# CODARcode/MGARD

Hardware: AMD Instinct MI355X
Metric: compress GB/s (input) at rel-Linf 1e-3, 3D 512^3 f32, decompose+quantize on device-resident data (higher is better)
Workload: dtype f32; 1 GPU; 3D 512x512x512 float32 uniform grid, REL L-inf tol 1e-3, s=inf; [norm+]decompose+quantize (int64 out); l_target=9, dict_size=8192, parallelism=1 subdomain per GPU

## Files before the change

### include/mgard_hip.h

```cpp
#ifndef MGARD_HIP_H
#define MGARD_HIP_H

#include <stddef.h>
#include <stdint.h>

#ifdef __cplusplus
extern "C" {
#endif

typedef enum mgh_status {
  MGH_SUCCESS = 0,
  MGH_ERR_INVALID_ARGUMENT = -1,
  MGH_ERR_UNSUPPORTED_DIMENSION = -2,
  MGH_ERR_UNSUPPORTED_DTYPE = -3,
  MGH_ERR_DEVICE = -4,
  MGH_ERR_OUT_OF_MEMORY = -5,
  MGH_ERR_NO_DEVICE = -6
} mgh_status;

typedef enum mgh_dtype { MGH_FLOAT = 0, MGH_DOUBLE = 1 } mgh_dtype;
typedef enum mgh_error_bound { MGH_REL = 0, MGH_ABS = 1 } mgh_error_bound;

#define MGH_MAX_DIM 5

// ... 30 lines not shown
int mgh_dequantize(mgh_hierarchy *h, int64_t *d_quantized, int error_bound_type, double tol,
                   double s, double norm, uint64_t dict_size, int prep_huffman,
                   const uint64_t *d_outlier_idx, const int64_t *d_outlier_val,
                   uint64_t outlier_count, void *d_coeff, void *stream);

int mgh_decompose_quantize(mgh_hierarchy *h, const void *d_data, int error_bound_type,
                           double tol, double s, double norm, double *h_norm_out,
                           uint64_t dict_size, int prep_huffman, int64_t *d_quantized,
                           uint64_t *d_outlier_count, uint64_t *d_outlier_idx,
                           int64_t *d_outlier_val, uint64_t outlier_capacity,
                           void *d_coeff_opt, void *stream);

int mgh_decompose_quantize_sym16(mgh_hierarchy *h, const void *d_data, int error_bound_type,
                                 double tol, double s, double norm, double *h_norm_out,
                                 uint64_t dict_size, uint16_t *d_symbols,
                                 uint64_t *d_outlier_count, uint64_t *d_outlier_idx,
                                 int64_t *d_outlier_val, uint64_t outlier_capacity, void *stream);

int mgh_dequantize_recompose_sym16(mgh_hierarchy *h, const uint16_t *d_symbols, int error_bound_type,
                                   double tol, double s, double norm, uint64_t dict_size,
                                   const uint64_t *d_outlier_idx, const int64_t *d_outlier_val,
                                   uint64_t outlier_count, void *d_data_out, void *stream);
int mgh_sym16_supported(const mgh_hierarchy *h);

#define MGH_LD_IN 0
#define MGH_LD_OUT 1
int mgh_set_ld(mgh_hierarchy *h, int which, const uint64_t *ld);

int mgh_norm_stream_begin(mgh_hierarchy *h, void *stream);
int mgh_norm_stream_add(mgh_hierarchy *h, const void *d_part, uint64_t count, double s, int cold,
                        void *stream);

int mgh_norm_device(mgh_hierarchy *h, const void *d_data, double s, void *d_norm_out,
                    void *stream);

int mgh_decompose_quantize_dn(mgh_hierarchy *h, const void *d_data, int error_bound_type,
                              double tol, double s, const void *d_norm, uint64_t num_subdomains,
                              uint64_t dict_size, int prep_huffman, int64_t *d_quantized,
                              uint64_t *d_outlier_count, uint64_t *d_outlier_idx,
                              int64_t *d_outlier_val, uint64_t outlier_capacity, void *stream);

int mgh_dequantize_recompose(mgh_hierarchy *h, int64_t *d_quantized, int error_bound_type,
                             double tol, double s, double norm, uint64_t dict_size,
                             int prep_huffman, const uint64_t *d_outlier_idx,
                             const int64_t *d_outlier_val, uint64_t outlier_count, void *d_data,
                             void *stream);

int mgh_recompose_to_level(mgh_hierarchy *h, const void *d_coeff, int level, void *d_out, void *stream);
int mgh_dequantize_recompose_to_level(mgh_hierarchy *h, int64_t *d_quantized, int error_bound_type,
                                      double tol, double s, double norm, uint64_t dict_size,
                                      int prep_huffman, const uint64_t *d_outlier_idx,
                                      const int64_t *d_outlier_val, uint64_t outlier_count, int level,
                                      void *d_out, void *stream);
int mgh_dequantize_recompose_sym16_to_level(mgh_hierarchy *h, const uint16_t *d_symbols,
                                            int error_bound_type, double tol, double s, double norm,
                                            uint64_t dict_size, const uint64_t *d_outlier_idx,
                                            const int64_t *d_outlier_val, uint64_t outlier_count,
                                            int level, void *d_out, void *stream);
int mgh_level_box_from_linear(mgh_hierarchy *h, const int64_t *d_linear, int level, int64_t *d_box_out,
                              void *stream);
int mgh_dequantize_recompose_linear_to_level(mgh_hierarchy *h, int64_t *d_linear, int error_bound_type,
                                             double tol, double s, double norm, uint64_t dict_size,
                                             int prep_huffman, const uint64_t *d_outlier_idx,
                                             const int64_t *d_outlier_val, uint64_t outlier_count,
                                             int level, void *d_out, void *stream);
int mgh_refine_level(mgh_hierarchy *h, const void *d_coarse, int64_t *d_segment, int error_bound_type,
                     double tol, double s, double norm, uint64_t dict_size, int prep_huffman,
                     const uint64_t *d_outlier_idx, const int64_t *d_outlier_val, uint64_t outlier_count,
                     int level, void *d_out, void *stream);
int mgh_level_nodes(const mgh_hierarchy *h, int level, int dim, uint64_t *h_idx_out, uint64_t cap);

int mgh_outlier_restore(int64_t *d_q, uint64_t n, const uint64_t *d_outlier_idx,
                        const int64_t *d_outlier_val, uint64_t outlier_count, void *stream);

int mgh_level_linearize(mgh_hierarchy *h, const int64_t *d_in, int64_t *d_out, int inverse,
                        uint64_t *d_outlier_idx, const uint64_t *d_outlier_count, uint64_t outlier_count,
                        uint64_t outlier_capacity, void *stream);

int mgh_profile_enable(mgh_hierarchy *h, int enable);
int mgh_profile_filter(mgh_hierarchy *h, const char *kernel_name_or_null);
int mgh_profile_read(mgh_hierarchy *h, const char **names, double *total_ms, uint64_t *launches,
                     int cap, int reset);

int mgh_stream_calibrate(int dtype, const void *d_in, int64_t *d_out, void *d_side, uint64_t n,
                         int reps, double *ms_out, void *stream);

#ifdef __cplusplus
}
#endif
#endif
```

### mgard_amd/__init__.py

```python
import ctypes as C
import os

import numpy as np

from . import _build

REL, ABS = 0, 1
LD_IN, LD_OUT = 0, 1
FLOAT, DOUBLE = 0, 1
INF = float("inf")

_lib = None

SYMBOLS = [
    "mgh_last_error", "mgh_device_count", "mgh_hierarchy_create", "mgh_hierarchy_destroy",
    "mgh_l_target", "mgh_level_shape", "mgh_total_num_elems", "mgh_device_bytes", "mgh_norm_device_ptr",
    "mgh_hierarchy_table", "mgh_norm", "mgh_decompose", "mgh_recompose", "mgh_quantize",
    "mgh_dequantize", "mgh_decompose_quantize", "mgh_dequantize_recompose",
    "mgh_norm_device", "mgh_decompose_quantize_dn", "mgh_decompose_quantize_sym16",
    "mgh_dequantize_recompose_sym16", "mgh_sym16_supported",
    "mgh_profile_enable", "mgh_profile_filter", "mgh_profile_read", "mgh_stream_calibrate",
    "mgh_level_linearize", "mgh_outlier_restore", "mgh_norm_stream_begin", "mgh_norm_stream_add",
    "mgh_set_ld",
    "mgh_recompose_to_level", "mgh_dequantize_recompose_to_level",
    "mgh_dequantize_recompose_sym16_to_level", "mgh_level_nodes",
    "mgh_level_box_from_linear", "mgh_dequantize_recompose_linear_to_level",
    "mgh_refine_level",
]


class MgardHipError(RuntimeError):
    pass


def lib_path():
    return _build.LIB


def load_library():
    global _lib
    if _lib is not None:
        return _lib
    if not os.path.exists(_build.LIB):
        raise MgardHipError(
            "libmgard_hip.so is not built: run `python -c 'import __graft_entry__ as g; g.build()'`")
    import torch
    L = C.CDLL(_build.LIB)
    vp, u64, i64p, u64p = C.c_void_p, C.c_uint64, C.POINTER(C.c_int64), C.POINTER(C.c_uint64)
    L.mgh_last_error.restype = C.c_char_p
    L.mgh_device_count.restype = C.c_int
    L.mgh_hierarchy_create.argtypes = [C.POINTER(vp), C.c_int, u64p, C.c_int, C.POINTER(vp),
                                       C.c_int, u64, C.c_int]
    L.mgh_hierarchy_destroy.argtypes = [vp]
    L.mgh_hierarchy_destroy.restype = None
    L.mgh_l_target.argtypes = [vp]
    L.mgh_level_shape.argtypes = [vp, C.c_int, u64p]
    L.mgh_total_num_elems.argtypes = [vp]
    L.mgh_total_num_elems.restype = u64
    L.mgh_device_bytes.argtypes = [vp]
    L.mgh_device_bytes.restype = C.c_size_t
    L.mgh_hierarchy_table.argtypes = [vp, C.c_int, C.c_int, C.c_int, vp, u64]
    L.mgh_hierarchy_table.restype = C.c_int64
    L.mgh_norm.argtypes = [vp, vp, C.c_double, C.POINTER(C.c_double), vp]
    L.mgh_decompose.argtypes = [vp, vp, vp, vp]
    L.mgh_recompose.argtypes = [vp, vp, vp, vp]
    L.mgh_quantize.argtypes = [vp, vp, C.c_int, C.c_double, C.c_double, C.c_double, u64, C.c_int,
                               vp, vp, vp, vp, u64, vp]
    L.mgh_dequantize.argtypes = [vp, vp, C.c_int, C.c_double, C.c_double, C.c_double, u64,
                                 C.c_int, vp, vp, u64, vp, vp]
    L.mgh_decompose_quantize.argtypes = [vp, vp, C.c_int, C.c_double, C.c_double, C.c_double,
                                         C.POINTER(C.c_double), u64, C.c_int, vp, vp, vp, vp, u64,
                                         vp, vp]
    L.mgh_norm_device.argtypes = [vp, vp, C.c_double, vp, vp]
    L.mgh_norm_stream_begin.argtypes = [vp, vp]
    L.mgh_set_ld.argtypes = [vp, C.c_int, u64p]
    L.mgh_norm_stream_add.argtypes = [vp, vp, u64, C.c_double, C.c_int, vp]
    L.mgh_dequantize_recompose_sym16.argtypes = [vp, vp, C.c_int, C.c_double, C.c_double, C.c_double, u64,
                                                 vp, vp, u64, vp, vp]
    L.mgh_sym16_supported.argtypes = [vp]
    L.mgh_decompose_quantize_sym16.argtypes = [vp, vp, C.c_int, C.c_double, C.c_double, C.c_double,
                                               C.POINTER(C.c_double), u64, vp, vp, vp, vp, u64, vp]
    L.mgh_decompose_quantize_dn.argtypes = [vp, vp, C.c_int, C.c_double, C.c_double, vp, u64, u64,
                                            C.c_int, vp, vp, vp, vp, u64, vp]
    L.mgh_dequantize_recompose.argtypes = [vp, vp, C.c_int, C.c_double, C.c_double, C.c_double,
                                           u64, C.c_int, vp, vp, u64, vp, vp]
    L.mgh_profile_enable.argtypes = [vp, C.c_int]
    L.mgh_profile_filter.argtypes = [vp, C.c_char_p]
    L.mgh_profile_read.argtypes = [vp, C.POINTER(C.c_char_p), C.POINTER(C.c_double), u64p,
                                   C.c_int, C.c_int]
    L.mgh_outlier_restore.argtypes = [vp, u64, vp, vp, u64, vp]
    L.mgh_level_linearize.argtypes = [vp, vp, vp, C.c_int, vp, vp, u64, u64, vp]
    L.mgh_recompose_to_level.argtypes = [vp, vp, C.c_int, vp, vp]
    L.mgh_dequantize_recompose_to_level.argtypes = [vp, vp, C.c_int, C.c_double, C.c_double, C.c_double,
                                                    u64, C.c_int, vp, vp, u64, C.c_int, vp, vp]
    L.mgh_dequantize_recompose_sym16_to_level.argtypes = [vp, vp, C.c_int, C.c_double, C.c_double,
                                                          C.c_double, u64, vp, vp, u64, C.c_int, vp, vp]
    L.mgh_level_box_from_linear.argtypes = [vp, vp, C.c_int, vp, vp]
    L.mgh_dequantize_recompose_linear_to_level.argtypes = [vp, vp, C.c_int, C.c_double, C.c_double, C.c_double,
                                                           u64, C.c_int, vp, vp, u64, C.c_int, vp, vp]
    L.mgh_refine_level.argtypes = [vp, vp, vp, C.c_int, C.c_double, C.c_double, C.c_double, u64, C.c_int, vp, vp, u64,
                                   C.c_int, vp, vp]
    L.mgh_level_nodes.argtypes = [vp, C.c_int, C.c_int, u64p, u64]
    L.mgh_stream_calibrate.argtypes = [C.c_int, vp, vp, vp, u64, C.c_int, C.POINTER(C.c_double), vp]
    _lib = L
    return L


def _check(rc):
    if rc < 0:
        raise MgardHipError("mgard_hip error %d: %s" % (rc, load_library().mgh_last_error().decode()))
    return rc


def _stream():
    import torch
    return C.c_void_p(torch.cuda.current_stream().cuda_stream)


_NP = {FLOAT: np.float32, DOUBLE: np.float64}


class Hierarchy:

    def __init__(self, shape, dtype="float32", coords=None, normalize_coordinates=True,
                 max_level=None, device=0):
        import torch
        L = load_library()
        if not torch.cuda.is_available():
            raise MgardHipError("no HIP device visible: mgard_amd has no CPU fallback")
        self.shape = tuple(int(s) for s in shape)
        self.D = len(self.shape)
        self.np_dtype = np.dtype(dtype)
        self.dtype = {np.dtype(np.float32): FLOAT, np.dtype(np.float64): DOUBLE}[self.np_dtype]
        self.torch_dtype = torch.float32 if self.dtype == FLOAT else torch.float64
        self.device = int(device)
        shp = (C.c_uint64 * self.D)(*self.shape)
        cptr = None
        if coords is not None:
            self._coords = [np.ascontiguousarray(c, dtype=self.np_dtype) for c in coords]
            cptr = (C.c_void_p * self.D)(*[c.ctypes.data for c in self._coords])
        h = C.c_void_p()
        _check(L.mgh_hierarchy_create(C.byref(h), self.D, shp, self.dtype, cptr,
                                      int(normalize_coordinates),
                                      2**64 - 1 if max_level is None else int(max_level),
                                      self.device))
        self._h = h
        self._ld = {LD_IN: None, LD_OUT: None}
        self.l_target = L.mgh_l_target(h)
        self.total = int(L.mgh_total_num_elems(h))

    def close(self):
        if getattr(self, "_h", None) and _lib is not None:
            try:
                _lib.mgh_hierarchy_destroy(self._h)
            except Exception:
                pass
            self._h = None

    __del__ = close

    def level_shape(self, l):
        out = (C.c_uint64 * self.D)()
        _check(load_library().mgh_level_shape(self._h, l, out))
        return tuple(int(x) for x in out)

    def level_nodes(self, level, dim):
        n = self.shape[dim] if 0 <= dim < self.D else 1
        out = (C.c_uint64 * n)()
# ... 199 lines not shown
                self._h, self._chk(q, torch.int64), ebtype, tol, s, norm, dict_size, int(prep_huffman),
                C.c_void_p(outlier_idx.data_ptr() if n else 0),
                C.c_void_p(outlier_val.data_ptr() if n else 0), n, int(level),
                C.c_void_p(out.data_ptr()), _stream()))
            return out
        out = self._new_out(q.device) if out is None else out
        _check(load_library().mgh_dequantize_recompose(
            self._h, self._chk(q, torch.int64), ebtype, tol, s, norm, dict_size, int(prep_huffman),
            C.c_void_p(outlier_idx.data_ptr() if n else 0),
            C.c_void_p(outlier_val.data_ptr() if n else 0), n, self._chk(out), _stream()))
        return out

    def level_linearize(self, q, inverse=False, outlier_idx=None):
        import torch
        out = torch.empty_like(q)
        n = 0 if outlier_idx is None else int(outlier_idx.numel())
        _check(load_library().mgh_level_linearize(
            self._h, self._chk(q, torch.int64), C.c_void_p(out.data_ptr()), int(inverse),
            C.c_void_p(outlier_idx.data_ptr() if n else 0), None, n, 0, _stream()))
        return out

    def _linear_head(self, lin, level):
        import torch
        need = 1
        for e in self.level_shape(level):
            need *= int(e)
        if not (lin.is_cuda and lin.dtype == torch.int64 and lin.is_contiguous() and lin.numel() >= need):
            raise ValueError("expected a contiguous cuda int64 tensor of at least %d elements "
                             "(the head of the level-linearised array)" % need)
        return need

    def level_box_from_linear(self, lin, level, out=None):
        import torch
        need = self._linear_head(lin, level)
        if out is None:
            out = torch.empty(tuple(int(e) for e in self.level_shape(level)), dtype=torch.int64, device=lin.device)
        elif not (out.is_cuda and out.dtype == torch.int64 and out.is_contiguous() and out.numel() >= need):
            raise ValueError("out: expected a contiguous cuda int64 tensor of at least %d elements" % need)
        _check(load_library().mgh_level_box_from_linear(
            self._h, C.c_void_p(lin.data_ptr()), int(level), C.c_void_p(out.data_ptr()), _stream()))
        return out

    def dequantize_recompose_linear(self, lin, ebtype, tol, s, norm, dict_size=8192, prep_huffman=True,
                                    outlier_idx=None, outlier_val=None, out=None, level=None):
        level = self.l_target if level is None else int(level)
        self._linear_head(lin, level)
        n = 0 if outlier_idx is None else int(outlier_idx.numel())
        out = self._level_out(level, out, lin.device)
        _check(load_library().mgh_dequantize_recompose_linear_to_level(
            self._h, C.c_void_p(lin.data_ptr()), ebtype, tol, s, norm, dict_size, int(prep_huffman),
            C.c_void_p(outlier_idx.data_ptr() if n else 0), C.c_void_p(outlier_val.data_ptr() if n else 0),
            n, level, C.c_void_p(out.data_ptr()), _stream()))
        return out

    def refine_level(self, coarse, segment, ebtype, tol, s, norm, level, dict_size=8192, prep_huffman=True,
                     outlier_idx=None, outlier_val=None, out=None):
        import torch
        level = int(level)
        if not 1 <= level <= self.l_target:
            raise ValueError("level must be in 1 .. l_target")
        lo = hi = 1
        for e in self.level_shape(level - 1):
            lo *= int(e)
        for e in self.level_shape(level):
            hi *= int(e)
        if not (coarse.is_cuda and coarse.is_contiguous() and coarse.dtype == self.torch_dtype and
                coarse.numel() == lo):
            raise ValueError("coarse: expected the contiguous cuda array of level %d (%d elements)" % (level - 1, lo))
        if not (segment.is_cuda and segment.dtype == torch.int64 and segment.is_contiguous() and
                segment.numel() >= hi - lo):
            raise ValueError("segment: expected a contiguous cuda int64 tensor of at least %d elements" % (hi - lo))
        n = 0 if outlier_idx is None else int(outlier_idx.numel())
        out = self._level_out(level, out, coarse.device)
        _check(load_library().mgh_refine_level(
            self._h, C.c_void_p(coarse.data_ptr()), C.c_void_p(segment.data_ptr()), ebtype, tol, s, norm, dict_size,
            int(prep_huffman), C.c_void_p(outlier_idx.data_ptr() if n else 0),
            C.c_void_p(outlier_val.data_ptr() if n else 0), n, level, C.c_void_p(out.data_ptr()), _stream()))
        return out

    def profile(self, enable=True, only=None):
        _check(load_library().mgh_profile_filter(self._h, only.encode() if only else None))
        _check(load_library().mgh_profile_enable(self._h, int(enable)))

    def profile_read(self, reset=True):
        cap = 64
        names = (C.c_char_p * cap)()
        ms = (C.c_double * cap)()
        cnt = (C.c_uint64 * cap)()
        n = _check(load_library().mgh_profile_read(self._h, names, ms, cnt, cap, int(reset)))
        return {names[i].decode(): (ms[i], int(cnt[i])) for i in range(min(n, cap))}
```

### mgard_amd/csrc/capi.hip

```cpp
#include "../../include/mgard_hip.h"

#include <hip/hip_runtime.h>
#include <hip/hip_ext.h>

#include <cmath>
#include <cstdio>
#include <cstdlib>
#include <cstring>
#include <limits>
#include <atomic>
#include <map>
#include <mutex>
#include <string>
#include <type_traits>
#include <vector>

#include "env.hpp"
#include "hierarchy.hpp"
#include "ipk_plan.hpp"
#include "kernels_v1.hpp"
#include "kernels_ipk.hpp"
#include "kernels_ipk_stream.hpp"
#include "kernels_ipk_spec.hpp"
#include "kernels_ipk_dma.hpp"
#include "kernels_fused.hpp"
#include "kernels_fused2.hpp"
#include "kernels_box.hpp"
#include "kernels_tail.hpp"
#include "kernels_recompose.hpp"
#include "kernels_recompose2.hpp"
#include "kernels_nd.hpp"
#include "kernels_level.hpp"

namespace {

thread_local std::string g_last_error;

int fail(int code, const std::string &msg) {
  g_last_error = msg;
  return code;
}

#define HIP_TRY(expr)                                                                          \
  do {                                                                                         \
    hipError_t _e = (expr);                                                                    \
    if (_e != hipSuccess)                                                                      \
      return fail(_e == hipErrorOutOfMemory ? MGH_ERR_OUT_OF_MEMORY : MGH_ERR_DEVICE,          \
                  std::string(#expr) + ": " + hipGetErrorString(_e));                          \
  } while (0)

struct ProfileEntry {
  std::vector<std::pair<hipEvent_t, hipEvent_t>> pending;
  double total_ms = 0;
  uint64_t launches = 0;
};

}

struct mgh_hierarchy {
  int dtype = MGH_FLOAT;
  int device = 0;
  size_t num_cu = 256;
  int D = 0, L = 0;
  uint64_t total = 0;
  uint64_t plane_elems = 0;
  void *host = nullptr;
  void *impl = nullptr;
  bool profiling = false;
  int nd_rows = 1;
  bool force_nd_ipk = false;
  bool force_v1 = false;
  int force_v1_env = -1;
  bool force_nd = false;
  std::string prof_filter;
  mgh::IpkTuning ipk;
  int absmax_warm_mb = 192;
  int fused_faces = 1;
  int fused_tall = 1;
  int slice_batch = 1;
  int fused_xcd = 1;
  int fused_fixed = 1;
  int fused_wide = 1;
  int fused4 = 1;
  int box = 1;
  int outlier_agg = 2;
  int sym16_mixed = 1;
  int tail_solves = 1;
  size_t cls1 = 256, cls2 = 2048;
  int rch[3] = {1, 4, 16};
  int ipk_range_mb = 128;
  bool no_head = false;
  bool debug_sync = false;
  std::map<std::string, ProfileEntry> prof;
  size_t device_bytes = 0;
  uint64_t shape[MGH_MAX_DIM] = {};
  uint64_t ld[2][MGH_MAX_DIM] = {};
  bool has_ld[2] = {false, false};
};

namespace {

using namespace mgh;

template <typename T> int chunk_warmup_need(const std::vector<T> &tt) {
  const size_t n = tt.size() / 3;
  if (n < 2) return 0;
  const double target = -((sizeof(T) == 4 ? 24 : 53) + 12);
  std::vector<double> lf(n), lb(n);
  for (size_t i = 0; i < n; i++) {
    const double f = std::fabs((double)tt[i]);
    const double b = tt[2 * n + i] != 0 ? std::fabs((double)tt[n + i] / (double)tt[2 * n + i]) : 0.0;
    lf[i] = f > 0 ? std::log2(f) : -64.0;
    lb[i] = b > 0 ? std::log2(b) : -64.0;
  }
  int need = 0;
  for (const auto *lg : {&lf, &lb}) {
    for (size_t i = 0; i < n; i++) {
      double acc = 0;
      size_t k = 0;
      while (i + k < n && acc > target) acc += (*lg)[i + k++];
      if (acc > target) break;
      need = std::max(need, (int)k);
    }
  }
  return (need + 7) / 8 * 8;
}

template <typename T> struct LevelTables {
  const T *ratio[3] = {nullptr, nullptr, nullptr};
  const T *mass[3] = {nullptr, nullptr, nullptr};
  const T *thomas[3] = {nullptr, nullptr, nullptr};
  Box3 box;
  bool active[3] = {false, false, false};
};

template <typename T> struct DeviceState {
  HostHierarchy<T> *hh = nullptr;
  T *tables = nullptr;
  int *marks = nullptr;
  std::vector<LevelTables<T>> lt;
  std::vector<size_t> lt_end;
  struct NdLevel {
    const T *ratio[kNd], *mass[kNd], *thomas[kNd];
  };
  std::vector<NdLevel> nd;
  T *nd_w = nullptr, *nd_a = nullptr, *nd_b = nullptr;
  size_t nd_cap = 0;
  std::vector<T *> nodal4;
  T *load4 = nullptr, *corr4 = nullptr;
  bool state4_ready = false;
  std::vector<T *> nodal;
  T *t1 = nullptr, *t2 = nullptr, *t3 = nullptr;
  int t12_level = 0;
  T *level_box = nullptr;
  size_t level_box_elems = 0;
  T *scratch_full = nullptr;
  T *qz = nullptr;
  unsigned long long *scalar = nullptr;
  unsigned long long *fscal = nullptr;
  int scalar_slot = 0;
  bool fscal_dirty = false;
  bool norm_streamed = false;
  T *normval = nullptr;
  unsigned long long *oh_key = nullptr;
  long long *oh_val = nullptr;
  size_t oh_slots = 0;
  int64_t *qbox = nullptr;
  size_t qbox_elems = 0;
  T *spec_y = nullptr, *spec_a = nullptr, *spec_b = nullptr;
  size_t spec_y_elems = 0, spec_edge_elems = 0;
  unsigned long long *spec_fixed = nullptr;
  unsigned long long *outliers_seen = nullptr;
  QuantMeta qmeta;
  size_t full_I = 0, full_J = 0;
  T *pack_in = nullptr, *pack_out = nullptr;
};

template <typename T> HostHierarchy<T> *HH(const mgh_hierarchy *h) {
  return static_cast<HostHierarchy<T> *>(h->host);
}
template <typename T> DeviceState<T> *DS(const mgh_hierarchy *h) {
  return static_cast<DeviceState<T> *>(h->impl);
}

template <typename F> int launch(mgh_hierarchy *h, const char *name, hipStream_t s, F &&f) {
  if (h->debug_sync) {
    std::fprintf(stderr, "[mgh] %s\n", name);
    std::fflush(stderr);
    f();
    HIP_TRY(hipGetLastError());
    HIP_TRY(hipDeviceSynchronize());
    return MGH_SUCCESS;
  }
  if (!h->profiling || (!h->prof_filter.empty() && h->prof_filter != name)) {
    f();
    HIP_TRY(hipGetLastError());
    return MGH_SUCCESS;
  }
  hipEvent_t a, b;
  HIP_TRY(hipEventCreate(&a));
  HIP_TRY(hipEventCreate(&b));
  HIP_TRY(hipEventRecord(a, s));
  f();
  HIP_TRY(hipGetLastError());
  HIP_TRY(hipEventRecord(b, s));
  h->prof[name].pending.emplace_back(a, b);
  return MGH_SUCCESS;
}

template <typename K, typename... Args>
int launch_kernel(mgh_hierarchy *h, const char *name, hipStream_t s, K kernel, dim3 grid, dim3 block,
                  size_t lds, Args... args) {
  if (h->debug_sync || !h->profiling || (!h->prof_filter.empty() && h->prof_filter != name))
    return launch(h, name, s, [&] { hipLaunchKernelGGL(kernel, grid, block, (uint32_t)lds, s, args...); });
  hipEvent_t a, b;
  HIP_TRY(hipEventCreate(&a));
  HIP_TRY(hipEventCreate(&b));
  hipExtLaunchKernelGGL(kernel, grid, block, (uint32_t)lds, s, a, b, 0, args...);
  HIP_TRY(hipGetLastError());
  h->prof[name].pending.emplace_back(a, b);
  return MGH_SUCCESS;
}

#define TRY(expr)                 \
  do {                            \
    int _rc = (expr);             \
    if (_rc != MGH_SUCCESS) return _rc; \
  } while (0)

inline dim3 grid3(uint32_t n0, uint32_t n1, uint32_t n2, dim3 blk) {
  return dim3((n2 + blk.x - 1) / blk.x, (n1 + blk.y - 1) / blk.y, n0);
}

template <typename T> int dev_alloc(mgh_hierarchy *h, T **p, size_t count) {
  *p = nullptr;
  if (count == 0) return MGH_SUCCESS;
  HIP_TRY(hipMalloc((void **)p, count * sizeof(T)));
  h->device_bytes += count * sizeof(T);
  return MGH_SUCCESS;
}

template <typename T> void dev_free(mgh_hierarchy *h, T **p, size_t count) {
  if (!*p) return;
  if (hipFree(*p) == hipSuccess) h->device_bytes -= std::min(h->device_bytes, count * sizeof(T));
  *p = nullptr;
}

template <typename T> int build_device_state(mgh_hierarchy *h) {
  HostHierarchy<T> *hh = HH<T>(h);
  auto *ds = new DeviceState<T>();
  h->impl = ds;
  ds->hh = hh;
  const int D = hh->D, L = hh->L;
  if (D > 3) {
    std::vector<T> arena;
    auto push = [&](const std::vector<T> &v) {
      size_t off = arena.size();
      arena.insert(arena.end(), v.begin(), v.end());
      while (arena.size() % 4) arena.push_back(0);
      return off;
    };
    struct Off { size_t r[kNd], m[kNd], t[kNd]; };
    std::vector<Off> offs(L + 1);
    for (int l = 1; l <= L; l++)
      for (int d = 0; d < D; d++) {
        offs[l].r[d] = push(hh->lv[l][d].ratio);
        offs[l].m[d] = push(hh->mass_table(l, d));
// ... 19 lines not shown
    TRY(dev_alloc(h, &ds->marks, marks.size()));
    HIP_TRY(hipMemcpy(ds->marks, marks.data(), marks.size() * sizeof(int), hipMemcpyHostToDevice));
    TRY(dev_alloc(h, &ds->qz, (size_t)2 * (L + 1)));
    TRY(dev_alloc(h, &ds->scalar, (size_t)2));
    TRY(dev_alloc(h, &ds->fscal, (size_t)2));
    HIP_TRY(hipMemset(ds->fscal, 0, 16));
    TRY(dev_alloc(h, &ds->normval, (size_t)2));
    return MGH_SUCCESS;
  }

  std::vector<T> arena;
  auto push = [&](const std::vector<T> &v) {
    size_t off = arena.size();
    arena.insert(arena.end(), v.begin(), v.end());
    while (arena.size() % 4) arena.push_back(0);
    return off;
  };
  struct Off {
    size_t ratio[3], mass[3], thomas[3];
  };
  std::vector<Off> offs(L + 1);
  ds->lt.resize(L + 1);
  for (int l = 1; l <= L; l++) {
    LevelTables<T> &t = ds->lt[l];
    for (int k = 0; k < 3; k++) {
      const int d = D - 3 + k;
      if (d < 0) {
        t.box.n[k] = t.box.m[k] = 1;
        t.active[k] = false;
        continue;
      }
      t.active[k] = true;
      t.box.n[k] = (uint32_t)hh->level_shape[l][d];
      t.box.m[k] = (uint32_t)hh->level_shape[l - 1][d];
      offs[l].ratio[k] = push(hh->lv[l][d].ratio);
      offs[l].mass[k] = push(hh->mass_table(l, d));
      const std::vector<T> tt = hh->thomas_table(l - 1, d);
      h->ipk.chunk_need = std::max(h->ipk.chunk_need, chunk_warmup_need(tt));
      offs[l].thomas[k] = push(tt);
    }
  }
  TRY(dev_alloc(h, &ds->tables, arena.size()));
  HIP_TRY(hipMemcpy(ds->tables, arena.data(), arena.size() * sizeof(T), hipMemcpyHostToDevice));
  ds->lt_end.assign(L + 1, 0);
  for (int l = 1; l <= L; l++) {
    size_t next = arena.size();
    for (int l2 = l + 1; l2 <= L && next == arena.size(); l2++)
      for (int k = 0; k < 3; k++)
        if (ds->lt[l2].active[k]) {
          next = offs[l2].ratio[k];
          break;
        }
    ds->lt_end[l] = next;
  }
  for (int l = 1; l <= L; l++)
    for (int k = 0; k < 3; k++)
      if (ds->lt[l].active[k]) {
        ds->lt[l].ratio[k] = ds->tables + offs[l].ratio[k];
        ds->lt[l].mass[k] = ds->tables + offs[l].mass[k];
        ds->lt[l].thomas[k] = ds->tables + offs[l].thomas[k];
      }

  ds->nd.resize(L + 1);
  for (int l = 1; l <= L; l++)
    for (int d = 0; d < D; d++) {
      const int k = d + 3 - D;
      ds->nd[l].ratio[d] = ds->lt[l].ratio[k];
      ds->nd[l].mass[d] = ds->lt[l].mass[k];
      ds->nd[l].thomas[d] = ds->lt[l].thomas[k];
    }

  std::vector<int> marks;
  ds->qmeta.D = D;
  ds->qmeta.calc_vol = 0;
  for (int d = 0; d < D; d++) {
    ds->qmeta.shape[d] = (uint32_t)hh->shape[d];
    ds->qmeta.markoff[d] = (uint32_t)marks.size();
    marks.insert(marks.end(), hh->marks[d].begin(), hh->marks[d].end());
  }
  TRY(dev_alloc(h, &ds->marks, marks.size()));
  HIP_TRY(hipMemcpy(ds->marks, marks.data(), marks.size() * sizeof(int), hipMemcpyHostToDevice));

  ds->nodal.assign(L + 1, nullptr);
  for (int l = 0; l < L; l++) {
    size_t cnt = 1;
    for (int d = 0; d < D; d++) cnt *= hh->level_shape[l][d];
    TRY(dev_alloc(h, &ds->nodal[l], cnt));
  }
  if (L >= 1) {
    const Box3 &b = ds->lt[L].box;
    TRY(dev_alloc(h, &ds->t3, (size_t)b.m[0] * b.m[1] * b.m[2]));
  }
  TRY(dev_alloc(h, &ds->qz, (size_t)2 * (L + 1)));
  TRY(dev_alloc(h, &ds->scalar, (size_t)2));
  TRY(dev_alloc(h, &ds->fscal, (size_t)2));
  HIP_TRY(hipMemset(ds->fscal, 0, 16));
  TRY(dev_alloc(h, &ds->normval, (size_t)2));
  ds->full_J = hh->shape[D - 1];
  ds->full_I = (D >= 2 ? hh->shape[D - 2] : 1) * ds->full_J;
  return MGH_SUCCESS;
}

template <typename T> void destroy_state(mgh_hierarchy *h) {
  auto *ds = DS<T>(h);
  if (ds) {
    (void)hipFree(ds->tables);
    (void)hipFree(ds->marks);
    for (T *p : ds->nodal) (void)hipFree(p);
    (void)hipFree(ds->t1);
    (void)hipFree(ds->t2);
    (void)hipFree(ds->t3);
    (void)hipFree(ds->scratch_full);
    (void)hipFree(ds->pack_in);
    (void)hipFree(ds->pack_out);
    (void)hipFree(ds->nd_w);
    (void)hipFree(ds->nd_a);
    (void)hipFree(ds->nd_b);
    for (T *p : ds->nodal4) (void)hipFree(p);
    (void)hipFree(ds->load4);
    (void)hipFree(ds->corr4);
    (void)hipFree(ds->qz);
    (void)hipFree(ds->scalar);
    (void)hipFree(ds->fscal);
    (void)hipFree(ds->normval);
    (void)hipFree(ds->oh_key);
    (void)hipFree(ds->oh_val);
    (void)hipFree(ds->qbox);
    (void)hipFree(ds->level_box);
    (void)hipFree(ds->spec_y);
    (void)hipFree(ds->spec_a);
    (void)hipFree(ds->spec_b);
    (void)hipFree(ds->spec_fixed);
    (void)hipHostFree(ds->outliers_seen);
    delete ds;
  }
  delete HH<T>(h);
}

template <typename T> int ensure_scratch(mgh_hierarchy *h) {
  auto *ds = DS<T>(h);
  if (!ds->scratch_full) TRY(dev_alloc(h, &ds->scratch_full, (size_t)h->total));
  return MGH_SUCCESS;
}

template <typename K> int allow_big_lds(K kernel, size_t bytes = kLdsPerCU) {
  HIP_TRY(hipFuncSetAttribute(reinterpret_cast<const void *>(kernel),
                              hipFuncAttributeMaxDynamicSharedMemorySize, (int)bytes));
  return MGH_SUCCESS;
}
template <typename K> int allow_big_lds_once(K kernel, std::atomic<uint64_t> &done, size_t bytes = kLdsPerCU) {
  int dev = 0;
  HIP_TRY(hipGetDevice(&dev));
  const uint64_t bit = (uint64_t)1 << (dev & 63);
  if (done.load(std::memory_order_acquire) & bit) return MGH_SUCCESS;
  TRY(allow_big_lds(kernel, bytes));
  done.fetch_or(bit, std::memory_order_release);
  return MGH_SUCCESS;
}

template <int... V, typename F> int with_value(int v, F &&f) {
  int rc = MGH_ERR_INVALID_ARGUMENT;
  (void)((v == V ? (rc = f(std::integral_constant<int, V>{}), true) : false) || ...);
  return rc;
}

template <typename T> struct IpkArgs {
  mgh_hierarchy *h;
  const char *name;
  T *x;
  const T *tt;
  T *add_to;
  int sign;
  hipStream_t s;
  int add() const { return add_to ? (sign > 0 ? 1 : -1) : 0; }
};

template <typename T> int spec_scratch(mgh_hierarchy *h, size_t total, size_t edges, hipStream_t s) {
  auto *ds = DS<T>(h);
  if (total > ds->spec_y_elems) {
    (void)hipFree(ds->spec_y);
    ds->spec_y = nullptr;
    ds->spec_y_elems = 0;
    HIP_TRY(hipMalloc(&ds->spec_y, total * sizeof(T)));
    ds->spec_y_elems = total;
  }
  if (edges > ds->spec_edge_elems) {
    (void)hipFree(ds->spec_a);
    (void)hipFree(ds->spec_b);
    ds->spec_a = ds->spec_b = nullptr;
    ds->spec_edge_elems = 0;
    HIP_TRY(hipMalloc(&ds->spec_a, edges * sizeof(T)));
    HIP_TRY(hipMalloc(&ds->spec_b, edges * sizeof(T)));
    ds->spec_edge_elems = edges;
  }
  if (!ds->spec_fixed) {
    HIP_TRY(hipMalloc(&ds->spec_fixed, 16));
    HIP_TRY(hipMemsetAsync(ds->spec_fixed, 0, 16, s));
  }
  return MGH_SUCCESS;
}

template <typename T> int ipk_launch_spec(const IpkPlan &p, const IpkArgs<T> &a, int axis) {
  const IpkGeom &g = p.geom;
  const SpecGeom G{g.n, p.S, p.K, p.nchunk, g.npencil, g.n_inner, g.outer_stride, g.inner_stride, g.stride, axis != 2};
  const size_t total = (size_t)g.npencil * g.n;
  TRY(spec_scratch<T>(a.h, total, (size_t)g.npencil * p.nchunk, a.s));
  auto *ds = DS<T>(a.h);
  T *x = a.x, *y = ds->spec_y, *ea = ds->spec_a, *eb = ds->spec_b;
  unsigned long long *fx = ds->spec_fixed;
  unsigned *mm = reinterpret_cast<unsigned *>(ds->spec_fixed + 1);
  hipStream_t s = a.s;
  HIP_TRY(hipMemsetAsync(mm, 0, 8, s));
  return launch(a.h, a.name, s, [&] {
    k_ipk_spec_fwd<T><<<p.grid, 64, 0, s>>>(G, x, y, a.tt, ea, eb);
    k_ipk_spec_check<T><<<p.check_grid, 256, 0, s>>>(p.nchunk, g.npencil, ea, eb, +1, mm);
    k_ipk_spec_fix<T><<<p.fix_grid, 64, 0, s>>>(G, x, y, a.tt, ea, eb, +1, fx, mm);
    k_ipk_spec_bwd<T><<<p.grid, 64, 0, s>>>(G, y, x, a.tt, ea, eb);
    k_ipk_spec_check<T><<<p.check_grid, 256, 0, s>>>(p.nchunk, g.npencil, ea, eb, -1, mm + 1);
    k_ipk_spec_fix<T><<<p.fix_grid, 64, 0, s>>>(G, y, x, a.tt, ea, eb, -1, fx, mm + 1);
    if (a.add_to) k_ipk_spec_apply<T><<<p.apply_grid, 256, 0, s>>>(total, a.add_to, x, a.sign);
  });
}

template <typename T, bool CHUNKED> int ipk_launch_lds_contig(const IpkPlan &p, const IpkArgs<T> &a) {
  static std::atomic<uint64_t> once{0};
  TRY(allow_big_lds_once(k_ipk_lds_contig<T, CHUNKED>, once, p.lds_attr));
  return launch(a.h, a.name, a.s, [&] {
    k_ipk_lds_contig<T, CHUNKED><<<p.grid, p.block, p.lds, a.s>>>(p.geom.npencil, p.geom.n, p.pad, p.magic, p.P,
                                                                  a.x, a.tt, a.add_to, a.sign, p.K);
  });
}

template <typename T, int ADD> int ipk_launch_dma(const IpkPlan &p, const IpkArgs<T> &a) {
  constexpr uint32_t U = 64 / sizeof(T), KR = 10;
  const IpkGeom &g = p.geom;
  static std::atomic<uint64_t> once{0};
  TRY(allow_big_lds_once(k_ipk_dma<T, U, KR, ADD>, once, p.lds_attr));
  return launch(a.h, a.name, a.s, [&] {
    k_ipk_dma<T, U, KR, ADD><<<p.grid, p.block, p.lds, a.s>>>(g.npencil, g.n_inner, g.outer_stride, 1, g.stride,
                                                              g.n, a.x, a.tt, a.add_to);
  });
}

template <typename T, int KR, bool CONTIG> int ipk_launch_stream(const IpkPlan &p, const IpkArgs<T> &a) {
  constexpr uint32_t U = 64 / sizeof(T);
  const IpkGeom &g = p.geom;
  static std::atomic<uint64_t> once{0};
  TRY(allow_big_lds_once(k_ipk_stream<T, U, KR, 1, CONTIG, false>, once, p.lds_attr));
  return launch(a.h, a.name, a.s, [&] {
    k_ipk_stream<T, U, KR, 1, CONTIG, false><<<p.grid, p.block, p.lds, a.s>>>(
        g.npencil, g.n_inner, g.outer_stride, g.inner_stride, g.stride, g.n, p.W, p.n_glob, a.x, a.tt, a.add_to,
        a.sign);
  });
}

template <typename T, int W> int ipk_launch_lds_strided(const IpkPlan &p, const IpkArgs<T> &a) {
  const IpkGeom &g = p.geom;
  static std::atomic<uint64_t> once{0};
  TRY(allow_big_lds_once(k_ipk_lds_strided<T, W>, once, p.lds_attr));
  return launch(a.h, a.name, a.s, [&] {
    k_ipk_lds_strided<T, W><<<p.grid, p.block, p.lds, a.s>>>(g.npencil / g.n_inner, g.n_inner, g.outer_stride,
                                                             g.stride, g.n, a.x, a.tt, a.add_to, a.sign);
  });
}

template <typename T, int AXIS> int ipk_launch_thread(const IpkPlan &p, const IpkArgs<T> &a, const uint32_t *m) {
  return launch(a.h, a.name, a.s, [&] {
    k_ipk<T, AXIS><<<dim3(p.grid, p.grid_y, 1), dim3(p.block, 1, 1), 0, a.s>>>(m[0], m[1], m[2], a.x, a.tt,
                                                                             a.add_to, a.sign);
  });
}

template <typename T>
int ipk_launch(mgh_hierarchy *h, int axis, const uint32_t *m, T *x, const T *tt, T *add_to,
               int sign, hipStream_t s, uint32_t nbatch = 1, size_t batch_stride = 0) {
  if (nbatch > 1 && axis != 0) return fail(MGH_ERR_INVALID_ARGUMENT, "ipk_launch: batches along the slowest axis only");
  static const char *names[3] = {"ipk_r", "ipk_c", "ipk_f"};
  const IpkArgs<T> a{h, names[axis], x, tt, add_to, sign, s};
  const IpkPlan p = ipk_plan(h->ipk, sizeof(T), axis, m, nbatch, batch_stride);
  switch (p.kernel) {
  case IpkKernel::Spec: return ipk_launch_spec<T>(p, a, axis);
  case IpkKernel::LdsContigChunked: return ipk_launch_lds_contig<T, true>(p, a);
  case IpkKernel::Dma:
    if constexpr (sizeof(T) == 4)
      return with_value<0, 1, -1>(a.add(), [&](auto add) { return ipk_launch_dma<T, add()>(p, a); });
    break;
  case IpkKernel::Stream:
    if constexpr (sizeof(T) == 4)
      if (p.KR == 16)
        return axis == 2 ? ipk_launch_stream<T, 16, true>(p, a) : ipk_launch_stream<T, 16, false>(p, a);
    return axis == 2 ? ipk_launch_stream<T, 8, true>(p, a) : ipk_launch_stream<T, 8, false>(p, a);
  case IpkKernel::LdsContig: return ipk_launch_lds_contig<T, false>(p, a);
  case IpkKernel::LdsStrided:
    return with_value<64, 48, 32, 16>((int)p.W, [&](auto w) { return ipk_launch_lds_strided<T, w()>(p, a); });
  case IpkKernel::Thread:
    if (p.per_batch) {
      for (uint32_t bi = 0; bi < nbatch; bi++)
        TRY(ipk_launch<T>(h, axis, m, x + (size_t)bi * batch_stride, tt,
                          add_to ? add_to + (size_t)bi * batch_stride : nullptr, sign, s));
      return MGH_SUCCESS;
    }
    return with_value<0, 1, 2>(axis, [&](auto ax) { return ipk_launch_thread<T, ax()>(p, a, m); });
  }
  return fail(MGH_ERR_INVALID_ARGUMENT, "ipk_launch: no kernel for this plan");
}

template <typename T>
int ipk_fc_launch(mgh_hierarchy *h, const uint32_t *m, T *x, const T *tt_f, const T *tt_c,
                  hipStream_t s) {
  const uint32_t pitch = m[2] | 1u;
  if (ipk_plane_fits_lds(sizeof(T), m)) {
    static std::atomic<uint64_t> once{0};
    TRY(allow_big_lds_once(k_ipk_plane_fc<T>, once));
    const uint32_t magic = (uint32_t)((((uint64_t)1 << 32) + m[2] - 1) / m[2]);
    return launch(h, "ipk_fc", s, [&] {
      k_ipk_plane_fc<T><<<m[0], 256, (size_t)m[1] * pitch * sizeof(T), s>>>(m[1], m[2], pitch, magic,
                                                                              x, tt_f, tt_c);
    });
  }
  TRY(ipk_launch<T>(h, 2, m, x, tt_f, nullptr, +1, s));
  return ipk_launch<T>(h, 1, m, x, tt_c, nullptr, +1, s);
}

template <typename T>
int correction(mgh_hierarchy *h, int l, const T *coef, size_t cI, size_t cJ, T *target, int sign,
               hipStream_t s, int top_level = -1) {
  auto *ds = DS<T>(h);
  const LevelTables<T> &t = ds->lt[l];
  const Box3 &b = t.box;
  const dim3 blk(64, 4, 1);
  const int tl = top_level < 0 ? h->L : top_level;
  if (ds->t12_level < tl) {
    if (ds->t12_level >= 1) {
      const Box3 &ob = ds->lt[ds->t12_level].box;
      dev_free(h, &ds->t1, (size_t)ob.n[0] * ob.n[1] * ob.m[2]);
      dev_free(h, &ds->t2, (size_t)ob.n[0] * ob.m[1] * ob.m[2]);
      ds->t12_level = 0;
    }
    const Box3 &tb = ds->lt[tl].box;
    const size_t c1 = (size_t)tb.n[0] * tb.n[1] * tb.m[2], c2 = (size_t)tb.n[0] * tb.m[1] * tb.m[2];
    int rc = dev_alloc(h, &ds->t1, c1);
    if (rc == MGH_SUCCESS) rc = dev_alloc(h, &ds->t2, c2);
    if (rc != MGH_SUCCESS) {
      dev_free(h, &ds->t1, c1);
      dev_free(h, &ds->t2, c2);
      return rc;
    }
    ds->t12_level = tl;
  }
  TRY(launch(h, "lpk_f", s, [&] {
    k_lpk<T, 2><<<grid3(b.n[0], b.n[1], b.m[2], blk), blk, 0, s>>>(
        b.n[0], b.n[1], b.n[2], b.n[2], b.m[2], coef, cI, cJ, ds->t1, (size_t)b.n[1] * b.m[2],
        (size_t)b.m[2], t.mass[2], b.m[0], b.m[1]);
  }));
  T *cur = ds->t1;
  if (t.active[1]) {
    TRY(launch(h, "lpk_c", s, [&] {
      k_lpk<T, 1><<<grid3(b.n[0], b.m[1], b.m[2], blk), blk, 0, s>>>(
          b.n[0], b.n[1], b.m[2], b.n[1], b.m[1], cur, (size_t)b.n[1] * b.m[2], (size_t)b.m[2],
          ds->t2, (size_t)b.m[1] * b.m[2], (size_t)b.m[2], t.mass[1], 0, 0);
    }));
    cur = ds->t2;
  }
  if (t.active[0]) {
    TRY(launch(h, "lpk_r", s, [&] {
      k_lpk<T, 0><<<grid3(b.m[0], b.m[1], b.m[2], blk), blk, 0, s>>>(
          b.n[0], b.m[1], b.m[2], b.n[0], b.m[0], cur, (size_t)b.m[1] * b.m[2], (size_t)b.m[2],
          ds->t3, (size_t)b.m[1] * b.m[2], (size_t)b.m[2], t.mass[0], 0, 0);
    }));
    cur = ds->t3;
  }
  const int last = t.active[0] ? 0 : (t.active[1] ? 1 : 2);
  TRY(ipk_launch<T>(h, 2, b.m, cur, t.thomas[2], last == 2 ? target : nullptr, sign, s));
  if (t.active[1])
    TRY(ipk_launch<T>(h, 1, b.m, cur, t.thomas[1], last == 1 ? target : nullptr, sign, s));
  if (t.active[0]) TRY(ipk_launch<T>(h, 0, b.m, cur, t.thomas[0], target, sign, s));
  return MGH_SUCCESS;
}

template <typename T> struct QuantParams {
  std::vector<T> qz, vol;
  int64_t dict_size = 0;
  int prep_huffman = 0;
  int64_t *q = nullptr;
  uint16_t *q16 = nullptr;
  unsigned long long *ocount = nullptr;
  uint64_t *oidx = nullptr;
  int64_t *oval = nullptr;
  unsigned long long ocap = 0;
  const T *d_qp = nullptr;
};

template <typename T>
QuantParams<T> make_quant_params(mgh_hierarchy *h, int ebtype, double tol, double s, double norm,
                                 bool reciprocal) {
  auto *hh = HH<T>(h);
  QuantParams<T> qp;
  qp.qz.resize(h->L + 1);
  qp.vol.resize(h->L + 1);
  hh->quantizers(ebtype, (T)tol, (T)s, (T)norm, reciprocal, qp.qz.data());
  const bool calc_vol = !((T)s == std::numeric_limits<T>::infinity());
  for (int l = 0; l <= h->L; l++) qp.vol[l] = calc_vol ? hh->level_volume(l, !reciprocal) : (T)1;
  return qp;
}
// ... 105 lines not shown
  bool native3 = false;
};
inline Layout make_layout(const mgh_hierarchy *h, const uint64_t *ext, bool pitched) {
  Layout lay;
  const int D = h->D;
  uint64_t st = 1, str[MGH_MAX_DIM] = {};
  for (int d = D - 1; d >= 0; d--) {
    str[d] = st;
    st *= ext[d];
  }
  lay.view.rows = 1;
  for (int k = 0; k < MGH_MAX_DIM; k++) {
    const int d = k - (MGH_MAX_DIM - D);
    lay.view.ext[k] = d >= 0 ? (uint32_t)h->shape[d] : 1u;
    lay.view.stride[k] = d >= 0 ? str[d] : 0;
    if (k < MGH_MAX_DIM - 1) lay.view.rows *= lay.view.ext[k];
  }
  lay.J = (size_t)ext[D - 1];
  lay.I = (size_t)((D >= 2 ? ext[D - 2] : 1) * ext[D - 1]);
  lay.pitched = pitched;
  lay.native3 = pitched && fused_ok(h) && !h->force_v1 && lay.I < ((size_t)1 << 30);
  return lay;
}
inline Layout dense_layout(const mgh_hierarchy *h) { return make_layout(h, h->shape, false); }
inline Layout caller_layout(const mgh_hierarchy *h, int which) {
  return h->has_ld[which] ? make_layout(h, h->ld[which], true) : dense_layout(h);
}

template <typename T, int OUT, typename AfterFirst>
int decompose_fused4(mgh_hierarchy *h, const T *data, T *coeff, const QuantParams<T> *qp,
                     hipStream_t s, AfterFirst &&after_first);

template <typename T, int OUT, typename AfterFirst>
int decompose_fused(mgh_hierarchy *h, const T *data, const Layout &in, T *coeff, const QuantParams<T> *qp,
                    hipStream_t s, AfterFirst &&after_first) {
  if (h->D == 4) return decompose_fused4<T, OUT>(h, data, coeff, qp, s, after_first);
  auto *ds = DS<T>(h);
  const int L = h->L;
  const size_t fI = ds->full_I, fJ = ds->full_J;
  const T *src = data;
  size_t sI = in.I, sJ = in.J;

  FusedArgs<T> A{};
  A.coef = coeff;
  A.dI = fI;
  A.dJ = fJ;
  if (OUT == OUT_Q) {
    A.q = qp->q;
    A.q16 = qp->q16;
    A.dict_size = qp->dict_size;
    A.prep_huffman = qp->prep_huffman;
    A.outlier_count = qp->ocount;
    A.outlier_idx = qp->oidx;
    A.outlier_val = qp->oval;
    A.outlier_cap = qp->ocap;
    A.qp = qp->d_qp;
    A.nlev = L + 1;
  }
  const bool agg = OUT == OUT_Q && outlier_agg_now<T>(h, qp);
  constexpr size_t kTailLdsMax = 150 * 1024;
  int l_tail = 0;
  for (int l = std::min(L, kTailMaxLevels); l >= 1; l--) {
    const size_t tab = ds->lt_end[std::min(l + 1, L)];
    if ((tail_lds_elems(ds->lt[l].box) + tab) * sizeof(T) + tail_header_bytes<T>() <= kTailLdsMax) {
      l_tail = l;
      break;
    }
  }
  bool tail_pre = false;
  for (int l = L; l > l_tail; l--) {
    const LevelTables<T> &t = ds->lt[l];
    const Box3 &b = t.box;
    for (int k = 0; k < 3; k++) {
      A.n[k] = (int)b.n[k];
      A.m[k] = (int)b.m[k];
      A.ratio[k] = t.ratio[k];
      A.mass[k] = t.mass[k];
    }
    A.u = src;
    A.uI = sI;
    A.uJ = sJ;
    A.coarse = ds->nodal[l - 1];
    A.load = ds->t3;
    A.level = l;
    if (OUT == OUT_Q && !qp->d_qp) {
      A.quantizer = qp->qz[l];
      A.volume = qp->vol[l];
    }
    const int cls = level_class(h, b);
    if (l == L) TRY(after_first());
    if (OUT == OUT_Q && !(qp->dict_size >= 0 && qp->dict_size <= ((int64_t)1 << 30)))
      return fail(MGH_ERR_INVALID_ARGUMENT, "fused path: dict_size must be at most 2^30");
    if (cls < h->box) {
      constexpr int BR = 4, BC = 4, BF = 8;
      const int bx = ((int)b.m[2] + BF - 1) / BF, by = ((int)b.m[1] + BC - 1) / BC,
                bz = ((int)b.m[0] + BR - 1) / BR;
      TRY(launch(h, OUT == OUT_Q ? "level_box_q" : "level_box", s, [&] {
        k_level_box<T, OUT, BR, BC, BF><<<(unsigned)(bx * by * bz), 256, 0, s>>>(A, bx, by);
      }));
    } else {
      const char *nm = cls == 2 ? (OUT == OUT_Q ? "level_fused_q" : "level_fused")
                                : (OUT == OUT_Q ? "level_fused_q_small" : "level_fused_small");
      if (OUT == OUT_Q && agg) {
        if (A.prep_huffman && !A.q16 && h->fused_fixed)
          TRY((launch_fused2<T, OUT == OUT_Q ? OUT_QH : OUT, OUT == OUT_Q>(h, A, b, cls, nm, s)));
        else
          TRY((launch_fused2<T, OUT, OUT == OUT_Q>(h, A, b, cls, nm, s)));
      } else if (OUT == OUT_Q && A.prep_huffman && !A.q16 && h->fused_fixed)
        TRY((launch_fused2<T, OUT == OUT_Q ? OUT_QH : OUT>(h, A, b, cls, nm, s)));
      else
        TRY((launch_fused2<T, OUT>(h, A, b, cls, nm, s)));
    }
    tail_pre = h->tail_solves && l == l_tail + 1 && l_tail >= 1;
    if (!tail_pre) {
      const size_t box_b = (size_t)b.m[0] * b.m[1] * b.m[2] * sizeof(T);
      const size_t range_b = (size_t)h->ipk_range_mb << 20;
      if (range_b && box_b > 2 * range_b) {
        const uint32_t nrange = (uint32_t)((box_b + range_b - 1) / range_b);
        for (uint32_t k = 0; k < nrange; k++) {
          const uint32_t R_lo = (uint32_t)((uint64_t)b.m[0] * k / nrange), R_hi = (uint32_t)((uint64_t)b.m[0] * (k + 1) / nrange);
          const uint32_t ms[3] = {R_hi - R_lo, b.m[1], b.m[2]};
          TRY(ipk_fc_launch<T>(h, ms, ds->t3 + (size_t)R_lo * b.m[1] * b.m[2], t.thomas[2], t.thomas[1], s));
        }
      } else {
        TRY(ipk_fc_launch<T>(h, b.m, ds->t3, t.thomas[2], t.thomas[1], s));
      }
      TRY(ipk_launch<T>(h, 0, b.m, ds->t3, t.thomas[0], ds->nodal[l - 1], +1, s));
    }
    src = ds->nodal[l - 1];
    sJ = b.m[2];
    sI = (size_t)b.m[1] * b.m[2];
  }
  if (L <= l_tail) TRY(after_first());
  if (l_tail >= 1) {
    TailArgs<T> TA{};
    TA.nlevels = l_tail;
    TA.fine = src;
    TA.fI = sI;
    TA.fJ = sJ;
    if (tail_pre) {
      TA.pre_load = ds->t3;
      for (int k = 0; k < 3; k++) TA.pre_thomas[k] = ds->lt[l_tail + 1].thomas[k];
    }
    for (int l = l_tail; l >= 1; l--) {
      TailLevel<T> &tl = TA.lv[l_tail - l];
      const LevelTables<T> &t = ds->lt[l];
      tl.b = t.box;
      for (int k = 0; k < 3; k++) {
        tl.ratio[k] = t.ratio[k];
        tl.mass[k] = t.mass[k];
        tl.thomas[k] = t.thomas[k];
      }
      tl.level = l;
      if (OUT == OUT_Q && !qp->d_qp) {
        tl.quantizer = qp->qz[l];
        tl.volume = qp->vol[l];
      }
    }
    if (OUT == OUT_Q && !qp->d_qp) {
      TA.head_quantizer = qp->qz[0];
      TA.head_volume = qp->vol[0];
    }
    TA.out = A;
    TA.outliers_seen = OUT == OUT_Q && A.prep_huffman ? ds->outliers_seen : nullptr;
    const size_t tab = ds->lt_end[tail_pre ? l_tail + 1 : l_tail];
    TA.tab_base = ds->tables;
    TA.tab_count = (uint32_t)tab;
    const size_t lds = (tail_lds_elems(ds->lt[l_tail].box) + tab) * sizeof(T) + tail_header_bytes<T>();
    static std::atomic<uint64_t> once{0};
    TRY(allow_big_lds_once(k_tail<T, OUT>, once));
    TRY(launch(h, "tail", s, [&] { k_tail<T, OUT><<<1, 1024, lds, s>>>(TA); }));
  } else {
    const Box3 &b = ds->lt[1].box;
    if (OUT == OUT_Q && !qp->d_qp) {
      A.quantizer = qp->qz[0];
      A.volume = qp->vol[0];
    }
    TRY(launch(h, "head_out", s, [&] {
      const size_t tot = (size_t)b.m[0] * b.m[1] * b.m[2];
      k_head_out<T, OUT><<<(unsigned)std::min<size_t>((tot + 255) / 256, 1024), 256, 0, s>>>(
          (int)b.m[0], (int)b.m[1], (int)b.m[2], ds->nodal[0], A);
    }));
    if (OUT == OUT_Q && A.prep_huffman && A.outlier_count && ds->outliers_seen)
      k_publish_count<<<1, 1, 0, s>>>(A.outlier_count, ds->outliers_seen);
  }
  return MGH_SUCCESS;
}

template <typename T, int OUT, int TC, int TF, bool AGG = false>
int launch_fused4_t(mgh_hierarchy *h, const FusedArgs<T> &A, const Fused4<T> &Q, const Box3 &b, int cls,
                    int n_t, int m_t, hipStream_t s) {
    const int RCHv = fused_rch(h, cls);
    Fused2Grid G{};
    G.rch = RCHv;
    const int mfi = (int)b.m[2], mci = (int)b.m[1], mri = (int)b.m[0];
    const int nfull_f = (mfi - 1) / TF, rem_f = mfi - nfull_f * TF;
    const int nfull_c = (mci - 1) / TC, rem_c = mci - nfull_c * TC;
    const bool face_f = h->fused_faces && nfull_f >= 1 && rem_f <= 4;
    const bool face_c = h->fused_faces && nfull_c >= 1 && rem_c <= 4;
    G.gxm = face_f ? nfull_f : (mfi + TF - 1) / TF;
    const int gym = face_c ? nfull_c : (mci + TC - 1) / TC;
    G.n_main = G.gxm * gym;
    G.ff_F0 = nfull_f * TF;
    G.n_ff = face_f ? (mci + 63) / 64 : 0;
    G.cf_C0 = nfull_c * TC;
    G.n_cf = face_c ? ((face_f ? G.ff_F0 : mfi) + 63) / 64 : 0;
    G.nchunk = fused_nchunk(mri, RCHv);
    G.chunk_hi = G.nchunk;
    const unsigned ntile = (unsigned)(G.n_main + G.n_ff + G.n_cf);
    G.xcd_ranges = ntile >= kXcdRangeMinTiles ? h->fused_xcd : 0;
    const unsigned gx = G.xcd_ranges ? (ntile + 7) / 8 * 8 : ntile;
    const bool faces = G.n_ff || G.n_cf;
    const unsigned n_even = (unsigned)m_t, n_odd = (unsigned)(n_t - m_t);
#define MGH_F4(RCH, TMODE, NZ, NAME)                                                          \
  if ((NZ) > 0) {                                                                             \
    const dim3 grid(gx, (unsigned)G.nchunk, (NZ));                                            \
    if (faces)                                                                                \
      TRY(launch_kernel(h, NAME, s, k_level_fused2<T, OUT, TC, TF, RCH, true, TMODE, AGG>, grid, dim3(256), 0, A, G, Q));  \
    else                                                                                      \
      TRY(launch_kernel(h, NAME, s, k_level_fused2<T, OUT, TC, TF, RCH, false, TMODE, AGG>, grid, dim3(256), 0, A, G, Q)); \
  }
    MGH_F4(16, 1, n_even, "level4_even")
    MGH_F4(16, 2, n_odd, "level4_odd")
#undef MGH_F4
    return MGH_SUCCESS;
}

template <typename T>
int tsweep_launch(mgh_hierarchy *h, const T *load, T *corr, size_t M, int m_t, const T *mass, hipStream_t s) {
  constexpr int MT = 9;
  if (m_t <= MT) {
    const unsigned blocks = (unsigned)std::min<size_t>((M + 255) / 256, (size_t)h->num_cu * 32);
    return launch(h, "tsweep", s, [&] { k_tsweep_once<T, MT><<<blocks, 256, 0, s>>>(load, corr, M, m_t, mass); });
  }
  const dim3 grid((unsigned)std::min<size_t>((M + 255) / 256, 4096), (unsigned)m_t, 1);
  return launch(h, "tsweep", s, [&] { k_tsweep<T><<<grid, 256, 0, s>>>(load, corr, M, m_t, mass); });
}

template <typename T>
int tsolve_apply(mgh_hierarchy *h, T *corr, T *coarse, size_t M, int m_t, size_t m_rc, size_t m_f,
                 const T *tt, int sign, hipStream_t s) {
  constexpr int MT = 9;
  if (m_t <= MT) {
    const unsigned blocks = (unsigned)std::min<size_t>((M + 255) / 256, (size_t)h->num_cu * 32);
    return launch(h, "ipk_t", s, [&] {
      k_tsolve_apply<T, MT><<<blocks, 256, 0, s>>>(corr, coarse, M, m_t, tt, sign);
    });
  }
  const uint32_t m3t[3] = {(uint32_t)m_t, (uint32_t)m_rc, (uint32_t)m_f};
  return ipk_launch<T>(h, 0, m3t, corr, tt, coarse, sign, s);
}

template <typename T> int ensure_state4(mgh_hierarchy *h) {
  auto *ds = DS<T>(h);
  auto *hh = HH<T>(h);
  const int L = h->L;
  const auto &sh = hh->level_shape;
  if (ds->state4_ready) return MGH_SUCCESS;
  const size_t M = (size_t)sh[L - 1][1] * sh[L - 1][2] * sh[L - 1][3];
  auto nodal_count = [&](int l) { return (size_t)sh[l][0] * sh[l][1] * sh[l][2] * sh[l][3]; };
  const size_t load_count = (2 * (size_t)sh[L - 1][0] - 1) * M, corr_count = (size_t)sh[L - 1][0] * M;
  auto drop = [&] {
    for (size_t l = 0; l < ds->nodal4.size(); l++) dev_free(h, &ds->nodal4[l], nodal_count((int)l));
    ds->nodal4.clear();
    dev_free(h, &ds->load4, load_count);
    dev_free(h, &ds->corr4, corr_count);
  };
  drop();
  ds->nodal4.assign(L + 1, nullptr);
  int rc = MGH_SUCCESS;
  for (int l = 0; l < L && rc == MGH_SUCCESS; l++) rc = dev_alloc(h, &ds->nodal4[l], nodal_count(l));
  if (rc == MGH_SUCCESS) rc = dev_alloc(h, &ds->load4, load_count);
  if (rc == MGH_SUCCESS) rc = dev_alloc(h, &ds->corr4, corr_count);
  if (rc != MGH_SUCCESS) {
    drop();
    return rc;
  }
  ds->state4_ready = true;
  return MGH_SUCCESS;
}

template <typename T, int OUT, typename AfterFirst>
int decompose_fused4(mgh_hierarchy *h, const T *data, T *coeff, const QuantParams<T> *qp,
                     hipStream_t s, AfterFirst &&after_first) {
  auto *ds = DS<T>(h);
  auto *hh = HH<T>(h);
  const int L = h->L;
  const auto &sh = hh->level_shape;
  const size_t full[4] = {(size_t)sh[L][1] * sh[L][2] * sh[L][3], (size_t)sh[L][2] * sh[L][3],
                          (size_t)sh[L][3], 1};
  TRY(ensure_state4<T>(h));
  FusedArgs<T> A{};
  A.coef = coeff;
  A.dI = full[1];
  A.dJ = full[2];
  if (OUT == OUT_Q) {
    A.q = qp->q;
    A.q16 = qp->q16;
    A.dict_size = qp->dict_size;
    A.prep_huffman = qp->prep_huffman;
    A.outlier_count = qp->ocount;
    A.outlier_idx = qp->oidx;
    A.outlier_val = qp->oval;
    A.outlier_cap = qp->ocap;
    A.qp = qp->d_qp;
    A.nlev = L + 1;
  }
  TRY(after_first());
  const bool agg = OUT == OUT_Q && outlier_agg_now<T>(h, qp);
  const T *src = data;
  size_t sT = full[0], sI = full[1], sJ = full[2];
  for (int l = L; l >= 1; l--) {
    const auto &N = sh[l], &Mc = sh[l - 1];
    Box3 b;
    for (int k = 0; k < 3; k++) {
      b.n[k] = (uint32_t)N[1 + k];
      b.m[k] = (uint32_t)Mc[1 + k];
      A.n[k] = (int)N[1 + k];
      A.m[k] = (int)Mc[1 + k];
      A.ratio[k] = ds->nd[l].ratio[1 + k];
      A.mass[k] = ds->nd[l].mass[1 + k];
    }
    const size_t M = (size_t)Mc[1] * Mc[2] * Mc[3];
    const int n_t = (int)N[0], m_t = (int)Mc[0];
    A.u = src;
    A.uI = sI;
    A.uJ = sJ;
    A.coarse = ds->nodal4[l - 1];
    A.load = ds->load4;
    A.level = l;
    if (OUT == OUT_Q && !qp->d_qp) {
      A.quantizer = qp->qz[l];
      A.volume = qp->vol[l];
    }
    Fused4<T> Q{};
    Q.ratio_t = ds->nd[l].ratio[0];
    Q.uT = sT;
    Q.dT = full[0];
    Q.cT = M;
    Q.n_t = n_t;
    Q.m_t = m_t;
    if (n_t % 2 == 0)
      HIP_TRY(hipMemsetAsync(ds->load4 + (size_t)(n_t - 1) * M, 0, M * sizeof(T), s));
    const int cls = level_class(h, b, (size_t)std::max(1, n_t - m_t));
    const bool wide = fused_wide_tiles(h, cls, b.m[2]), tall = fused_tall_tiles(h, b);
    if (OUT == OUT_Q && agg) {
      if (tall) TRY((launch_fused4_t<T, OUT, 64, 4, OUT == OUT_Q>(h, A, Q, b, cls, n_t, m_t, s)));
      else if (wide) TRY((launch_fused4_t<T, OUT, 4, 64, OUT == OUT_Q>(h, A, Q, b, cls, n_t, m_t, s)));
      else TRY((launch_fused4_t<T, OUT, 8, 32, OUT == OUT_Q>(h, A, Q, b, cls, n_t, m_t, s)));
    } else if (tall)
      TRY((launch_fused4_t<T, OUT, 64, 4>(h, A, Q, b, cls, n_t, m_t, s)));
    else if (wide)
      TRY((launch_fused4_t<T, OUT, 4, 64>(h, A, Q, b, cls, n_t, m_t, s)));
    else
      TRY((launch_fused4_t<T, OUT, 8, 32>(h, A, Q, b, cls, n_t, m_t, s)));
    {
      TRY((tsweep_launch<T>(h, ds->load4, ds->corr4, M, m_t, ds->nd[l].mass[0], s)));
    }
    const uint32_t m3a[3] = {(uint32_t)(m_t * Mc[1]), (uint32_t)Mc[2], (uint32_t)Mc[3]};
    TRY(ipk_launch<T>(h, 2, m3a, ds->corr4, ds->nd[l].thomas[3], nullptr, +1, s));
    TRY(ipk_launch<T>(h, 1, m3a, ds->corr4, ds->nd[l].thomas[2], nullptr, +1, s));
    TRY(ipk_launch<T>(h, 0, b.m, ds->corr4, ds->nd[l].thomas[1], nullptr, +1, s, (uint32_t)m_t, M));
    TRY((tsolve_apply<T>(h, ds->corr4, ds->nodal4[l - 1], M, m_t, Mc[1] * Mc[2], Mc[3], ds->nd[l].thomas[0], +1, s)));
    src = ds->nodal4[l - 1];
    sT = M;
    sI = (size_t)Mc[2] * Mc[3];
    sJ = Mc[3];
  }
  {
    if (OUT == OUT_Q && !qp->d_qp) {
      A.quantizer = qp->qz[0];
      A.volume = qp->vol[0];
    }
    const auto &M0 = sh[0];
    const size_t tot = (size_t)M0[0] * M0[1] * M0[2] * M0[3];
    TRY(launch(h, "head_out", s, [&] {
      k_head_out4<T, OUT><<<(unsigned)std::min<size_t>((tot + 1023) / 1024, 1024), 1024, 0, s>>>(
          (int)M0[0], (int)M0[1], (int)M0[2], (int)M0[3], ds->nodal4[0], A, full[0]);
    }));
    if (OUT == OUT_Q && A.prep_huffman && A.outlier_count && ds->outliers_seen)
      k_publish_count<<<1, 1, 0, s>>>(A.outlier_count, ds->outliers_seen);
  }
  return MGH_SUCCESS;
}

template <typename T, int OUT>
int decompose_fused(mgh_hierarchy *h, const T *data, const Layout &in, T *coeff, const QuantParams<T> *qp,
                    hipStream_t s) {
  return decompose_fused<T, OUT>(h, data, in, coeff, qp, s, [] { return (int)MGH_SUCCESS; });
}

template <typename T> int nd_ensure(mgh_hierarchy *h, size_t count = 0) {
  auto *ds = DS<T>(h);
  if (!count) count = (size_t)h->total;
  if (ds->nd_cap < count) {
    dev_free(h, &ds->nd_w, ds->nd_cap);
    dev_free(h, &ds->nd_a, ds->nd_cap);
    dev_free(h, &ds->nd_b, ds->nd_cap);
    ds->nd_cap = 0;
    int rc = dev_alloc(h, &ds->nd_w, count);
    if (rc == MGH_SUCCESS) rc = dev_alloc(h, &ds->nd_a, count);
    if (rc == MGH_SUCCESS) rc = dev_alloc(h, &ds->nd_b, count);
    if (rc != MGH_SUCCESS) {
      dev_free(h, &ds->nd_w, count);
      dev_free(h, &ds->nd_a, count);
      dev_free(h, &ds->nd_b, count);
      return rc;
    }
    ds->nd_cap = count;
  }
  return MGH_SUCCESS;
}
// ... 1366 lines not shown
      if (D == 4) TRY(ensure_state4<T>(h));
      TRY(coarse_in<T>(h, D == 4 ? ds->nodal4[start - 1] : ds->nodal[start - 1], tg.coarse, start - 1, st));
    }
    RecomposeArgs<T> A{};
    A.q = src.q;
    A.half = dict_half(qs);
    A.dI = ds->full_I;
    A.dJ = ds->full_J;
    const size_t sT = compact ? box_source(A, D, lb.m) : 0;
    TRY((recompose_levels_any<T, int64_t>(h, A, sT, level_quanta<T>(h, qs), out, lay, st, nullptr, 1, stop, start)));
    return o.finish(h, st);
  }
  if (stop == L && !start) {
    TRY(dequantize_dense<T>(h, src.q, qs, out, st));
    TRY(recompose_dense<T>(h, out, out, st));
    return o.finish(h, st);
  }
  TRY(upload_quantizers<T>(h, qs.ebtype, qs.tol, qs.s, qs.norm, false, st));
  TRY(outliers_back(h, qs, "outlier_restore", st, k_outlier_restore_in_box, src.q, lb));
  if (start)
    for (int d = 0; d < D; d++) lb.n[d] = (uint32_t)HH<T>(h)->level_shape[stop - 1][d];
  const uint64_t rows = level_box_rows(lb);
  const T *coarse = (const T *)tg.coarse;
  return recompose_box_to_level<T>(h, stop, out, st, [&](T *dst) {
    if (start)
      return launch(h, "box_refine_fill", st, [&] {
        k_box_refine_fill<T><<<level_box_grid(lb), 256, 0, st>>>(lb, ds->qmeta, src.q, coarse, ds->marks, ds->qz,
                                                                    ds->qz + (L + 1), (int64_t)qs.dict_size,
                                                                    qs.prep_huffman, dst, rows);
      });
    return launch(h, "box_dequantize", st, [&] {
      k_box_dequantize<T><<<level_box_grid(lb), 256, 0, st>>>(lb, ds->qmeta, src.q, ds->marks, ds->qz,
                                                                 ds->qz + (L + 1), (int64_t)qs.dict_size,
                                                                 qs.prep_huffman, dst, rows);
    });
  }, start, tg.coarse);
}

template <typename T> int norm_stream_begin(mgh_hierarchy *h, hipStream_t st) {
  auto *ds = DS<T>(h);
  if (ds->fscal_dirty) HIP_TRY(hipMemsetAsync(ds->fscal, 0, 16, st));
  ds->fscal_dirty = true;
  ds->norm_streamed = true;
  return MGH_SUCCESS;
}
template <typename T>
int norm_stream_add(mgh_hierarchy *h, const T *part, size_t count, double s, int cold, hipStream_t st) {
  auto *ds = DS<T>(h);
  if (!ds->norm_streamed) return fail(MGH_ERR_INVALID_ARGUMENT, "mgh_norm_stream_add without mgh_norm_stream_begin");
  if (count == 0) return MGH_SUCCESS;
  unsigned long long *slot = ds->fscal + ds->scalar_slot;
  const unsigned grid = (unsigned)std::min<size_t>((count + 1023) / 1024, 256 * 8);
  if ((T)s == std::numeric_limits<T>::infinity())
    return launch(h, "absmax", st, [&] { k_absmax<T><<<grid, 256, 0, st>>>(part, count, slot, cold ? count : 0); });
  return launch(h, "sqsum", st, [&] { k_sqsum<T><<<grid, 256, 0, st>>>(part, count, (double *)slot, cold ? count : 0); });
}

inline IpkTuning ipk_tuning_from_env(size_t num_cu) {
  IpkTuning t;
  t.num_cu = num_cu;
  t.stream = (int)env_get("MGH_IPK_STREAM", t.stream);
  t.dma = (int)env_get("MGH_IPK_DMA", t.dma);
  t.dma_min = (size_t)env_get("MGH_IPK_DMA_MIN", (long)(2 * num_cu));
  t.dma_rounds = (int)env_get("MGH_IPK_DMA_ROUNDS", t.dma_rounds);
  t.spec = (int)env_get("MGH_IPK_SPEC", t.spec);
  t.spec_k = (int)env_get("MGH_IPK_SPEC_K", t.spec_k);
  t.spec_long = (int)env_get("MGH_IPK_SPEC_LONG", t.spec_long);
  t.spec_max = (uint32_t)env_get("MGH_IPK_SPEC_MAX", (long)t.spec_max);
  t.chunk = (int)env_get("MGH_IPK_CHUNK", t.chunk);
  t.chunk_k = (int)env_get("MGH_IPK_CHUNK_K", t.chunk_k);
  t.w = (uint32_t)env_get("MGH_IPK_W", t.w);
  t.wpc = (size_t)env_get("MGH_IPK_WPC", (long)t.wpc);
  t.kr16 = (int)env_get("MGH_IPK_KR16", t.kr16);
  t.contig_rounds = (size_t)env_get("MGH_IPK_CONTIG", (long)t.contig_rounds);
  return t;
}

template <typename F> auto with_type(const mgh_hierarchy *h, F &&f) {
  return h->dtype == MGH_FLOAT ? f(float()) : f(double());
}

}

extern "C" {

const char *mgh_last_error(void) { return g_last_error.c_str(); }

void mgh_set_last_error_(const char *msg) { g_last_error = msg ? msg : ""; }

int mgh_device_count(void) {
  int n = 0;
  if (hipGetDeviceCount(&n) != hipSuccess) return 0;
  return n;
}

int mgh_hierarchy_create(mgh_hierarchy **out, int D, const uint64_t *shape, int dtype,
                         const void *const *h_coords, int normalize_coordinates,
                         uint64_t max_level, int device) {
  if (!out || !shape) return fail(MGH_ERR_INVALID_ARGUMENT, "null argument");
  *out = nullptr;
  if (D < 1 || D > MGH_MAX_DIM) return fail(MGH_ERR_UNSUPPORTED_DIMENSION, "D must be 1..5");
  if (dtype != MGH_FLOAT && dtype != MGH_DOUBLE) return fail(MGH_ERR_UNSUPPORTED_DTYPE, "dtype");
  if (mgh_device_count() <= device || device < 0)
    return fail(MGH_ERR_NO_DEVICE, "HIP device " + std::to_string(device) + " not available");
  HIP_TRY(hipSetDevice(device));
  {
    const std::string bad = env_validate();
    if (!bad.empty()) return fail(MGH_ERR_INVALID_ARGUMENT, bad);
  }
  auto *h = new mgh_hierarchy();
  {
    h->force_v1_env = (int)env_get("MGH_FORCE_V1", -1);
    h->force_v1 = h->force_v1_env == 1;
    h->force_nd = env_get("MGH_FORCE_ND", 0) != 0;
    h->force_nd_ipk = env_get("MGH_ND_IPK", 0) != 0;
    h->absmax_warm_mb = (int)env_get("MGH_ABSMAX_WARM_MB", h->absmax_warm_mb);
    h->fused_faces = (int)env_get("MGH_FUSED_FACES", h->fused_faces);
    h->fused_xcd = (int)env_get("MGH_FUSED_XCD", h->fused_xcd);
    h->slice_batch = (int)env_get("MGH_SLICE_BATCH", h->slice_batch);
    h->fused_tall = (int)env_get("MGH_FUSED_TALL", h->fused_tall);
    h->fused_fixed = (int)env_get("MGH_FUSED_FIXED", h->fused_fixed);
    h->fused_wide = (int)env_get("MGH_FUSED_WIDE", -1);
    h->fused4 = (int)env_get("MGH_FUSED4", h->fused4);
    h->box = (int)env_get("MGH_BOX", h->box);
    h->sym16_mixed = (int)env_get("MGH_SYM16_MIXED", h->sym16_mixed);
    h->outlier_agg = (int)env_get("MGH_OUTLIER_AGG", h->outlier_agg);
    h->tail_solves = (int)env_get("MGH_TAIL_SOLVES", h->tail_solves);
    h->nd_rows = (int)env_get("MGH_ND_ROWS", h->nd_rows);
    h->cls1 = (size_t)env_get("MGH_CLS1", (long)h->cls1);
    h->cls2 = (size_t)env_get("MGH_CLS2", (long)h->cls2);
    if (const char *e = std::getenv("MGH_RCH")) std::sscanf(e, "%d,%d,%d", &h->rch[0], &h->rch[1], &h->rch[2]);
    h->ipk_range_mb = (int)env_get("MGH_IPK_RANGE_MB", h->ipk_range_mb);
    h->no_head = env_get("MGH_NO_RECOMPOSE_HEAD", 0) != 0;
    h->debug_sync = env_get("MGH_DEBUG_SYNC", 0) != 0;
    if (h->force_nd) h->force_v1 = true;
  }
  h->dtype = dtype;
  h->device = device;
  if (h->fused_wide < 0) h->fused_wide = dtype == MGH_FLOAT ? 1 : 0;
  {
    int cus = 0;
    if (hipDeviceGetAttribute(&cus, hipDeviceAttributeMultiprocessorCount, device) == hipSuccess && cus > 0)
      h->num_cu = (size_t)cus;
  }
  h->ipk = ipk_tuning_from_env(h->num_cu);
  h->D = D;
  bool ok;
  if (dtype == MGH_FLOAT) {
    auto *hh = new HostHierarchy<float>();
    h->host = hh;
    ok = hh->init(D, shape, (const float *const *)h_coords, normalize_coordinates != 0, max_level);
    hh->normalize_coordinates = normalize_coordinates != 0;
    h->L = hh->L;
    h->total = ok ? hh->total() : 0;
  } else {
    auto *hh = new HostHierarchy<double>();
    h->host = hh;
    ok = hh->init(D, shape, (const double *const *)h_coords, normalize_coordinates != 0, max_level);
    hh->normalize_coordinates = normalize_coordinates != 0;
    h->L = hh->L;
    h->total = ok ? hh->total() : 0;
  }
  if (!ok) {
    if (dtype == MGH_FLOAT) delete HH<float>(h); else delete HH<double>(h);
    delete h;
    return fail(MGH_ERR_INVALID_ARGUMENT,
                "invalid shape: every dimension must have at least 3 nodes");
  }
  h->plane_elems = shape[D - 1] * (D >= 2 ? shape[D - 2] : 1);
  for (int d = 0; d < D; d++) h->shape[d] = shape[d];
  if (h->force_v1_env < 0 && D == 3) {
    const uint64_t m1 = shape[1] / 2 + 1, m2 = shape[2] / 2 + 1;
    double tiles = (double)((m1 + 7) / 8) * (double)((m2 + 31) / 32);
    if (h->fused_tall && m2 <= 16 && m1 >= 48) tiles = (double)((m1 + 63) / 64) * (double)((m2 + 3) / 4);
    if ((double)(m1 * m2) < 0.125 * tiles * 256.0) h->force_v1 = true;
  }
  int rc = with_type(h, [&](auto t) { return build_device_state<decltype(t)>(h); });
  if (rc != MGH_SUCCESS) {
    mgh_hierarchy_destroy(h);
    return rc;
  }
  *out = h;
  return MGH_SUCCESS;
}

void mgh_hierarchy_destroy(mgh_hierarchy *h) {
  if (!h) return;
  (void)hipSetDevice(h->device);
  for (auto &kv : h->prof)
    for (auto &ev : kv.second.pending) {
      (void)hipEventDestroy(ev.first);
      (void)hipEventDestroy(ev.second);
    }
  with_type(h, [&](auto t) { destroy_state<decltype(t)>(h); return 0; });
  delete h;
}

int mgh_l_target(const mgh_hierarchy *h) { return h ? h->L : MGH_ERR_INVALID_ARGUMENT; }

int mgh_level_shape(const mgh_hierarchy *h, int level, uint64_t *out_shape) {
  if (!h || !out_shape || level < 0 || level > h->L) return fail(MGH_ERR_INVALID_ARGUMENT, "level");
  return with_type(h, [&](auto t) {
    for (int d = 0; d < h->D; d++) out_shape[d] = HH<decltype(t)>(h)->level_shape[level][d];
    return (int)MGH_SUCCESS;
  });
}

uint64_t mgh_total_num_elems(const mgh_hierarchy *h) { return h ? h->total : 0; }
size_t mgh_device_bytes(const mgh_hierarchy *h) { return h ? h->device_bytes : 0; }
const void *mgh_norm_device_ptr(const mgh_hierarchy *h) {
  if (!h) return nullptr;
  return with_type(h, [&](auto t) { return (const void *)DS<decltype(t)>(h)->normval; });
}


// ... 234 lines not shown
    if (level == h->L)
      return recompose_impl<T>(h, (const T *)d_coeff, in, (T *)d_out, dense_layout(h), (hipStream_t)stream);
    return recompose_to_level_impl<T>(h, (const T *)d_coeff, in, level, (T *)d_out, (hipStream_t)stream);
  });
}

int mgh_dequantize_recompose_to_level(mgh_hierarchy *h, int64_t *d_quantized, int ebtype, double tol, double s,
                                      double norm, uint64_t dict_size, int prep_huffman,
                                      const uint64_t *d_outlier_idx, const int64_t *d_outlier_val,
                                      uint64_t outlier_count, int level, void *d_out, void *stream) {
  if (!h || !d_out || !d_quantized) return fail(MGH_ERR_INVALID_ARGUMENT, "null argument");
  if (prep_huffman && outlier_count && (!d_outlier_idx || !d_outlier_val))
    return fail(MGH_ERR_INVALID_ARGUMENT, "null outlier list");
  TRY(level_arg(h, level));
  return reconstruct_entry(h, {ebtype, tol, s, norm, dict_size, prep_huffman, d_outlier_idx, d_outlier_val, outlier_count},
                           {IntSource::Full, d_quantized, nullptr}, {level, 0, nullptr, d_out, dense_layout(h)}, stream);
}

int mgh_level_box_from_linear(mgh_hierarchy *h, const int64_t *d_linear, int level, int64_t *d_box_out, void *stream) {
  if (!h || !d_linear || !d_box_out || d_linear == d_box_out)
    return fail(MGH_ERR_INVALID_ARGUMENT, "mgh_level_box_from_linear: null or aliasing argument");
  TRY(level_arg(h, level));
  HIP_TRY(hipSetDevice(h->device));
  return box_from_linear(h, d_linear, level, d_box_out, (hipStream_t)stream);
}

int mgh_dequantize_recompose_linear_to_level(mgh_hierarchy *h, int64_t *d_linear, int ebtype, double tol, double s,
                                             double norm, uint64_t dict_size, int prep_huffman,
                                             const uint64_t *d_outlier_idx, const int64_t *d_outlier_val,
                                             uint64_t outlier_count, int level, void *d_out, void *stream) {
  if (!h || !d_out || !d_linear) return fail(MGH_ERR_INVALID_ARGUMENT, "null argument");
  if (prep_huffman && outlier_count && (!d_outlier_idx || !d_outlier_val))
    return fail(MGH_ERR_INVALID_ARGUMENT, "null outlier list");
  TRY(level_arg(h, level));
  return reconstruct_entry(h, {ebtype, tol, s, norm, dict_size, prep_huffman, d_outlier_idx, d_outlier_val, outlier_count},
                           {IntSource::Linear, d_linear, nullptr}, {level, 0, nullptr, d_out, dense_layout(h)}, stream);
}

int mgh_refine_level(mgh_hierarchy *h, const void *d_coarse, int64_t *d_segment, int ebtype, double tol, double s,
                     double norm, uint64_t dict_size, int prep_huffman, const uint64_t *d_outlier_idx,
                     const int64_t *d_outlier_val, uint64_t outlier_count, int level, void *d_out, void *stream) {
  if (!h || !d_coarse || !d_segment || !d_out) return fail(MGH_ERR_INVALID_ARGUMENT, "null argument");
  if (prep_huffman && outlier_count && (!d_outlier_idx || !d_outlier_val))
    return fail(MGH_ERR_INVALID_ARGUMENT, "null outlier list");
  if (level < 1 || level > h->L) return fail(MGH_ERR_INVALID_ARGUMENT, "mgh_refine_level: level outside 1 .. l_target");
  if (d_out == d_coarse || d_out == (void *)d_segment)
    return fail(MGH_ERR_INVALID_ARGUMENT, "mgh_refine_level: d_out must not alias an input");
  return reconstruct_entry(h, {ebtype, tol, s, norm, dict_size, prep_huffman, d_outlier_idx, d_outlier_val, outlier_count},
                           {IntSource::Linear, d_segment, nullptr}, {level, level, d_coarse, d_out, dense_layout(h)}, stream);
}

int mgh_dequantize_recompose_sym16_to_level(mgh_hierarchy *h, const uint16_t *d_symbols, int error_bound_type,
                                            double tol, double s, double norm, uint64_t dict_size,
                                            const uint64_t *d_outlier_idx, const int64_t *d_outlier_val,
                                            uint64_t outlier_count, int level, void *d_out, void *stream) {
  if (!h || !d_symbols || !d_out || (outlier_count && (!d_outlier_idx || !d_outlier_val)))
    return fail(MGH_ERR_INVALID_ARGUMENT, "null argument");
  if (dict_size == 0 || dict_size > 65536) return fail(MGH_ERR_INVALID_ARGUMENT, "dict_size must be in 1..65536");
  TRY(level_arg(h, level));
  if (!mgh_sym16_supported(h))
    return fail(MGH_ERR_UNSUPPORTED_DIMENSION, "16-bit symbols: only on the fused 3-D / 4-D path");
  return reconstruct_entry(h, {error_bound_type, tol, s, norm, dict_size, 1, d_outlier_idx, d_outlier_val, outlier_count},
                           {IntSource::Sym16, nullptr, d_symbols}, {level, 0, nullptr, d_out, dense_layout(h)}, stream);
}

#ifdef MGH_PHASE_TIMING
int mgh_debug_tail_read(unsigned long long *out64, int reset) {
  HIP_TRY(hipMemcpyFromSymbol(out64, HIP_SYMBOL(mgh::g_tail), sizeof(unsigned long long) * 64));
  if (reset) {
    unsigned long long z[64] = {0};
    HIP_TRY(hipMemcpyToSymbol(HIP_SYMBOL(mgh::g_tail), z, sizeof z));
  }
  return MGH_SUCCESS;
}
int mgh_debug_phase_read(unsigned long long *out16, int reset) {
  HIP_TRY(hipMemcpyFromSymbol(out16, HIP_SYMBOL(mgh::g_phase), sizeof(unsigned long long) * 16));
  if (reset) {
    unsigned long long z[16] = {0};
    HIP_TRY(hipMemcpyToSymbol(HIP_SYMBOL(mgh::g_phase), z, sizeof z));
  }
  return MGH_SUCCESS;
}
#endif

int mgh_profile_enable(mgh_hierarchy *h, int enable) {
  if (!h) return fail(MGH_ERR_INVALID_ARGUMENT, "null argument");
  h->profiling = enable != 0;
  return MGH_SUCCESS;
}

int mgh_profile_filter(mgh_hierarchy *h, const char *name) {
  if (!h) return fail(MGH_ERR_INVALID_ARGUMENT, "null argument");
  h->prof_filter = name ? name : "";
  return MGH_SUCCESS;
}

int mgh_profile_read(mgh_hierarchy *h, const char **names, double *total_ms, uint64_t *launches,
                     int cap, int reset) {
  if (!h) return fail(MGH_ERR_INVALID_ARGUMENT, "null argument");
  HIP_TRY(hipSetDevice(h->device));
  HIP_TRY(hipDeviceSynchronize());
  int n = 0;
  for (auto &kv : h->prof) {
    ProfileEntry &e = kv.second;
    for (auto &ev : e.pending) {
      float ms = 0;
      HIP_TRY(hipEventElapsedTime(&ms, ev.first, ev.second));
      e.total_ms += ms;
      e.launches++;
      (void)hipEventDestroy(ev.first);
      (void)hipEventDestroy(ev.second);
    }
    e.pending.clear();
    if (n < cap) {
      if (names) names[n] = kv.first.c_str();
      if (total_ms) total_ms[n] = e.total_ms;
      if (launches) launches[n] = e.launches;
    }
    n++;
    if (reset) {
      e.total_ms = 0;
      e.launches = 0;
    }
  }
  return n;
}

int mgh_outlier_restore(int64_t *d_q, uint64_t n, const uint64_t *d_outlier_idx,
                        const int64_t *d_outlier_val, uint64_t outlier_count, void *stream) {
  if (!d_q || (outlier_count && (!d_outlier_idx || !d_outlier_val)))
    return fail(MGH_ERR_INVALID_ARGUMENT, "mgh_outlier_restore: null argument");
  if (!outlier_count) return MGH_SUCCESS;
  hipStream_t st = (hipStream_t)stream;
  mgh::k_outlier_restore<<<(unsigned)((outlier_count + 255) / 256), 256, 0, st>>>(d_q, n, d_outlier_idx,
                                                                                 d_outlier_val, outlier_count);
  HIP_TRY(hipGetLastError());
  return MGH_SUCCESS;
}

int mgh_level_linearize(mgh_hierarchy *h, const int64_t *d_in, int64_t *d_out, int inverse,
                        uint64_t *d_outlier_idx, const uint64_t *d_outlier_count, uint64_t outlier_count,
                        uint64_t outlier_capacity, void *stream) {
  if (!h || !d_in || !d_out || d_in == d_out) return fail(MGH_ERR_INVALID_ARGUMENT, "mgh_level_linearize: null or aliasing argument");
  if (inverse && d_outlier_idx) return fail(MGH_ERR_INVALID_ARGUMENT, "mgh_level_linearize: indices are mapped forward only");
  if (h->L + 1 > mgh::kLinMaxLevels + 1) return fail(MGH_ERR_INVALID_ARGUMENT, "too many levels");
  HIP_TRY(hipSetDevice(h->device));
  hipStream_t st = (hipStream_t)stream;
  mgh::LinMeta m{};
  const int *marks = lin_meta(h, m);
  const size_t total = h->total;
  const unsigned grid = (unsigned)std::min<size_t>((total + 255) / 256, 256 * 32);
  TRY(launch(h, "level_linearize", st, [&] {
    if (inverse) mgh::k_level_linearize<int64_t, true><<<grid, 256, 0, st>>>(m, marks, total, d_in, d_out);
    else mgh::k_level_linearize<int64_t, false><<<grid, 256, 0, st>>>(m, marks, total, d_in, d_out);
  }));
  if (d_outlier_idx && (d_outlier_count || outlier_count)) {
    const unsigned long long cap = outlier_capacity ? outlier_capacity : (d_outlier_count ? ~0ull : outlier_count);
    const size_t work = d_outlier_count ? (size_t)std::min<unsigned long long>(cap, total) : (size_t)outlier_count;
    const unsigned g2 = (unsigned)std::max<size_t>(1, std::min<size_t>((work + 255) / 256, 4096));
    TRY(launch(h, "linearize_indices", st, [&] {
      mgh::k_linearize_indices<<<g2, 256, 0, st>>>(m, marks, total, d_outlier_idx,
                                                   (const unsigned long long *)d_outlier_count,
                                                   (unsigned long long)outlier_count, cap);
    }));
  }
  return MGH_SUCCESS;
// ... 35 lines not shown
```

### mgard_amd/csrc/env.hpp

```cpp
#pragma once
#include <cerrno>
#include <cstdlib>
#include <cstdio>
#include <cstring>
#include <mutex>
#include <string>

extern char **environ;

namespace mgh {

struct EnvSwitch {
  const char *name;
  long lo, hi;
};

inline const EnvSwitch *env_switches(size_t *count) {
  static const EnvSwitch k[] = {
      {"MGH_FORCE_V1", 0, 1},       {"MGH_FORCE_ND", 0, 1},        {"MGH_IPK_STREAM", 0, 1},      {"MGH_IPK_DMA", 0, 1},  {"MGH_IPK_DMA_MIN", 0, 1 << 30},  {"MGH_MULTI_FORCE_PEER", 0, 1},  {"MGH_ABSMAX_WARM_MB", 0, 1 << 20},      {"MGH_FUSED_FACES", 0, 1},
      {"MGH_FUSED_XCD", 0, 1},      {"MGH_FUSED_FIXED", 0, 1},     {"MGH_FUSED_WIDE", 0, 2},
      {"MGH_SLICE_BATCH", 0, 1},      {"MGH_FUSED_TALL", 0, 1},
      {"MGH_FUSED4", 0, 1},         {"MGH_CLS1", 0, 1 << 30},     {"MGH_CLS2", 0, 1 << 30},      {"MGH_RCH", 1, 16},
      {"MGH_IPK_W", 16, 64},        {"MGH_NO_RECOMPOSE_HEAD", 0, 1}, {"MGH_DEBUG_SYNC", 0, 1},
      {"MGH_HL_TIMING", 0, 1},      {"MGH_HUFF_TB", 8, 15},        {"MGH_HUFF_SERIAL_DECODE", 0, 1},
      {"MGH_HUFF_PAR_DECODE", 0, 1}, {"MGH_SYM16_DECODE", 0, 1},   {"MGH_BOX", 0, 3},            {"MGH_IPK_WPC", 1, 16},
      {"MGH_TAIL_SOLVES", 0, 1},    {"MGH_IPK_CONTIG", 2, 1 << 20},
      {"MGH_IPK_KR16", 0, 1},
      {"MGH_IPK_RANGE_MB", 0, 1 << 20},
      {"MGH_HL_PIPELINE", 0, 1},
      {"MGH_SYM16_MIXED", 0, 1},
      {"MGH_IPK_SPEC", 0, 1},
      {"MGH_IPK_SPEC_K", 0, 4096},
      {"MGH_IPK_SPEC_LONG", 0, 1 << 30},
      {"MGH_IPK_SPEC_MAX", 0, 1 << 30},
      {"MGH_IPK_CHUNK", 0, 1},
      {"MGH_OUTLIER_AGG", 0, 2},
      {"MGH_ND_IPK", 0, 1},
      {"MGH_HUFF_SYNC", 0, 1},
      {"MGH_HUFF_SYNC_DECODE", 0, 1},
      {"MGH_IPK_CHUNK_K", 0, 64},
      {"MGH_HL_STREAM_NORM", 0, 1},
      {"MGH_ND_ROWS", 0, 1},
      {"MGH_HUFF_PAIR", 0, 2},
      {"MGH_HL_COPY_THREADS", 1, 32},
      {"MGH_HL_RING_MB", 1, 256},
      {"MGH_HL_DECODE_FOLLOWS", 0, 1},
      {"MGH_HL_COPY_AFFINITY", 0, 1},
      {"MGH_IPK_DMA_ROUNDS", 1, 64},
  };
  *count = sizeof(k) / sizeof(k[0]);
  return k;
}

inline bool env_parse_long(const char *txt, long &v) {
  if (!txt || !*txt) return false;
  char *end = nullptr;
  errno = 0;
  v = std::strtol(txt, &end, 10);
  return errno == 0 && end && *end == '\0';
}

inline void env_warn_unknown_once() {
  static std::once_flag once;
  std::call_once(once, [] {
    size_t n = 0;
    const EnvSwitch *k = env_switches(&n);
    for (char **e = environ; e && *e; e++) {
      if (std::strncmp(*e, "MGH_", 4) != 0) continue;
      const char *eq = std::strchr(*e, '=');
      if (!eq) continue;
      const std::string name(*e, eq - *e);
      bool known = false;
      for (size_t i = 0; i < n; i++) known |= name == k[i].name;
      if (!known)
        std::fprintf(stderr, "libmgard_hip: unknown developer switch %s ignored (DESIGN.md lists them)\n",
                     name.c_str());
    }
  });
}

inline std::string env_validate() {
  env_warn_unknown_once();
  size_t n = 0;
  const EnvSwitch *k = env_switches(&n);
  for (size_t i = 0; i < n; i++) {
    const EnvSwitch *sw = &k[i];
    const char *txt = std::getenv(sw->name);
    if (!txt) continue;
    const std::string name(sw->name), val(txt);
    if (name == "MGH_RCH") {
      int parts = 0;
      size_t pos = 0;
      while (true) {
        const size_t c = val.find(',', pos);
        long v;
        if (!env_parse_long(val.substr(pos, c == std::string::npos ? c : c - pos).c_str(), v) ||
            v < sw->lo || v > sw->hi)
          return "MGH_RCH=" + val + ": expected a,b,c with every value in 1..16";
        parts++;
        if (c == std::string::npos) break;
        pos = c + 1;
      }
      if (parts != 3) return "MGH_RCH=" + val + ": expected three comma-separated values";
      continue;
    }
    long v;
    if (!env_parse_long(val.c_str(), v) || v < sw->lo || v > sw->hi)
      return name + "=" + val + ": expected an integer in " + std::to_string(sw->lo) + ".." +
             std::to_string(sw->hi);
  }
  return std::string();
}

inline long env_get(const char *name, long dflt) {
  const char *e = std::getenv(name);
  long v;
  return env_parse_long(e, v) ? v : dflt;
}

}
```

### mgard_amd/csrc/ipk_plan.hpp

```cpp
#pragma once
#include <algorithm>
#include <cstddef>
#include <cstdint>

namespace mgh {

struct IpkTuning {
  size_t num_cu = 256;
  int stream = 1;
  int dma = 1;
  size_t dma_min = 512;
  int dma_rounds = 4;
  int spec = 1;
  int spec_k = 0;
  int spec_long = 1024;
  uint32_t spec_max = 16384;
  int chunk = 1;
  int chunk_k = 0;
  int chunk_need = 0;
  uint32_t w = 64;
  size_t wpc = 8;
  int kr16 = 1;
  size_t contig_rounds = 4;
};

struct IpkGeom {
  uint32_t n = 0;
  uint32_t npencil = 0;
  uint32_t n_inner = 0;
  size_t outer_stride = 0, inner_stride = 0, stride = 0;
};

inline IpkGeom ipk_geom(int axis, const uint32_t m[3], uint32_t nbatch, size_t batch_stride) {
  IpkGeom g;
  g.n = m[axis];
  if (axis == 2) {
    g.npencil = m[0] * m[1];
    g.n_inner = g.npencil; g.outer_stride = 0; g.inner_stride = g.n; g.stride = 1;
  } else if (axis == 1) {
    g.npencil = m[0] * m[2];
    g.n_inner = m[2]; g.outer_stride = (size_t)m[1] * m[2]; g.inner_stride = 1; g.stride = m[2];
  } else {
    g.npencil = nbatch * m[1] * m[2];
    g.n_inner = m[1] * m[2]; g.outer_stride = batch_stride; g.inner_stride = 1; g.stride = (size_t)m[1] * m[2];
  }
  return g;
}

enum class IpkKernel {
  Spec,
  LdsContigChunked,
  Dma,
  Stream,
  LdsContig,
  LdsStrided,
  Thread
};

struct IpkPlan {
  IpkKernel kernel = IpkKernel::Thread;
  IpkGeom geom;
  uint32_t KR = 0;
  uint32_t W = 0;
  uint32_t P = 0;
  uint32_t n_glob = 0;
  uint32_t K = 0;
  uint32_t S = 0, nchunk = 0;
  uint32_t pad = 0, magic = 0;
  size_t lds = 0;
  size_t lds_attr = 0;
  uint32_t grid = 0, grid_y = 1, block = 64;
  uint32_t check_grid = 0, fix_grid = 0, apply_grid = 0;
  bool per_batch = false;
};

constexpr size_t kLdsPerCU = 160 * 1024;
constexpr size_t kLdsMarginWave = 4096;
constexpr size_t kLdsMarginChunked = 8192;
constexpr size_t kIpkBoxBytesLimit = (size_t)1 << 32;

constexpr size_t ipk_stream_stage_elems(uint32_t U) { return 64 * ((size_t)U + 1); }

inline bool ipk_plane_fits_lds(size_t elem_size, const uint32_t m[3]) {
  return (size_t)m[1] * (m[2] | 1u) * elem_size <= 150 * 1024 && m[1] <= 1024 && m[2] <= 1024;
}

inline IpkPlan ipk_plan(const IpkTuning &t, size_t elem_size, int axis, const uint32_t m[3],
                        uint32_t nbatch, size_t batch_stride) {
  IpkPlan p;
  p.geom = ipk_geom(axis, m, nbatch, batch_stride);
  const uint32_t n = p.geom.n, npencil = p.geom.npencil;
  const size_t pencil_bytes = (size_t)(n + (axis == 2 && n % 2 == 0 ? 1 : 0)) * elem_size;
  auto spec_solve = [&] {
    p.kernel = IpkKernel::Spec;
    p.K = t.spec_k > 0 ? (uint32_t)t.spec_k : (elem_size == 4 ? 64u : 128u);
    const uint32_t S = std::max<uint32_t>(128, std::min<uint32_t>(1024, n / 16384));
    p.S = (S + 7) / 8 * 8;
    p.nchunk = (n + p.S - 1) / p.S;
    const size_t total = (size_t)npencil * n, edges = (size_t)npencil * p.nchunk;
    p.grid = (uint32_t)((edges + 63) / 64);
    p.fix_grid = (npencil + 63) / 64;
    p.check_grid = (uint32_t)((edges + 255) / 256);
    p.apply_grid = (uint32_t)std::min<size_t>((total + 255) / 256, 4096);
    return p;
  };
  const bool spec_ok = t.spec && (nbatch == 1 || batch_stride == (size_t)m[0] * m[1] * m[2]);
  if (axis == 2 && nbatch == 1 && t.spec && npencil <= 64 && n >= 2048) return spec_solve();
  int best_w = 0;
  size_t best_rounds = ~(size_t)0;
  for (int w : {64, 48, 32, 16}) {
    const size_t lds = w * pencil_bytes;
    if (lds > kLdsPerCU) continue;
    const size_t per_cu = std::min<size_t>(kLdsPerCU / lds, 8);
    const size_t blocks = (npencil + w - 1) / w;
    const size_t rounds = (blocks + per_cu * t.num_cu - 1) / (per_cu * t.num_cu);
    if (rounds < best_rounds) {
      best_rounds = rounds;
      best_w = w;
    }
  }
  if (axis != 2 && spec_ok && t.spec_long && n >= (uint32_t)t.spec_long &&
      npencil <= 64u * (uint32_t)t.num_cu && npencil <= t.spec_max)
    return spec_solve();
  auto lds_contig = [&](IpkKernel kernel, uint32_t K, size_t lds_attr) {
    p.kernel = kernel;
    p.K = K;
    p.pad = (n % 2 == 0) ? 1u : 0u;
    p.magic = (uint32_t)((((uint64_t)1 << 32) + n - 1) / n);
    p.P = (uint32_t)best_w;
    p.grid = (npencil + p.P - 1) / p.P;
    p.block = 256;
    p.lds = p.P * pencil_bytes;
    p.lds_attr = lds_attr;
    return p;
  };
  if (t.chunk && axis == 2 && best_w && n >= 64 && best_w * pencil_bytes + kLdsMarginChunked <= kLdsPerCU) {
    const uint32_t K = t.chunk_k > 0 ? (uint32_t)t.chunk_k : (uint32_t)t.chunk_need;
    if (K > 0 && K <= n / 2) return lds_contig(IpkKernel::LdsContigChunked, K, kLdsPerCU - kLdsMarginChunked);
  }
  const uint32_t U = (uint32_t)(64 / elem_size);
  const size_t box_bytes = (nbatch > 1 ? nbatch * batch_stride : (size_t)m[0] * m[1] * m[2]) * elem_size;
  if (elem_size == 4 && t.dma && axis != 2 && box_bytes < kIpkBoxBytesLimit) {
    const uint32_t KR = 10;
    const size_t lds = n < KR * U ? 0 : (size_t)(n - KR * U) * 64 * elem_size;
    if (n >= KR * U && lds <= kLdsPerCU - kLdsMarginWave) {
      const size_t per_cu = lds ? std::min<size_t>((kLdsPerCU - kLdsMarginWave) / lds, 8) : 8;
      const size_t tiles = ((size_t)npencil + 63) / 64;
      const size_t rounds = per_cu >= 4 ? (size_t)t.dma_rounds : 1;
      if (tiles <= per_cu * t.num_cu * rounds && tiles >= t.dma_min) {
        p.kernel = IpkKernel::Dma;
        p.KR = KR;
        p.grid = (uint32_t)((tiles + 7) / 8 * 8);
        p.lds = lds;
        p.lds_attr = kLdsPerCU;
        return p;
      }
    }
  }
  auto stream_plan = [&](uint32_t KR, size_t wpc_cap) {
    const size_t wpc = std::min(t.wpc, wpc_cap);
    const uint32_t nb = n / U;
    const size_t min_rounds = axis == 2 ? t.contig_rounds : 2;
    if (!(t.stream && best_w && best_rounds >= min_rounds && nb >= KR && box_bytes < kIpkBoxBytesLimit))
      return false;
    const uint32_t parked = (nb - KR) * U;
    const size_t stage_bytes = axis == 2 ? ipk_stream_stage_elems(U) * elem_size : 0;
    uint32_t W = 0, n_glob = 0;
    size_t w_rounds = ~(size_t)0;
    for (uint32_t ng = 0; ng <= parked; ng += U) {
      for (uint32_t w : {64u, 60u, 56u, 48u, 40u, 32u, 24u, 16u}) {
        if (w > t.w) continue;
        const size_t lds = (size_t)w * (parked - ng) * elem_size + stage_bytes;
        const size_t per_cu = lds ? std::min<size_t>((kLdsPerCU - kLdsMarginWave) / lds, wpc) : wpc;
        if (!per_cu) continue;
        const size_t blocks = ((size_t)npencil + w - 1) / w;
        const size_t rounds = (blocks + per_cu * t.num_cu - 1) / (per_cu * t.num_cu);
        if (rounds < w_rounds) {
          w_rounds = rounds;
          W = w;
          n_glob = ng;
        }
      }
      if (w_rounds == 1) break;
    }
    if (!(W && w_rounds < best_rounds)) return false;
    p.kernel = IpkKernel::Stream;
    p.KR = KR;
    p.W = W;
    p.n_glob = n_glob;
    p.lds = (size_t)W * (parked - n_glob) * elem_size + stage_bytes;
    p.lds_attr = kLdsPerCU;
    p.grid = ((npencil + W - 1) / W + 7) / 8 * 8;
    return true;
  };
  if (elem_size == 4 && t.kr16 && n / U >= 32 && stream_plan(16, 4)) return p;
  if (stream_plan(8, 16)) return p;
  if (axis == 2 && best_w) return lds_contig(IpkKernel::LdsContig, 0, kLdsPerCU);
  if (axis != 2 && best_w) {
    p.kernel = IpkKernel::LdsStrided;
    p.W = (uint32_t)best_w;
    p.lds = best_w * pencil_bytes;
    p.lds_attr = kLdsPerCU;
    p.grid = ((npencil + best_w - 1) / best_w + 7) / 8 * 8;
    p.block = 256;
    return p;
  }
  if (spec_ok && n >= 2048 && npencil <= t.spec_max) return spec_solve();
  p.kernel = IpkKernel::Thread;
  p.per_batch = nbatch > 1;
  p.grid = (m[axis == 2 ? 1 : 2] + 63) / 64;
  p.grid_y = m[axis == 0 ? 1 : 0];
  return p;
}

}
```

### mgard_amd/csrc/kernels_box.hpp

```cpp
#pragma once
#include <hip/hip_runtime.h>
#include <stdint.h>

#include "kernels_fused.hpp"

namespace mgh {

template <int TR, int TC, int TF> struct BoxGeom {
  static constexpr int WR = 2 * TR + 3, WC = 2 * TC + 3, WF = 2 * TF + 3;
  static constexpr int NW = WR * WC * WF;
  static constexpr int N1 = WR * WC * TF;
  static constexpr int N2 = WR * TC * TF;
  static constexpr int NO = 8 * TR * TC * TF;
  static constexpr int o_cf = NW, o_t1 = 2 * NW, o_t2 = o_t1 + N1, o_rr = o_t2 + N2, o_rc = o_rr + WR,
                       o_rf = o_rc + WC, o_wr = o_rf + WF, o_wc = o_wr + 9 * TR, o_wf = o_wc + 9 * TC,
                       elems = o_wf + 9 * TF;
};

template <typename T, int OUT, int TR, int TC, int TF>
__global__ void __launch_bounds__(256)
k_level_box(FusedArgs<T> A, int gx, int gy) {
  using G = BoxGeom<TR, TC, TF>;
  constexpr int WR = G::WR, WC = G::WC, WF = G::WF, NT = 256, NCOL = WC * WF;
  constexpr bool kQuant = OUT == OUT_Q || OUT == OUT_QH;
// ... 31 lines not shown
      for (int lr = 0; lr < WR; lr++) reg[lr] = col[(size_t)min(max(r_lo + lr, 0), nr - 1) * A.uI];
    }
    for (int e = tid; e < WR; e += NT) {
      const int P = r_lo + e;
      rrs[e] = (P >= 0 && P < nr) ? A.ratio[0][P] : (T)0;
    }
    for (int e = tid; e < WC; e += NT) {
      const int P = c_lo + e;
      rcs[e] = (P >= 0 && P < nc) ? A.ratio[1][P] : (T)0;
    }
    for (int e = tid; e < WF; e += NT) {
      const int P = f_lo + e;
      rfs[e] = (P >= 0 && P < nf) ? A.ratio[2][P] : (T)0;
    }
    for (int e = tid; e < 9 * TR; e += NT) {
      const int k = e / TR, J = R0 + e % TR;
      wrs[e] = J < mr ? A.mass[0][k * mr + J] : (T)0;
    }
    for (int e = tid; e < 9 * TC; e += NT) {
      const int k = e / TC, J = C0 + e % TC;
      wcs[e] = J < mc ? A.mass[1][k * mc + J] : (T)0;
    }
    for (int e = tid; e < 9 * TF; e += NT) {
      const int k = e / TF, J = F0 + e % TF;
      wfs[e] = J < mf ? A.mass[2][k * mf + J] : (T)0;
    }
    if (colthr) {
#pragma unroll
      for (int lr = 0; lr < WR; lr++) raw[lr * NCOL + tid] = reg[lr];
    }
  }
  __syncthreads();

  if (colthr) {
    const int co = lc & 1, fo = lf & 1;
    const bool vcf = Pc >= 0 && Pc <= Pmax_c && Pc != ghost_c && Pf >= 0 && Pf <= Pmax_f && Pf != ghost_f;
    const int i00 = (lc - co) * WF + (lf - fo), i01 = (lc - co) * WF + (lf + fo),
              i10 = (lc + co) * WF + (lf - fo), i11 = (lc + co) * WF + (lf + fo);
    const T rf = rfs[lf - fo], rc = rcs[lc - co];
    auto interp = [&](int lr) {
      const T *pl = raw + lr * NCOL;
      const T x00 = pl[i00], x01 = pl[i01], x10 = pl[i10], x11 = pl[i11];
      const T g0 = fo ? lerp_ref(x00, x01, rf) : x00;
      const T g1 = fo ? lerp_ref(x10, x11, rf) : x10;
      return co ? lerp_ref(g0, g1, rc) : g0;
    };
    auto plane_ok = [&](int lr) {
      const int P = r_lo + lr;
      return P >= 0 && P <= Pmax_r && P != ghost_r;
    };
    const bool odd_cf = (co | fo) != 0;
    T Gp = interp(0);
    cf[tid] = (vcf && odd_cf && plane_ok(0)) ? raw[tid] - Gp : (T)0;
#pragma unroll
    for (int lr = 1; lr < WR; lr += 2) {
      const T Gn = interp(lr + 1);
      cf[(lr + 1) * NCOL + tid] = (vcf && odd_cf && plane_ok(lr + 1)) ? raw[(lr + 1) * NCOL + tid] - Gn : (T)0;
      const T res = lerp_ref(Gp, Gn, rrs[lr - 1]);
      cf[lr * NCOL + tid] = (vcf && plane_ok(lr)) ? raw[lr * NCOL + tid] - res : (T)0;
      Gp = Gn;
    }
  }
  __syncthreads();

  constexpr int NB = TR * TC * TF;
  int64_t qd[4];
  size_t lin[4];
  bool ol[4];
  unsigned long long omask[4];
  const int wave = tid >> 6, lane = tid & 63;
  {
    unsigned nout = 0;
#pragma unroll
    for (int k = 0; k < 4; k++) {
      const int o = k * NT + tid;
      const int cls = o / NB, w = o % NB;
      const int a = w / (TC * TF), bb = (w / TF) % TC, c = w % TF;
      const int pr = (cls >> 2) & 1, pc = (cls >> 1) & 1, pf = cls & 1;
      const int wr_ = 2 * a + 2 + pr, wc_ = 2 * bb + 2 + pc, wf_ = 2 * c + 2 + pf;
      const int Pr = r_lo + wr_, Pcc = c_lo + wc_, Pff = f_lo + wf_;
      const bool valid = Pr <= Pmax_r && Pr != ghost_r && Pcc <= Pmax_c && Pcc != ghost_c &&
                         Pff <= Pmax_f && Pff != ghost_f;
      const int e = wr_ * NCOL + wc_ * WF + wf_;
      if (cls == 0 && valid) A.coarse[((size_t)(R0 + a) * mc + (C0 + bb)) * mf + (F0 + c)] = raw[e];
      lin[k] = (size_t)((pr ? mr : 0) + R0 + a) * A.dI + (size_t)((pc ? mc : 0) + C0 + bb) * A.dJ +
               (size_t)((pf ? mf : 0) + F0 + c);
      const bool on = valid && cls != 0;
      const T v = cf[e];
      ol[k] = false;
      omask[k] = 0;
      if (OUT == OUT_T) {
        if (on) A.coef[lin[k]] = v;
      } else if (kQuant) {
        qd[k] = quantize_fast(v, A.quantizer, A.volume);
        if (A.prep_huffman) {
          qd[k] += A.dict_size / 2;
          ol[k] = on && !(qd[k] >= 0 && qd[k] < A.dict_size);
        }
        omask[k] = __ballot(ol[k]);
        nout += __popcll(omask[k]);
        if (on) {
          const int64_t st = ol[k] ? 0 : qd[k];
          if (A.q16) A.q16[lin[k]] = (uint16_t)st;
          else A.q[lin[k]] = st;
        }
      }
    }
    if (kQuant && lane == 0) wcnt[wave] = nout;
  }
  for (int e = tid; e < G::N1; e += NT) {
    const int jf = e % TF, row = e / TF;
    const T *x = cf + row * WF + 2 * jf;
    T w[9];
#pragma unroll
    for (int k = 0; k < 9; k++) w[k] = wfs[k * TF + jf];
    t1[e] = mass_apply(x[0], x[1], x[2], x[3], x[4], w);
  }
  __syncthreads();
  if (kQuant && tid == 0) {
    const unsigned c0 = wcnt[0], c1 = wcnt[1], c2 = wcnt[2], c3 = wcnt[3];
    const unsigned total = c0 + c1 + c2 + c3;
    wbase_lo[0] = 0;
    wbase_lo[1] = c0;
    wbase_lo[2] = c0 + c1;
    wbase_lo[3] = c0 + c1 + c2;
    gbase = total ? atomicAdd(A.outlier_count, (unsigned long long)total) : 0ull;
  }
  for (int e = tid; e < G::N2; e += NT) {
    const int jf = e % TF, jc = (e / TF) % TC, lr = e / (TF * TC);
    const T *x = t1 + (lr * WC + 2 * jc) * TF + jf;
    T w[9];
#pragma unroll
    for (int k = 0; k < 9; k++) w[k] = wcs[k * TC + jc];
    t2[e] = mass_apply(x[0], x[TF], x[2 * TF], x[3 * TF], x[4 * TF], w);
  }
  __syncthreads();
  if (kQuant) {
    unsigned long long at = gbase + wbase_lo[wave];
#pragma unroll
    for (int k = 0; k < 4; k++) {
      if (ol[k]) {
        const unsigned long long o = at + __popcll(omask[k] & ((1ULL << lane) - 1ULL));
        if (o < A.outlier_cap) {
          A.outlier_idx[o] = lin[k];
          A.outlier_val[o] = qd[k];
        }
      }
      at += __popcll(omask[k]);
    }
  }
  for (int e = tid; e < TR * TC * TF; e += NT) {
    const int jf = e % TF, jc = (e / TF) % TC, jr = e / (TF * TC);
    if (R0 + jr < mr && C0 + jc < mc && F0 + jf < mf) {
      const T *x = t2 + ((2 * jr) * TC + jc) * TF + jf;
      constexpr int S = TC * TF;
      T w[9];
#pragma unroll
      for (int k = 0; k < 9; k++) w[k] = wrs[k * TR + jr];
      A.load[((size_t)(R0 + jr) * mc + (C0 + jc)) * mf + (F0 + jf)] =
          mass_apply(x[0], x[S], x[2 * S], x[3 * S], x[4 * S], w);
    }
  }
}

}
```

### mgard_amd/csrc/kernels_fused.hpp

```cpp
#pragma once
#include <hip/hip_runtime.h>
#include <stdint.h>

#include "kernels_v1.hpp"

namespace mgh {

template <typename T> struct QParamArgs;

template <typename T> struct FusedArgs {
  int n[3], m[3];
  const T *u;
  size_t uI, uJ;
  T *coarse;
  T *load;
  T *coef;
  int64_t *q;
  uint16_t *q16;
  size_t dI, dJ;
  const T *ratio[3];
  const T *mass[3];
  T quantizer, volume;
  const T *qp;
  int level, nlev;
  int64_t dict_size;
  int prep_huffman;
  unsigned long long *outlier_count;
  uint64_t *outlier_idx;
  int64_t *outlier_val;
  unsigned long long outlier_cap;
  unsigned long long *absmax_bits;
};

enum { OUT_T = 0, OUT_Q = 1, OUT_NONE = 2, OUT_QH = 3 };

template <typename T>
__device__ __forceinline__ T mass_apply(T a, T b, T c, T d, T e, const T (&w)[9]) {
  const T tb = a * w[0] + b * w[1] + c * w[2];
  T tc = b * w[2] + c * w[3] + d * w[4];
  const T td = c * w[4] + d * w[5] + e * w[6];
  tc += tb * w[7] + td * w[8];
  return tc;
}

template <typename T>
__device__ __forceinline__ int64_t quantize_fast(T t, T quantizer, T volume) {
  const T a = (T)0.5 + abs_t(t * quantizer * volume);
  if (a < (T)2147483520.0) {
    const int r = (int)a;
    return (int64_t)(t < 0 || (t == 0 && copysign_t((T)1, t) < 0) ? -r : r);
  }
  return (int64_t)copysign_t(a, t);
}

template <typename T, int NV>
__device__ __forceinline__ void emit_quantized(const FusedArgs<T> &A, const T (&v)[NV],
                                               const size_t (&lin)[NV], const bool (&on)[NV]) {
  int64_t qd[NV];
  bool outl[NV];
  bool any = false;
#pragma unroll
  for (int k = 0; k < NV; k++) {
    qd[k] = quantize_fast(v[k], A.quantizer, A.volume);
    outl[k] = false;
    if (A.prep_huffman) {
      qd[k] += A.dict_size / 2;
      outl[k] = on[k] && !(qd[k] >= 0 && qd[k] < A.dict_size);
      any |= outl[k];
    }
  }
  if (__any(any)) {
    unsigned long long masks[NV];
    unsigned total = 0;
#pragma unroll
    for (int k = 0; k < NV; k++) {
      masks[k] = __ballot(outl[k]);
      total += __popcll(masks[k]);
    }
    unsigned long long base = 0;
    const int lane = threadIdx.x & 63;
    if (lane == 0) base = atomicAdd(A.outlier_count, (unsigned long long)total);
    base = __shfl(base, 0, 64);
    unsigned before = 0;
#pragma unroll
    for (int k = 0; k < NV; k++) {
      if (outl[k]) {
        const unsigned rank = __popcll(masks[k] & ((1ULL << lane) - 1ULL));
        const unsigned long long o = base + before + rank;
        if (o < A.outlier_cap) {
          A.outlier_idx[o] = lin[k];
          A.outlier_val[o] = qd[k];
        }
        qd[k] = 0;
      }
      before += __popcll(masks[k]);
    }
  }
#pragma unroll
  for (int k = 0; k < NV; k++)
    if (on[k]) {
      if (A.q16) A.q16[lin[k]] = (uint16_t)qd[k];
      else A.q[lin[k]] = qd[k];
    }
}

template <typename T, int OUT>
__global__ void __launch_bounds__(256)
k_head_out(int m0, int m1, int m2, const T *__restrict__ nodal, FusedArgs<T> A) {
  if (OUT == OUT_Q && A.qp) {
    A.quantizer = A.qp[0];
    A.volume = A.qp[A.nlev];
  }
  const int total = m0 * m1 * m2;
  for (int e = blockIdx.x * blockDim.x + threadIdx.x; e < total; e += gridDim.x * blockDim.x) {
    const int k = e % m2, j = (e / m2) % m1, i = e / (m2 * m1);
    const size_t lin = (size_t)i * A.dI + (size_t)j * A.dJ + k;
    const T v = nodal[e];
    if (OUT == OUT_T) {
      A.coef[lin] = v;
    } else {
      int64_t qd = quantize_one(v, A.quantizer, A.volume);
      if (A.prep_huffman) {
        qd += A.dict_size / 2;
        if (!(qd >= 0 && qd < A.dict_size)) {
          const unsigned long long o = atomicAdd(A.outlier_count, 1ULL);
          if (o < A.outlier_cap) {
            A.outlier_idx[o] = lin;
            A.outlier_val[o] = qd;
          }
          qd = 0;
        }
      }
      if (A.q16) A.q16[lin] = (uint16_t)qd;
      else A.q[lin] = qd;
    }
  }
}

constexpr int kMaxLevels = 40;
template <typename T> struct QParamArgs {
  const T *d_norm;
  const unsigned long long *scalar;
  int s_is_inf, rel, decomposed, normalize;
  unsigned long long total, nsub;
  T tol;
  int nlev;
  double den[kMaxLevels];
  T vol[kMaxLevels];
  T *qp;
  T *norm_out;
  unsigned long long *reset_count;
  unsigned long long *zero_next;
};

template <typename T>
__device__ __forceinline__ T qparams_norm(const QParamArgs<T> &P, const unsigned long long *scalar) {
  T norm;
  if (P.d_norm) {
    norm = *P.d_norm;
  } else if (P.s_is_inf) {
    const unsigned long long bits = *scalar;
    if (sizeof(T) == 4) norm = (T)__uint_as_float((unsigned)bits); else norm = (T)__longlong_as_double((long long)bits);
  } else {
    const double sum = __longlong_as_double((long long)*scalar);
    norm = (T)sum;
    if (sizeof(T) == 4) norm = P.normalize ? (T)sqrtf((float)(norm / (T)P.total)) : (T)sqrtf((float)norm);
    else norm = P.normalize ? (T)sqrt((double)(norm / (T)P.total)) : (T)sqrt((double)norm);
  }
  if (!P.d_norm && norm == 0) norm = sizeof(T) == 4 ? (T)1.1920928955078125e-7f : (T)2.220446049250313e-16;
  return norm;
}
template <typename T> __device__ __forceinline__ double qparams_abs_tol2(const QParamArgs<T> &P, T norm) {
  double abs_tol;
  if (P.decomposed) {
    T lt;
    if (P.s_is_inf) {
      lt = P.rel ? P.tol * norm : P.tol;
    } else {
      const T a = P.rel ? (P.tol * norm) * (P.tol * norm) / (T)P.nsub : (P.tol * P.tol) / (T)P.nsub;
      lt = sizeof(T) == 4 ? (T)sqrtf((float)a) : (T)sqrt((double)a);
    }
    abs_tol = lt;
  } else {
    abs_tol = P.tol;
    if (P.rel) abs_tol *= norm;
  }
  abs_tol *= 2;
  return abs_tol;
}
template <typename T> __device__ __forceinline__ T qparams_level(double abs_tol2, double den) {
  T q = (T)(abs_tol2 / den);
  q = 1.0f / q;
  return q;
}

template <typename T>
__device__ __forceinline__ void make_qparams_body(const QParamArgs<T> &P) {
  const T norm = qparams_norm<T>(P, P.scalar);
  *P.norm_out = norm;
  const double abs_tol = qparams_abs_tol2<T>(P, norm);
// ... 15 lines not shown
```

### mgard_amd/csrc/kernels_fused2.hpp

```cpp
#pragma once
#include <hip/hip_runtime.h>
#include <stdint.h>

#include "kernels_fused.hpp"

namespace mgh {

#ifdef MGH_PHASE_TIMING
__device__ unsigned long long g_phase[2][8];
#define MGH_PT_DECL unsigned long long pt_t = clock64(); const bool pt_on = (blockIdx.x % 97 == 5) && (threadIdx.x == 0 || threadIdx.x == 192); const int pt_w = threadIdx.x == 0 ? 0 : 1;
#define MGH_PT(k) do { const unsigned long long pt_n = clock64(); if (pt_on) atomicAdd(&g_phase[pt_w][k], pt_n - pt_t); pt_t = pt_n; } while (0)
#else
#define MGH_PT_DECL
#define MGH_PT(k)
#endif

__device__ __forceinline__ int32_t cvt_i32_sat(float x) {
  int32_t r;
  asm("v_cvt_i32_f32 %0, %1" : "=v"(r) : "v"(x));
  return r;
}
__device__ __forceinline__ int32_t cvt_i32_sat(double x) {
  int32_t r;
  asm("v_cvt_i32_f64 %0, %1" : "=v"(r) : "v"(x));
// ... 110 lines not shown
    const T *base = vol + (size_t)min(max(p, 0), nr - 1) * A.uI;
#pragma unroll
    for (int k = 0; k < NL; k++) reg[k] = base[goff[k]];
  };
  auto fetch = [&](int p, T(&reg)[NL]) { fetch_from(A.u, p, reg); };
  T amax = 0;
  auto stash = [&](T *dst, const T(&reg)[NL]) {
#pragma unroll
    for (int k = 0; k < NL; k++) {
      dst[lidx[k]] = reg[k];
      if (OUT == OUT_NONE) {
        const T a = abs_t(reg[k]);
        amax = a > amax ? a : amax;
      }
    }
  };

  struct Cell {
    bool c1, f1;
    bool m0, m1, m2, m3;
    bool s0, s1, s2, s3;
    T rc, rf;
    uint32_t i00, i01, i02, i10, i11, i20, i22;
  };
  auto make_cell = [&](int cj, int fj) {
    Cell c;
    const int lc0 = 2 * cj + 2, lf0 = 2 * fj + 2;
    c.c1 = cj < TC;
    c.f1 = fj < TF;
    const int Pc0 = c_lo + lc0, Pf0 = f_lo + lf0;
    const bool vc0 = Pc0 >= 0 && Pc0 <= Pmax_c;
    const bool vf0 = Pf0 >= 0 && Pf0 <= Pmax_f;
    const bool vc1 = c.c1 && Pc0 + 1 >= 0 && Pc0 + 1 <= Pmax_c && Pc0 + 1 != ghost_c;
    const bool vf1 = c.f1 && Pf0 + 1 >= 0 && Pf0 + 1 <= Pmax_f && Pf0 + 1 != ghost_f;
    c.m0 = vc0 && vf0;
    c.m1 = vc0 && vf1;
    c.m2 = vc1 && vf0;
    c.m3 = vc1 && vf1;
    const bool mine = C0 + cj < c_end && F0 + fj < f_end;
    c.s0 = c.m0 && mine;
    c.s1 = c.m1 && mine;
    c.s2 = c.m2 && mine;
    c.s3 = c.m3 && mine;
    const int dc1 = c.c1 ? 1 : 0, dc2 = c.c1 ? 2 : 0, df1 = c.f1 ? 1 : 0, df2 = c.f1 ? 2 : 0;
    c.rc = rcs[lc0];
    c.rf = rfs[lf0];
    c.i00 = LI(lc0, lf0);
    c.i01 = LI(lc0, lf0 + df1);
    c.i02 = LI(lc0, lf0 + df2);
    c.i10 = LI(lc0 + dc1, lf0);
    c.i11 = LI(lc0 + dc1, lf0 + df1);
    c.i20 = LI(lc0 + dc2, lf0);
    c.i22 = LI(lc0 + dc2, lf0 + df2);
    return c;
  };
  __syncthreads();
  const Cell own = make_cell(jc, jf);
  int hcj = 0, hfj = 0;
  if (tid < NH) {
    if (tid < 2 * (TF + 2)) {
      hcj = tid < TF + 2 ? -1 : TC;
      hfj = tid % (TF + 2) - 1;
    } else {
      const int h2 = tid - 2 * (TF + 2);
      hfj = h2 < TC ? -1 : TF;
      hcj = h2 % TC;
    }
  }
  const Cell halo = make_cell(hcj, hfj);
  bool st_on[4];
  {
    const Cell left = make_cell(jc, jf - 1);
    const bool mine = C0 + jc < c_end && F0 + jf < f_end;
    st_on[0] = own.s0;
    st_on[1] = left.m1 && mine;
    st_on[2] = own.s2;
    st_on[3] = left.m3 && mine;
  }
  const bool all_on = __syncthreads_and(st_on[0] && st_on[1] && st_on[2] && st_on[3]) != 0;

  const uint32_t oc0 = (uint32_t)(C0 + jc) * (uint32_t)A.dJ, oc1 = (uint32_t)(mc + C0 + jc) * (uint32_t)A.dJ;
  const uint32_t of0 = (uint32_t)(F0 + jf), of1 = (uint32_t)(mf + F0 + jf - 1 + (F0 + jf == 0));
  const uint32_t off[4] = {oc0 + of0, oc0 + of1, oc1 + of0, oc1 + of1};
  const uint32_t coarse_off = (uint32_t)(C0 + jc) * (uint32_t)mf + (uint32_t)(F0 + jf);
  const T qz = A.quantizer, qv = A.volume;
  const uint32_t dict = (uint32_t)A.dict_size, half = (uint32_t)(A.dict_size / 2);

  auto cell_even = [&](const Cell &c, const T *rw, T *cs, bool pv, T(&E)[4], T(&cv)[4]) {
    const T v00 = rw[c.i00], v01 = rw[c.i01], v02 = rw[c.i02], v10 = rw[c.i10], v11 = rw[c.i11],
            v20 = rw[c.i20], v22 = rw[c.i22];
    const T f0 = lerp_ref(v00, v02, c.rf), f2 = lerp_ref(v20, v22, c.rf);
    E[0] = v00;
    E[1] = f0;
    E[2] = lerp_ref(v00, v20, c.rc);
    E[3] = lerp_ref(f0, f2, c.rc);
    cv[0] = (T)0;
    cv[1] = (pv && c.m1) ? v01 - E[1] : (T)0;
    cv[2] = (pv && c.m2) ? v10 - E[2] : (T)0;
    cv[3] = (pv && c.m3) ? v11 - E[3] : (T)0;
    cs[c.i00] = cv[0];
    if (c.f1) cs[c.i01] = cv[1];
    if (c.c1) cs[c.i10] = cv[2];
    if (c.c1 && c.f1) cs[c.i11] = cv[3];
  };
  auto cell_odd = [&](const Cell &c, const T *rw, T *cs, bool pv, T rr, const T(&G)[4],
                      const T(&E)[4], T(&cv)[4]) {
    const T v00 = rw[c.i00], v01 = rw[c.i01], v10 = rw[c.i10], v11 = rw[c.i11];
    cv[0] = (pv && c.m0) ? v00 - lerp_ref(G[0], E[0], rr) : (T)0;
    cv[1] = (pv && c.m1) ? v01 - lerp_ref(G[1], E[1], rr) : (T)0;
    cv[2] = (pv && c.m2) ? v10 - lerp_ref(G[2], E[2], rr) : (T)0;
    cv[3] = (pv && c.m3) ? v11 - lerp_ref(G[3], E[3], rr) : (T)0;
    cs[c.i00] = cv[0];
    if (c.f1) cs[c.i01] = cv[1];
    if (c.c1) cs[c.i10] = cv[2];
    if (c.c1 && c.f1) cs[c.i11] = cv[3];
  };

  auto interp2 = [&](const Cell &c, const T *rw, T(&E)[4]) {
    const T v00 = rw[c.i00], v02 = rw[c.i02], v20 = rw[c.i20], v22 = rw[c.i22];
    const T f0 = lerp_ref(v00, v02, c.rf), f2 = lerp_ref(v20, v22, c.rf);
    E[0] = v00;
    E[1] = f0;
    E[2] = lerp_ref(v00, v20, c.rc);
    E[3] = lerp_ref(f0, f2, c.rc);
  };
  auto cell_todd = [&](const Cell &c, const T *rw, T *cs, bool pv, const T(&Xa)[4],
                       const T(&Xb)[4], T(&cv)[4]) {
    const T v00 = rw[c.i00], v01 = rw[c.i01], v10 = rw[c.i10], v11 = rw[c.i11];
    cv[0] = (pv && c.m0) ? v00 - lerp_ref(Xa[0], Xb[0], rt) : (T)0;
    cv[1] = (pv && c.m1) ? v01 - lerp_ref(Xa[1], Xb[1], rt) : (T)0;
    cv[2] = (pv && c.m2) ? v10 - lerp_ref(Xa[2], Xb[2], rt) : (T)0;
    cv[3] = (pv && c.m3) ? v11 - lerp_ref(Xa[3], Xb[3], rt) : (T)0;
    cs[c.i00] = cv[0];
    if (c.f1) cs[c.i01] = cv[1];
    if (c.c1) cs[c.i10] = cv[2];
    if (c.c1 && c.f1) cs[c.i11] = cv[3];
  };
  auto pair_todd = [&](const Cell &c, bool pv_o, bool pv_e, T rr, T(&Ga)[4], T(&Gb)[4],
                       T(&cvo)[4], T(&cve)[4]) {
    T Ea[4], Eb[4], Xa[4], Xb[4];
    interp2(c, rawa, Ea);
    interp2(c, rawb, Eb);
    cell_todd(c, raw1, Cs1, pv_e, Ea, Eb, cve);
#pragma unroll
    for (int k = 0; k < 4; k++) {
      Xa[k] = lerp_ref(Ga[k], Ea[k], rr);
      Xb[k] = lerp_ref(Gb[k], Eb[k], rr);
      Ga[k] = Ea[k];
      Gb[k] = Eb[k];
    }
    cell_todd(c, raw0, Cs0, pv_o, Xa, Xb, cvo);
  };

  constexpr bool kLists = AGG && (OUT == OUT_Q || OUT == OUT_QH);
  constexpr int kOutlierStash = kOutlierStashOf<T>;
  auto emit = [&](const T *cs, const T c0, const T c2, int oi, int K0, int which) {
    const size_t ob = out_base + (size_t)oi * A.dI;
    const T cv[4] = {c0, cs[own.i01 - 1], c2, cs[own.i11 - 1]};
    const bool(&on)[4] = st_on;
    if (OUT == OUT_T) {
      T *o = A.coef + ob;
      if (all_on) {
#pragma unroll
        for (int k = 0; k < 4; k++)
          if (k >= K0) o[off[k]] = cv[k];
      } else {
        if (K0 == 0 && on[0]) o[off[0]] = cv[0];
// ... 156 lines not shown
    tc += tb * wc[7] + td * wc[8];
    return tc;
  };

  T Go[4], Gh[4];
  T e_prev;
  T td_prev = 0;
  T Ga2[TODD ? 4 : 1], Gb2[TODD ? 4 : 1], Gha[TODD ? 4 : 1], Ghb[TODD ? 4 : 1];
  struct Pre {
    T o[NL], e[NL], a[TODD ? NL : 1], b[TODD ? NL : 1];
  };
  Pre P0;
  auto fetch_pair = [&](int p, Pre &Q) {
    fetch(p, Q.o);
    fetch(p + 1, Q.e);
    if constexpr (TODD) {
      fetch_from(ua, p + 1, Q.a);
      fetch_from(ub, p + 1, Q.b);
    }
  };
  auto stash_pair = [&](const Pre &Q) {
    stash(raw0, Q.o);
    stash(raw1, Q.e);
    if constexpr (TODD) {
      stash(rawa, Q.a);
      stash(rawb, Q.b);
    }
  };
  fetch(r_lo, P0.e);
  stash(raw1, P0.e);
  if constexpr (TODD) {
    fetch_from(ua, r_lo, P0.a);
    fetch_from(ub, r_lo, P0.b);
    stash(rawa, P0.a);
    stash(rawb, P0.b);
  }
  fetch_pair(r_lo + 1, P0);
  __syncthreads();
  {
    const bool pv = r_lo >= 0 && r_lo <= Pmax_r && r_lo != ghost_r;
    T cv[4];
    if constexpr (TODD) {
      interp2(own, rawa, Ga2);
      interp2(own, rawb, Gb2);
      cell_todd(own, raw1, Cs1, pv, Ga2, Gb2, cv);
      if (tid < NH) {
        interp2(halo, rawa, Gha);
        interp2(halo, rawb, Ghb);
        cell_todd(halo, raw1, Cs1, pv, Gha, Ghb, cv);
      }
    } else {
      cell_even(own, raw1, Cs1, pv, Go, cv);
      if (tid < NH) cell_even(halo, raw1, Cs1, pv, Gh, cv);
    }
  }
  __syncthreads();
  stash_pair(P0);
  if (r_lo + 3 < r_hi) fetch_pair(r_lo + 3, P0);
  phase_b(Cs1, t1s1);
  __syncthreads();
  e_prev = c_sweep(t1s1);
  T o_prev = 0;
  auto pair_step = [&](const int p, Pre &Q) {
    MGH_PT_DECL
    const bool pv_o = p >= 0 && p <= Pmax_r && p != ghost_r;
    const bool pv_e = p + 1 >= 0 && p + 1 <= Pmax_r && p + 1 != ghost_r;
    T keep_o0, keep_o2, keep_e0, keep_e2;
    {
      const T rr = rrs[p - r_lo];
      T E[4], cve[4], cvo[4];
      if constexpr (TODD) {
        pair_todd(own, pv_o, pv_e, rr, Ga2, Gb2, cvo, cve);
        if (tid < NH) {
          T ho[4], he[4];
          pair_todd(halo, pv_o, pv_e, rr, Gha, Ghb, ho, he);
        }
      } else {
        cell_even(own, raw1, Cs1, pv_e, E, cve);
        cell_odd(own, raw0, Cs0, pv_o, rr, Go, E, cvo);
#pragma unroll
        for (int k = 0; k < 4; k++) Go[k] = E[k];
        MGH_PT(6);
        if (pv_e && p + 1 < 2 * R0 + 2 * rch)
          if (all_on || own.s0) A.coarse[(size_t)((p + 1) / 2) * mc * mf + coarse_off] = E[0];
        MGH_PT(7);
        if (tid < NH) {
          T Eh[4], ch[4];
          cell_even(halo, raw1, Cs1, pv_e, Eh, ch);
          cell_odd(halo, raw0, Cs0, pv_o, rr, Gh, Eh, ch);
#pragma unroll
          for (int k = 0; k < 4; k++) Gh[k] = Eh[k];
        }
      }
      keep_o0 = cvo[0];
      keep_o2 = cvo[2];
      keep_e0 = cve[0];
      keep_e2 = cve[2];
    }
    MGH_PT(0);
    __syncthreads();
    MGH_PT(1);
    if (p + 2 < r_hi) {
      stash_pair(Q);
      if (p + 4 < r_hi) fetch_pair(p + 4, Q);
    }
    MGH_PT(2);
    phase_b(Cs0, t1s0);
    phase_b(Cs1, t1s1);
    const bool em_o = pv_o && p >= 2 * R0, em_e = pv_e && p + 1 < 2 * R0 + 2 * rch;
    if (em_o) emit(Cs0, keep_o0, keep_o2, mr + (p - 1) / 2, 0, 0);
    else if (kLists && (tid & 63) == 0) OS.cnt[(tid >> 6) * 2] = 0;
    if (em_e) emit(Cs1, keep_e0, keep_e2, (p + 1) / 2, TODD ? 0 : 1, 1);
    else if (kLists && (tid & 63) == 0) OS.cnt[(tid >> 6) * 2 + 1] = 0;
    MGH_PT(3);
    __syncthreads();
    MGH_PT(4);
    if constexpr (kLists) flush_outliers(mr + (p - 1) / 2, (p + 1) / 2, (unsigned)(p + 64));
    const T vo = c_sweep(t1s0);
    const T ve = c_sweep(t1s1);
    if (p + 1 == 2 * R0) {
      T wr[9];
#pragma unroll
      for (int k = 0; k < 3; k++) wr[k] = wrs[k];
      td_prev = e_prev * wr[0] + vo * wr[1] + ve * wr[2];
    } else {
      const int R = (p - 1) / 2;
      if (R < mr) {
        T wr[9];
#pragma unroll
        for (int k = 0; k < 9; k++) wr[k] = wrs[(R - R0) * 12 + k];
        T tc = mass_tc(o_prev, e_prev, vo, wr);
        const T td = mass_td(e_prev, vo, ve, wr);
        tc += td_prev * wr[7] + td * wr[8];
        td_prev = td;
        if (all_on || own.s0) A.load[(size_t)R * mc * mf + coarse_off] = tc;
      }
    }
    o_prev = vo;
    e_prev = ve;
    MGH_PT(5);
  };
  for (int p = r_lo + 1; p < r_hi; p += 2) pair_step(p, P0);
  if (OUT == OUT_NONE && A.absmax_bits) {
    for (int off = 32; off > 0; off >>= 1) {
      const T o = __shfl_down(amax, off, 64);
      amax = o > amax ? o : amax;
    }
    if ((tid & 63) == 0) {
      unsigned long long bits;
      if (sizeof(T) == 4) bits = __float_as_uint((float)amax); else bits = __double_as_longlong((double)amax);
      if (bits > __atomic_load_n(A.absmax_bits, __ATOMIC_RELAXED)) atomicMax(A.absmax_bits, bits);
    }
  }
#undef LI
}

struct Fused2Grid {
  int gxm, n_main;
  int ff_F0, n_ff;
  int cf_C0, n_cf;
  int rch, nchunk;
  int chunk_hi;
  int xcd_ranges;
};

template <typename T> struct Fused4 {
  const T *ratio_t;
  size_t uT;
  size_t dT;
  size_t cT;
  int n_t, m_t;
};

template <typename T, int OUT, int TC, int TF, int RCH, bool FACES, int TMODE = 0, bool AGG = false>
__global__ void __launch_bounds__(TC * TF)
k_level_fused2(FusedArgs<T> A, Fused2Grid G, Fused4<T> Q) {
  static_assert(TC * TF == 256, "face tiles are 64 x 4 and 4 x 64");
  constexpr bool TODD = TMODE == 2;
  constexpr int e0 = Fused2Geom<TC, TF, RCH, TODD>::elems, e1 = Fused2Geom<64, 4, RCH, TODD>::elems,
                e2 = Fused2Geom<4, 64, RCH, TODD>::elems;
  constexpr int elems = FACES ? (e0 > e1 ? (e0 > e2 ? e0 : e2) : (e1 > e2 ? e1 : e2)) : e0;
  __shared__ __attribute__((aligned(16))) T lds[elems];
  constexpr bool kLists = AGG && (OUT == OUT_Q || OUT == OUT_QH);
  __shared__ __attribute__((aligned(16))) unsigned ol_cnt[8];
  __shared__ unsigned long long ol_base;
  __shared__ unsigned ol_flag;
  __shared__ T ol_val[kLists ? 8 * kOutlierStashOf<T> : 1];
  __shared__ uint32_t ol_off[kLists ? 8 * kOutlierStashOf<T> : 1];
  if (kLists && threadIdx.x == 0) ol_flag = 0;
  const OutlierShared<T> OS{ol_cnt, &ol_base, &ol_flag, ol_val, ol_off};
  if ((OUT == OUT_Q || OUT == OUT_QH) && A.qp) {
    A.quantizer = A.qp[A.level];
    A.volume = A.qp[A.nlev + A.level];
  }
  const T *ua = nullptr, *ub = nullptr;
  T rt = 0;
  size_t out_base = 0;
  if (TMODE != 0) {
    const int zi = blockIdx.z;
    const int P = 2 * zi + (TODD ? 1 : 0);
    const T *vol = A.u;
    A.u = vol + (size_t)min(P, Q.n_t - 1) * Q.uT;
    A.load = A.load + (size_t)P * Q.cT;
    if (TODD) {
      ua = vol + (size_t)(P - 1) * Q.uT;
      ub = vol + (size_t)min(P + 1, Q.n_t - 1) * Q.uT;
      rt = Q.ratio_t[P - 1];
      out_base = (size_t)(Q.m_t + zi) * Q.dT;
    } else {
      A.coarse = A.coarse + (size_t)zi * Q.cT;
      out_base = (size_t)zi * Q.dT;
    }
  }
  const int chunk = G.chunk_hi - 1 - (int)blockIdx.y;
  const int R0 = chunk * G.rch;
  const int rch = chunk == G.nchunk - 1 ? A.m[0] - R0 : G.rch;
  int b = blockIdx.x;
  if (G.xcd_ranges) {
// ... 159 lines not shown
```

### mgard_amd/csrc/kernels_ipk.hpp

```cpp
#pragma once
#include <hip/hip_runtime.h>
#include <stdint.h>

#ifndef MGH_IPK_PHASES
#define MGH_IPK_PHASES 7
#endif

namespace mgh {

template <typename T> struct VecU;
template <> struct VecU<float> {
  typedef float aligned_type __attribute__((ext_vector_type(4)));
  typedef aligned_type type __attribute__((aligned(4)));
  static constexpr int N = 4;
};
template <> struct VecU<double> {
  typedef double aligned_type __attribute__((ext_vector_type(2)));
  typedef aligned_type type __attribute__((aligned(8)));
  static constexpr int N = 2;
};

template <typename T, int U, bool VMEM>
__device__ __forceinline__ void table_load(const T *t, uint32_t zero, T (&out)[U]) {
  if constexpr (VMEM) {
// ... 70 lines not shown
  if constexpr (UB != US)
    for (; k >= US - 1; k -= US) thomas_bwd<T, US, BIG>(s, stride, (uint32_t)k, am, bm, zero, prev);
  for (; k >= 0; k--) {
    T a = s[k * stride];
    a = (a - am[k] * prev) / bm[k];
    s[k * stride] = a;
    prev = a;
  }
}

__device__ __forceinline__ bool same_bits(float a, float b) { return __float_as_uint(a) == __float_as_uint(b); }
__device__ __forceinline__ bool same_bits(double a, double b) { return __double_as_longlong(a) == __double_as_longlong(b); }

template <typename T, int NCH>
__device__ __forceinline__ bool thomas_chunked(T *s, uint32_t stride, uint32_t n,
                                               const T *__restrict__ tt, uint32_t K, uint32_t c,
                                               uint32_t j, bool live, T *edge) {
  const uint32_t CS = (n + NCH - 1) / NCH;
  const uint32_t start = min(n, c * CS), end = min(n, start + CS);
  const T *am = tt + n, *bm = tt + 2 * n;
  uint32_t zero = 0;
  asm volatile("v_mov_b32 %0, 0" : "=v"(zero));
  T *spec = edge + c * 64 + j, *last = edge + (NCH + c) * 64 + j;
  T prev = 0;
  if (live) {
    uint32_t i = start > K ? start - K : 0;
    for (; i + 8 <= start; i += 8) {
      T a[8], w[8];
      table_load<T, 8, true>(tt + i, zero, w);
#pragma unroll
      for (int u = 0; u < 8; u++) a[u] = s[(i + u) * stride];
#pragma unroll
      for (int u = 0; u < 8; u++) prev = a[u] - prev * w[u];
    }
    for (; i < start; i++) prev = s[i * stride] - prev * tt[i];
    *spec = prev;
  }
  __syncthreads();
  if (live) {
    uint32_t i = start;
    for (; i + 8 <= end; i += 8) thomas_fwd<T, 8, true>(s, stride, i, tt, zero, prev);
    for (; i < end; i++) {
      T a = s[i * stride];
      a = a - prev * tt[i];
      s[i * stride] = a;
      prev = a;
    }
    *last = prev;
  }
  __syncthreads();
  bool bad = live && c >= 1 && !same_bits(*spec, edge[(NCH + c - 1) * 64 + j]);
  prev = 0;
  if (live) {
    int64_t k = (int64_t)min((uint64_t)n, (uint64_t)end + K) - 1;
    for (; k - 7 >= (int64_t)end; k -= 8) {
      T a[8], ca[8], cb[8];
      table_load<T, 8, true>(am + (k - 7), zero, ca);
      table_load<T, 8, true>(bm + (k - 7), zero, cb);
#pragma unroll
      for (int u = 0; u < 8; u++) a[u] = s[(k - u) * stride];
#pragma unroll
      for (int u = 0; u < 8; u++) prev = (a[u] - ca[7 - u] * prev) / cb[7 - u];
    }
    for (; k >= (int64_t)end; k--) prev = (s[k * stride] - am[k] * prev) / bm[k];
  }
  if (__syncthreads_or(bad)) return true;
  if (live) {
    *spec = prev;
    int64_t k = (int64_t)end - 1;
    for (; k - 7 >= (int64_t)start; k -= 8) thomas_bwd<T, 8, true>(s, stride, (uint32_t)k, am, bm, zero, prev);
    for (; k >= (int64_t)start; k--) {
      T a = s[k * stride];
      a = (a - am[k] * prev) / bm[k];
      s[k * stride] = a;
      prev = a;
    }
    *last = prev;
  }
  __syncthreads();
  bad = live && c + 1 < NCH && !same_bits(*spec, edge[(NCH + c + 1) * 64 + j]);
  return __syncthreads_or(bad);
}

template <typename T, bool CH = false>
__global__ void __launch_bounds__(256, CH ? 3 : 1)
k_ipk_lds_contig(uint32_t npencil, uint32_t n, uint32_t pad, uint32_t magic, uint32_t P,
                 T *__restrict__ x, const T *__restrict__ tt, T *__restrict__ add_to, int sign,
                 uint32_t K) {
  extern __shared__ __attribute__((aligned(16))) unsigned char smem_raw[];
  T *sm = reinterpret_cast<T *>(smem_raw);
  __shared__ T edge[CH ? 2 * 4 * 64 : 1];
  using VU = typename VecU<T>::type;
  using VA = typename VecU<T>::aligned_type;
  constexpr int VN = VecU<T>::N;
  constexpr int UV = 8;
  const uint32_t tid = threadIdx.x;
  const uint32_t p0 = blockIdx.x * P;
  const uint32_t cnt = min(P, npencil - p0);
  const size_t base = (size_t)p0 * n;
  const uint32_t total = cnt * n;
  const uint32_t nvec = total / VN;
  const T *g = x + base;
  auto lds_put = [&](uint32_t e, const VA &v) {
    if (pad) {
#pragma unroll
      for (int k = 0; k < VN; k++) sm[e + k + __umulhi(e + k, magic)] = v[k];
    } else {
      *reinterpret_cast<VA *>(sm + e) = v;
    }
  };
  auto lds_get = [&](uint32_t e) {
    VA v;
    if (pad) {
#pragma unroll
      for (int k = 0; k < VN; k++) v[k] = sm[e + k + __umulhi(e + k, magic)];
    } else {
      v = *reinterpret_cast<const VA *>(sm + e);
    }
    return v;
  };
  for (int attempt = CH && K > 0 ? 0 : 1; attempt < 2; attempt++) {
    for (uint32_t q = tid; (MGH_IPK_PHASES & 1) && q < nvec; q += UV * 256) {
      VA v[UV];
#pragma unroll
      for (int u = 0; u < UV; u++) {
        const uint32_t qq = min(q + u * 256, nvec - 1);
        v[u] = *reinterpret_cast<const VU *>(g + (size_t)qq * VN);
      }
#pragma unroll
      for (int u = 0; u < UV; u++)
        if (q + u * 256 < nvec) lds_put((q + u * 256) * VN, v[u]);
    }
    for (uint32_t e = nvec * VN + tid; e < total; e += 256)
      sm[e + (pad ? __umulhi(e, magic) : 0u)] = g[e];
    __syncthreads();
    if (CH && attempt == 0) {
      const uint32_t c = __builtin_amdgcn_readfirstlane(tid >> 6), j = tid & 63;
      if (!thomas_chunked<T, 4>(sm + j * (n + pad), 1, n, tt, K, c, j, j < cnt, edge)) break;
      continue;
    }
    if ((MGH_IPK_PHASES & 2) && tid < cnt) thomas_lds<T, !CH>(sm + tid * (n + pad), 1, n, tt);
  }
  __syncthreads();
  T *o = (add_to ? add_to : x) + base;
  if (!(MGH_IPK_PHASES & 4)) return;
  if (add_to) {
    for (uint32_t q = tid; q < nvec; q += UV * 256) {
      VA v[UV];
#pragma unroll
      for (int u = 0; u < UV; u++) {
        const uint32_t qq = min(q + u * 256, nvec - 1);
        v[u] = *reinterpret_cast<const VU *>(o + (size_t)qq * VN);
      }
#pragma unroll
      for (int u = 0; u < UV; u++) {
        if (q + u * 256 < nvec) {
          const uint32_t e = (q + u * 256) * VN;
          const VA d = lds_get(e);
          VA r;
#pragma unroll
          for (int k = 0; k < VN; k++) r[k] = sign > 0 ? v[u][k] + d[k] : v[u][k] - d[k];
          *reinterpret_cast<VU *>(o + e) = r;
        }
      }
    }
    for (uint32_t e = nvec * VN + tid; e < total; e += 256) {
      const T d = sm[e + (pad ? __umulhi(e, magic) : 0u)];
      o[e] = sign > 0 ? o[e] + d : o[e] - d;
    }
  } else {
    for (uint32_t q = tid; q < nvec; q += 256) *reinterpret_cast<VU *>(o + (size_t)q * VN) = lds_get(q * VN);
    for (uint32_t e = nvec * VN + tid; e < total; e += 256)
      o[e] = sm[e + (pad ? __umulhi(e, magic) : 0u)];
  }
}

template <typename T, int W>
__global__ void __launch_bounds__(256)
k_ipk_lds_strided(uint32_t n_outer, uint32_t n_inner, size_t outer_stride, size_t stride,
                  uint32_t n, T *__restrict__ x, const T *__restrict__ tt,
                  T *__restrict__ add_to, int sign) {
  extern __shared__ __attribute__((aligned(16))) unsigned char smem_raw[];
  T *sm = reinterpret_cast<T *>(smem_raw);
  using VU = typename VecU<T>::type;
  using VA = typename VecU<T>::aligned_type;
  constexpr int VN = VecU<T>::N;
  constexpr int WV = W / VN;
  constexpr int RW = 256 / WV;
  constexpr int UR = 9;
  static_assert(W % VN == 0, "tile width must be a multiple of the vector width");
  const uint32_t npencil = n_outer * n_inner;
  const uint32_t cv = threadIdx.x % WV;
  const uint32_t r0 = threadIdx.x / WV;
  const uint32_t per = (gridDim.x + 7) / 8;
  const uint32_t bid = (blockIdx.x % 8) * per + blockIdx.x / 8;
  if ((uint64_t)bid * W >= (uint64_t)n_outer * n_inner) return;
  const uint32_t p = bid * W + cv * VN;
  const bool rows_live = r0 < (uint32_t)RW;
  const uint32_t po = p / n_inner;
  const bool vec = p + VN - 1 < npencil && (p + VN - 1) / n_inner == po;
  size_t base[VN];
  bool live[VN];
#pragma unroll
  for (int k = 0; k < VN; k++) {
    live[k] = p + k < npencil;
    const uint32_t pk = live[k] ? p + k : 0;
    base[k] = (size_t)(pk / n_inner) * outer_stride + (pk % n_inner);
  }
  auto gload = [&](const T *src, uint32_t row) {
    VA v;
    if (vec) {
      v = *reinterpret_cast<const VU *>(src + base[0] + (size_t)row * stride);
    } else {
#pragma unroll
      for (int k = 0; k < VN; k++) v[k] = live[k] ? src[base[k] + (size_t)row * stride] : T(0);
    }
    return v;
  };
  auto gstore = [&](T *dst, uint32_t row, const VA &v) {
    if (vec) {
      *reinterpret_cast<VU *>(dst + base[0] + (size_t)row * stride) = v;
    } else {
#pragma unroll
      for (int k = 0; k < VN; k++)
        if (live[k]) dst[base[k] + (size_t)row * stride] = v[k];
    }
  };
  if ((MGH_IPK_PHASES & 1) && rows_live) {
    for (uint32_t i = r0; i < n; i += UR * RW) {
      VA v[UR];
#pragma unroll
      for (int u = 0; u < UR; u++) v[u] = gload(x, min(i + u * RW, n - 1));
#pragma unroll
      for (int u = 0; u < UR; u++)
        if (i + u * RW < n) *reinterpret_cast<VA *>(sm + (i + u * RW) * W + cv * VN) = v[u];
    }
  }
  __syncthreads();
  if ((MGH_IPK_PHASES & 2) && threadIdx.x < W && bid * W + threadIdx.x < npencil)
    thomas_lds<T>(sm + threadIdx.x, W, n, tt);
  __syncthreads();
  if ((MGH_IPK_PHASES & 4) && rows_live) {
    if (add_to) {
      for (uint32_t i = r0; i < n; i += UR * RW) {
        VA v[UR];
#pragma unroll
        for (int u = 0; u < UR; u++) v[u] = gload(add_to, min(i + u * RW, n - 1));
#pragma unroll
        for (int u = 0; u < UR; u++) {
          if (i + u * RW < n) {
            const VA d = *reinterpret_cast<const VA *>(sm + (i + u * RW) * W + cv * VN);
            VA r;
#pragma unroll
            for (int k = 0; k < VN; k++) r[k] = sign > 0 ? v[u][k] + d[k] : v[u][k] - d[k];
            gstore(add_to, i + u * RW, r);
          }
        }
      }
    } else {
      for (uint32_t i = r0; i < n; i += RW)
        gstore(x, i, *reinterpret_cast<const VA *>(sm + i * W + cv * VN));
    }
  }
}

template <typename T>
__global__ void __launch_bounds__(256)
k_ipk_plane_fc(uint32_t m1, uint32_t m2, uint32_t pitch, uint32_t magic, T *__restrict__ x,
               const T *__restrict__ tt_f, const T *__restrict__ tt_c) {
  extern __shared__ __attribute__((aligned(16))) unsigned char smem_raw[];
  T *sm = reinterpret_cast<T *>(smem_raw);
  using VU = typename VecU<T>::type;
  using VA = typename VecU<T>::aligned_type;
  constexpr int VN = VecU<T>::N;
  constexpr int UV = 8;
  T *g = x + (size_t)blockIdx.x * m1 * m2;
  const uint32_t total = m1 * m2;
  const uint32_t nvec = total / VN;
  const uint32_t padw = pitch - m2;
  auto at = [&](uint32_t e) { return e + (padw ? __umulhi(e, magic) : 0u); };
  for (uint32_t q = threadIdx.x; q < nvec; q += UV * 256) {
    VA v[UV];
#pragma unroll
    for (int u = 0; u < UV; u++)
      v[u] = *reinterpret_cast<const VU *>(g + (size_t)min(q + u * 256, nvec - 1) * VN);
#pragma unroll
    for (int u = 0; u < UV; u++) {
      if (q + u * 256 < nvec) {
        const uint32_t e = (q + u * 256) * VN;
        if (padw) {
#pragma unroll
          for (int k = 0; k < VN; k++) sm[at(e + k)] = v[u][k];
        } else {
          *reinterpret_cast<VA *>(sm + e) = v[u];
        }
      }
    }
  }
  for (uint32_t e = nvec * VN + threadIdx.x; e < total; e += 256) sm[at(e)] = g[e];
  __syncthreads();
  for (uint32_t r = threadIdx.x; r < m1; r += 256) thomas_lds<T>(sm + r * pitch, 1, m2, tt_f);
  __syncthreads();
  for (uint32_t c = threadIdx.x; c < m2; c += 256) thomas_lds<T>(sm + c, pitch, m1, tt_c);
  __syncthreads();
  for (uint32_t q = threadIdx.x; q < nvec; q += 256) {
    const uint32_t e = q * VN;
    VA v;
    if (padw) {
#pragma unroll
      for (int k = 0; k < VN; k++) v[k] = sm[at(e + k)];
    } else {
      v = *reinterpret_cast<const VA *>(sm + e);
    }
    *reinterpret_cast<VU *>(g + e) = v;
  }
  for (uint32_t e = nvec * VN + threadIdx.x; e < total; e += 256) g[e] = sm[at(e)];
}

}
```

### mgard_amd/csrc/kernels_tail.hpp

```cpp
#pragma once
#include <hip/hip_runtime.h>
#include <stdint.h>

#include "kernels_fused.hpp"
#include "kernels_ipk.hpp"
#include "kernels_recompose.hpp"
#include "kernels_v1.hpp"

namespace mgh {

constexpr int kTailMaxLevels = 10;

#ifdef MGH_PHASE_TIMING
__device__ unsigned long long g_tail[64];
#define MGH_TT_DECL unsigned long long tt_t = wall_clock64();
#define MGH_TT(k) do { if (threadIdx.x == 0) { const unsigned long long tt_n = wall_clock64(); atomicAdd(&g_tail[(k) < 64 ? (k) : 63], tt_n - tt_t); tt_t = tt_n; } } while (0)
#else
#define MGH_TT_DECL
#define MGH_TT(k)
#endif

template <typename T> struct TailLevel {
  Box3 b;
  const T *ratio[3];
  const T *mass[3];
  const T *thomas[3];
  T quantizer, volume;
  int level;
};

template <typename T> struct TailArgs {
  int nlevels;
  TailLevel<T> lv[kTailMaxLevels];
  const T *fine;
  size_t fI, fJ;
  const T *pre_load;
  const T *pre_thomas[3];
  const T *tab_base;
  uint32_t tab_count;
  T head_quantizer, head_volume;
  FusedArgs<T> out;
  unsigned long long *outliers_seen;
};

inline size_t tail_lds_elems(const Box3 &b) {
  const size_t nf = (size_t)b.n[0] * b.n[1] * b.n[2];
  const size_t mc = (size_t)b.m[0] * b.m[1] * b.m[2];
  return 2 * nf + (size_t)b.n[0] * b.n[1] * b.m[2] + (size_t)b.n[0] * b.m[1] * b.m[2] + 2 * mc;
}

constexpr int kTailQpMax = 40;
template <typename T> constexpr size_t tail_header_bytes() {
  return (kTailMaxLevels * 9 * sizeof(uint32_t) + 2 * kTailQpMax * sizeof(T) + 15) / 16 * 16;
}
inline size_t tail_table_elems(const Box3 &b) {
  return (size_t)b.n[0] + b.n[1] + b.n[2] + 12 * ((size_t)b.m[0] + b.m[1] + b.m[2]);
}

template <typename T, int OUT>
__global__ void __launch_bounds__(1024)
k_tail(TailArgs<T> A) {
  extern __shared__ __attribute__((aligned(16))) unsigned char smem_raw[];
  const uint32_t tid = threadIdx.x, NT = blockDim.x;
  FusedArgs<T> O = A.out;
  MGH_TT_DECL
  T *qps = reinterpret_cast<T *>(smem_raw + kTailMaxLevels * 9 * sizeof(uint32_t));
  T *tab;
  T *X, *Y, *C, *T1, *T2, *T3;
  {
    const Box3 &b = A.lv[0].b;
    const size_t nf = (size_t)b.n[0] * b.n[1] * b.n[2];
    const size_t mc = (size_t)b.m[0] * b.m[1] * b.m[2];
    T *base = reinterpret_cast<T *>(smem_raw + tail_header_bytes<T>());
    X = base;
    C = X + nf;
    T1 = C + nf;
    T2 = T1 + (size_t)b.n[0] * b.n[1] * b.m[2];
    T3 = T2 + (size_t)b.n[0] * b.m[1] * b.m[2];
    Y = T3 + mc;
    tab = Y + mc;
    if (O.qp)
      for (uint32_t e = tid; e < 2u * (uint32_t)O.nlev && e < 2u * kMaxLevels; e += NT) qps[e] = O.qp[e];
    for (uint32_t e = tid; e < A.tab_count; e += NT) tab[e] = A.tab_base[e];
    const uint32_t n0 = b.n[0], n1 = b.n[1], n2 = b.n[2];
    for (uint32_t e = tid; e < nf; e += NT) {
      const uint32_t k = e % n2, j = (e / n2) % n1, i = e / (n2 * n1);
      X[e] = A.fine[i * A.fI + j * A.fJ + k];
    }
    if (A.pre_load)
      for (uint32_t e = tid; e < nf; e += NT) C[e] = A.pre_load[e];
    __syncthreads();
    MGH_TT(0);
    if (A.pre_load) {
      const T *pt0 = tab + (A.pre_thomas[0] - A.tab_base), *pt1 = tab + (A.pre_thomas[1] - A.tab_base),
              *pt2 = tab + (A.pre_thomas[2] - A.tab_base);
      for (uint32_t p = tid; p < n0 * n1; p += NT) thomas_lds<T, false>(C + (size_t)p * n2, 1, n2, pt2);
      __syncthreads();
      for (uint32_t p = tid; p < n0 * n2; p += NT)
        thomas_lds<T, false>(C + (size_t)(p / n2) * n1 * n2 + (p % n2), n2, n1, pt1);
      __syncthreads();
      for (uint32_t p = tid; p < n1 * n2; p += NT) thomas_lds<T, false>(C + p, n1 * n2, n0, pt0);
      __syncthreads();
      for (uint32_t e = tid; e < nf; e += NT) X[e] = X[e] + C[e];
    }
  }
  __syncthreads();
  MGH_TT(1);
  for (int li = 0; li < A.nlevels; li++) {
    const TailLevel<T> &L = A.lv[li];
    const Box3 b = L.b;
    const uint32_t n0 = b.n[0], n1 = b.n[1], n2 = b.n[2];
    const uint32_t m0 = b.m[0], m1 = b.m[1], m2 = b.m[2];
    const bool qp_lds = O.qp && O.nlev <= kMaxLevels;
    O.quantizer = qp_lds ? qps[L.level] : (O.qp ? O.qp[L.level] : L.quantizer);
    O.volume = qp_lds ? qps[O.nlev + L.level] : (O.qp ? O.qp[O.nlev + L.level] : L.volume);
    const T *ratio0 = tab + (L.ratio[0] - A.tab_base), *ratio1 = tab + (L.ratio[1] - A.tab_base),
            *ratio2 = tab + (L.ratio[2] - A.tab_base);
    const T *mass0 = tab + (L.mass[0] - A.tab_base), *mass1 = tab + (L.mass[1] - A.tab_base),
            *mass2 = tab + (L.mass[2] - A.tab_base);
    const T *thom0 = tab + (L.thomas[0] - A.tab_base), *thom1 = tab + (L.thomas[1] - A.tab_base),
            *thom2 = tab + (L.thomas[2] - A.tab_base);
    {
      const uint32_t total = n0 * n1 * n2;
      for (uint32_t e0 = 0; e0 < total; e0 += NT) {
        const uint32_t e = e0 + tid;
        const bool live = e < total;
        const uint32_t ee = live ? e : 0;
        const uint32_t k = ee % n2, j = (ee / n2) % n1, i = ee / (n2 * n1);
        bool is_coarse;
        const T v = gpk_reo_elem(b, (const T *)X, (size_t)n1 * n2, (size_t)n2, ratio0, ratio1,
                                 ratio2, i, j, k, is_coarse);
        const size_t lin = (size_t)i * O.dI + (size_t)j * O.dJ + k;
        if (live) {
          if (is_coarse)
            Y[((size_t)i * m1 + j) * m2 + k] = v;
          else
            C[ee] = v;
        }
        const bool emit = live && !is_coarse;
        if (OUT == OUT_T) {
          if (emit) O.coef[lin] = v;
        } else {
          const T vv[1] = {v};
          const size_t ll[1] = {lin};
          const bool on[1] = {emit};
          emit_quantized<T, 1>(O, vv, ll, on);
        }
      }
    }
    __syncthreads();
    MGH_TT(2 + 8 * li + 0);
    {
      const uint32_t total = n0 * n1 * m2;
      for (uint32_t e = tid; e < total; e += NT) {
        const uint32_t k = e % m2, j = (e / m2) % n1, i = e / (m2 * n1);
        T1[e] = lpk_elem<T, 2>(n2, m2, (const T *)C, (size_t)n1 * n2, (size_t)n2, mass2, m0, m1, i,
                               j, k);
      }
    }
    __syncthreads();
    MGH_TT(2 + 8 * li + 1);
    {
      const uint32_t total = n0 * m1 * m2;
      for (uint32_t e = tid; e < total; e += NT) {
        const uint32_t k = e % m2, j = (e / m2) % m1, i = e / (m2 * m1);
        T2[e] = lpk_elem<T, 1>(n1, m1, (const T *)T1, (size_t)n1 * m2, (size_t)m2, mass1, 0, 0, i, j,
                               k);
      }
    }
    __syncthreads();
    MGH_TT(2 + 8 * li + 2);
    const uint32_t mtot = m0 * m1 * m2;
    for (uint32_t e = tid; e < mtot; e += NT) {
// ... 179 lines not shown
```

Baseline: 618.2 GB/s.

## Pad work-array rows to 128-byte lines for 3D level solves

Adds a pitched layout for the per-level nodal and load work arrays, rounding the fastest-axis row length up to a 128-byte multiple when it is at least 128 elements. The IPK solve kernels, the plane fc kernel, the fused decompose kernel's coarse/load writes, the tail preload and head output all take explicit row strides, with a fallback to dense layout when a chosen solver cannot handle a pitch. The aim is to make row starts cache-line aligned so the vector loads and stores in the correction solves avoid split lines. In exchange it adds index arithmetic and scalar fallbacks for vectors that straddle rows, plus slightly larger allocations. A debug API that checks the padding is also added.

```diff
diff --git a/include/mgard_hip.h b/include/mgard_hip.h
--- a/include/mgard_hip.h
+++ b/include/mgard_hip.h
@@ -136,6 +136,9 @@
 int mgh_profile_read(mgh_hierarchy *h, const char **names, double *total_ms, uint64_t *launches,
                      int cap, int reset);
 
+int mgh_debug_work_arrays(mgh_hierarchy *h, int check, int byte, uint64_t *padding_elems,
+                          uint64_t *padding_changed);
+
 int mgh_stream_calibrate(int dtype, const void *d_in, int64_t *d_out, void *d_side, uint64_t n,
                          int reps, double *ms_out, void *stream);
 
diff --git a/mgard_amd/__init__.py b/mgard_amd/__init__.py
--- a/mgard_amd/__init__.py
+++ b/mgard_amd/__init__.py
@@ -25,7 +25,7 @@
     "mgh_recompose_to_level", "mgh_dequantize_recompose_to_level",
     "mgh_dequantize_recompose_sym16_to_level", "mgh_level_nodes",
     "mgh_level_box_from_linear", "mgh_dequantize_recompose_linear_to_level",
-    "mgh_refine_level",
+    "mgh_refine_level", "mgh_debug_work_arrays",
 ]
 
 
@@ -84,6 +84,7 @@
                                             C.c_int, vp, vp, vp, vp, u64, vp]
     L.mgh_dequantize_recompose.argtypes = [vp, vp, C.c_int, C.c_double, C.c_double, C.c_double,
                                            u64, C.c_int, vp, vp, u64, vp, vp]
+    L.mgh_debug_work_arrays.argtypes = [vp, C.c_int, C.c_int, u64p, u64p]
     L.mgh_profile_enable.argtypes = [vp, C.c_int]
     L.mgh_profile_filter.argtypes = [vp, C.c_char_p]
     L.mgh_profile_read.argtypes = [vp, C.POINTER(C.c_char_p), C.POINTER(C.c_double), u64p,
@@ -449,6 +450,11 @@
         _check(load_library().mgh_profile_filter(self._h, only.encode() if only else None))
         _check(load_library().mgh_profile_enable(self._h, int(enable)))
 
+    def debug_work_arrays(self, byte, check=False):
+        n, bad = C.c_uint64(0), C.c_uint64(0)
+        _check(load_library().mgh_debug_work_arrays(self._h, int(check), int(byte), C.byref(n), C.byref(bad)))
+        return int(n.value), int(bad.value)
+
     def profile_read(self, reset=True):
         cap = 64
         names = (C.c_char_p * cap)()
diff --git a/mgard_amd/csrc/capi.hip b/mgard_amd/csrc/capi.hip
--- a/mgard_amd/csrc/capi.hip
+++ b/mgard_amd/csrc/capi.hip
@@ -89,6 +89,7 @@
   size_t cls1 = 256, cls2 = 2048;
   int rch[3] = {1, 4, 16};
   int ipk_range_mb = 128;
+  int work_pitch = 1;
   bool no_head = false;
   bool debug_sync = false;
   std::map<std::string, ProfileEntry> prof;
@@ -183,6 +184,39 @@
   return static_cast<DeviceState<T> *>(h->impl);
 }
 
+inline uint32_t ipk_fc_ranges(const mgh_hierarchy *h, size_t box_bytes) {
+  const size_t range_b = (size_t)h->ipk_range_mb << 20;
+  return range_b && box_bytes > 2 * range_b ? (uint32_t)((box_bytes + range_b - 1) / range_b) : 1u;
+}
+inline void ipk_fc_range(const uint32_t *m, uint32_t k, uint32_t nrange, uint32_t &R_lo, uint32_t (&ms)[3]) {
+  R_lo = (uint32_t)((uint64_t)m[0] * k / nrange);
+  ms[0] = (uint32_t)((uint64_t)m[0] * (k + 1) / nrange) - R_lo;
+  ms[1] = m[1];
+  ms[2] = m[2];
+}
+
+struct WorkLayout {
+  size_t I = 0, J = 0;
+  size_t elems(const uint32_t *m) const { return (size_t)m[0] * I; }
+};
+template <typename T> WorkLayout work_layout(const mgh_hierarchy *h, const uint32_t *m) {
+  const WorkLayout dense{(size_t)m[1] * m[2], (size_t)m[2]};
+  const size_t J = work_row_pitch(sizeof(T), m[2], h->D == 3 && h->work_pitch != 0);
+  if (J == m[2]) return dense;
+  const WorkLayout w{(size_t)m[1] * J, J};
+  auto takes = [&](int axis, const uint32_t *mm) {
+    return ipk_plan_takes_pitch(ipk_plan(h->ipk, sizeof(T), axis, mm, 1, 0, J), axis);
+  };
+  if (!takes(0, m)) return dense;
+  const uint32_t nrange = ipk_fc_ranges(h, w.elems(m) * sizeof(T));
+  for (uint32_t k = 0; k < nrange; k++) {
+    uint32_t R_lo, ms[3];
+    ipk_fc_range(m, k, nrange, R_lo, ms);
+    if (!ipk_plane_fits_lds(sizeof(T), ms) && !(takes(2, ms) && takes(1, ms))) return dense;
+  }
+  return w;
+}
+
 template <typename F> int launch(mgh_hierarchy *h, const char *name, hipStream_t s, F &&f) {
   if (h->debug_sync) {
     std::fprintf(stderr, "[mgh] %s\n", name);
@@ -368,14 +402,15 @@
   HIP_TRY(hipMemcpy(ds->marks, marks.data(), marks.size() * sizeof(int), hipMemcpyHostToDevice));
 
   ds->nodal.assign(L + 1, nullptr);
+  size_t t3_cnt = 0;
   for (int l = 0; l < L; l++) {
-    size_t cnt = 1;
-    for (int d = 0; d < D; d++) cnt *= hh->level_shape[l][d];
+    const uint32_t *m = ds->lt[l + 1].box.m;
+    const size_t cnt = work_layout<T>(h, m).elems(m);
+    t3_cnt = std::max(t3_cnt, cnt);
     TRY(dev_alloc(h, &ds->nodal[l], cnt));
   }
   if (L >= 1) {
-    const Box3 &b = ds->lt[L].box;
-    TRY(dev_alloc(h, &ds->t3, (size_t)b.m[0] * b.m[1] * b.m[2]));
+    TRY(dev_alloc(h, &ds->t3, t3_cnt));
   }
   TRY(dev_alloc(h, &ds->qz, (size_t)2 * (L + 1)));
   TRY(dev_alloc(h, &ds->scalar, (size_t)2));
@@ -508,11 +543,13 @@
   });
 }
 
-template <typename T, bool CHUNKED> int ipk_launch_lds_contig(const IpkPlan &p, const IpkArgs<T> &a) {
+template <typename T, bool CHUNKED, bool PITCHED = false>
+int ipk_launch_lds_contig(const IpkPlan &p, const IpkArgs<T> &a) {
+  if (!PITCHED && p.geom.inner_stride != p.geom.n) return ipk_launch_lds_contig<T, CHUNKED, true>(p, a);
   static std::atomic<uint64_t> once{0};
-  TRY(allow_big_lds_once(k_ipk_lds_contig<T, CHUNKED>, once, p.lds_attr));
+  TRY(allow_big_lds_once(k_ipk_lds_contig<T, CHUNKED, PITCHED>, once, p.lds_attr));
   return launch(a.h, a.name, a.s, [&] {
-    k_ipk_lds_contig<T, CHUNKED><<<p.grid, p.block, p.lds, a.s>>>(p.geom.npencil, p.geom.n, p.pad, p.magic, p.P,
+    k_ipk_lds_contig<T, CHUNKED, PITCHED><<<p.grid, p.block, p.lds, a.s>>>(p.geom.npencil, p.geom.n, (uint32_t)p.geom.inner_stride, p.pad, p.magic, p.P,
                                                                   a.x, a.tt, a.add_to, a.sign, p.K);
   });
 }
@@ -559,11 +596,13 @@
 
 template <typename T>
 int ipk_launch(mgh_hierarchy *h, int axis, const uint32_t *m, T *x, const T *tt, T *add_to,
-               int sign, hipStream_t s, uint32_t nbatch = 1, size_t batch_stride = 0) {
+               int sign, hipStream_t s, uint32_t nbatch = 1, size_t batch_stride = 0, size_t pitch = 0) {
   if (nbatch > 1 && axis != 0) return fail(MGH_ERR_INVALID_ARGUMENT, "ipk_launch: batches along the slowest axis only");
   static const char *names[3] = {"ipk_r", "ipk_c", "ipk_f"};
   const IpkArgs<T> a{h, names[axis], x, tt, add_to, sign, s};
-  const IpkPlan p = ipk_plan(h->ipk, sizeof(T), axis, m, nbatch, batch_stride);
+  const IpkPlan p = ipk_plan(h->ipk, sizeof(T), axis, m, nbatch, batch_stride, pitch);
+  if (pitch && pitch != m[2] && (nbatch > 1 || !ipk_plan_takes_pitch(p, axis)))
+    return fail(MGH_ERR_INVALID_ARGUMENT, "ipk_launch: this solve takes dense boxes only");
   switch (p.kernel) {
   case IpkKernel::Spec: return ipk_launch_spec<T>(p, a, axis);
   case IpkKernel::LdsContigChunked: return ipk_launch_lds_contig<T, true>(p, a);
@@ -593,19 +632,26 @@
 
 template <typename T>
 int ipk_fc_launch(mgh_hierarchy *h, const uint32_t *m, T *x, const T *tt_f, const T *tt_c,
-                  hipStream_t s) {
+                  hipStream_t s, size_t gpitch = 0) {
   const uint32_t pitch = m[2] | 1u;
   if (ipk_plane_fits_lds(sizeof(T), m)) {
+    const uint32_t magic = (uint32_t)((((uint64_t)1 << 32) + m[2] - 1) / m[2]);
+    const size_t lds = (size_t)m[1] * pitch * sizeof(T);
+    if (gpitch && gpitch != m[2]) {
+      static std::atomic<uint64_t> once{0};
+      TRY(allow_big_lds_once(k_ipk_plane_fc<T, true>, once));
+      return launch(h, "ipk_fc", s, [&] {
+        k_ipk_plane_fc<T, true><<<m[0], 256, lds, s>>>(m[1], m[2], (uint32_t)gpitch, pitch, magic, x, tt_f, tt_c);
+      });
+    }
     static std::atomic<uint64_t> once{0};
     TRY(allow_big_lds_once(k_ipk_plane_fc<T>, once));
-    const uint32_t magic = (uint32_t)((((uint64_t)1 << 32) + m[2] - 1) / m[2]);
     return launch(h, "ipk_fc", s, [&] {
-      k_ipk_plane_fc<T><<<m[0], 256, (size_t)m[1] * pitch * sizeof(T), s>>>(m[1], m[2], pitch, magic,
-                                                                              x, tt_f, tt_c);
+      k_ipk_plane_fc<T><<<m[0], 256, lds, s>>>(m[1], m[2], m[2], pitch, magic, x, tt_f, tt_c);
     });
   }
-  TRY(ipk_launch<T>(h, 2, m, x, tt_f, nullptr, +1, s));
-  return ipk_launch<T>(h, 1, m, x, tt_c, nullptr, +1, s);
+  TRY(ipk_launch<T>(h, 2, m, x, tt_f, nullptr, +1, s, 1, 0, gpitch));
+  return ipk_launch<T>(h, 1, m, x, tt_c, nullptr, +1, s, 1, 0, gpitch);
 }
 
 template <typename T>
@@ -877,6 +923,9 @@
     A.uJ = sJ;
     A.coarse = ds->nodal[l - 1];
     A.load = ds->t3;
+    const WorkLayout wl = work_layout<T>(h, b.m);
+    A.cI = wl.I;
+    A.cJ = wl.J;
     A.level = l;
     if (OUT == OUT_Q && !qp->d_qp) {
       A.quantizer = qp->qz[l];
@@ -908,23 +957,17 @@
     }
     tail_pre = h->tail_solves && l == l_tail + 1 && l_tail >= 1;
     if (!tail_pre) {
-      const size_t box_b = (size_t)b.m[0] * b.m[1] * b.m[2] * sizeof(T);
-      const size_t range_b = (size_t)h->ipk_range_mb << 20;
-      if (range_b && box_b > 2 * range_b) {
-        const uint32_t nrange = (uint32_t)((box_b + range_b - 1) / range_b);
-        for (uint32_t k = 0; k < nrange; k++) {
-          const uint32_t R_lo = (uint32_t)((uint64_t)b.m[0] * k / nrange), R_hi = (uint32_t)((uint64_t)b.m[0] * (k + 1) / nrange);
-          const uint32_t ms[3] = {R_hi - R_lo, b.m[1], b.m[2]};
-          TRY(ipk_fc_launch<T>(h, ms, ds->t3 + (size_t)R_lo * b.m[1] * b.m[2], t.thomas[2], t.thomas[1], s));
-        }
-      } else {
-        TRY(ipk_fc_launch<T>(h, b.m, ds->t3, t.thomas[2], t.thomas[1], s));
+      const uint32_t nrange = ipk_fc_ranges(h, wl.elems(b.m) * sizeof(T));
+      for (uint32_t k = 0; k < nrange; k++) {
+        uint32_t R_lo, ms[3];
+        ipk_fc_range(b.m, k, nrange, R_lo, ms);
+        TRY(ipk_fc_launch<T>(h, ms, ds->t3 + (size_t)R_lo * wl.I, t.thomas[2], t.thomas[1], s, wl.J));
       }
-      TRY(ipk_launch<T>(h, 0, b.m, ds->t3, t.thomas[0], ds->nodal[l - 1], +1, s));
+      TRY(ipk_launch<T>(h, 0, b.m, ds->t3, t.thomas[0], ds->nodal[l - 1], +1, s, 1, 0, wl.J));
     }
     src = ds->nodal[l - 1];
-    sJ = b.m[2];
-    sI = (size_t)b.m[1] * b.m[2];
+    sJ = wl.J;
+    sI = wl.I;
   }
   if (L <= l_tail) TRY(after_first());
   if (l_tail >= 1) {
@@ -974,7 +1017,7 @@
     TRY(launch(h, "head_out", s, [&] {
       const size_t tot = (size_t)b.m[0] * b.m[1] * b.m[2];
       k_head_out<T, OUT><<<(unsigned)std::min<size_t>((tot + 255) / 256, 1024), 256, 0, s>>>(
-          (int)b.m[0], (int)b.m[1], (int)b.m[2], ds->nodal[0], A);
+          (int)b.m[0], (int)b.m[1], (int)b.m[2], src, sI, sJ, A);
     }));
     if (OUT == OUT_Q && A.prep_huffman && A.outlier_count && ds->outliers_seen)
       k_publish_count<<<1, 1, 0, s>>>(A.outlier_count, ds->outliers_seen);
@@ -1123,6 +1166,8 @@
     A.uJ = sJ;
     A.coarse = ds->nodal4[l - 1];
     A.load = ds->load4;
+    A.cI = (size_t)Mc[2] * Mc[3];
+    A.cJ = (size_t)Mc[3];
     A.level = l;
     if (OUT == OUT_Q && !qp->d_qp) {
       A.quantizer = qp->qz[l];
@@ -2655,6 +2700,43 @@
 
 }
 
+namespace {
+template <typename T>
+int debug_work_arrays(mgh_hierarchy *h, int check, int byte, uint64_t *padding_elems, uint64_t *padding_changed) {
+  auto *ds = DS<T>(h);
+  uint64_t npad = 0, nbad = 0;
+  if (h->D > 3 || h->L < 1) return fail(MGH_ERR_INVALID_ARGUMENT, "mgh_debug_work_arrays: no level work arrays");
+  HIP_TRY(hipDeviceSynchronize());
+  T pattern;
+  std::memset(&pattern, byte, sizeof(T));
+  std::vector<T> host;
+  for (int l = 0; l <= h->L; l++) {
+    const bool is_t3 = l == h->L;
+    const uint32_t *m = ds->lt[is_t3 ? h->L : l + 1].box.m;
+    const WorkLayout w = work_layout<T>(h, m);
+    T *buf = is_t3 ? ds->t3 : ds->nodal[l];
+    size_t cnt = w.elems(m);
+    if (is_t3)
+      for (int k = 1; k <= h->L; k++) cnt = std::max(cnt, work_layout<T>(h, ds->lt[k].box.m).elems(ds->lt[k].box.m));
+    if (!check) {
+      HIP_TRY(hipMemset(buf, byte, cnt * sizeof(T)));
+      continue;
+    }
+    if (w.J == m[2] || (is_t3 && check < 2)) continue;
+    host.resize(w.elems(m));
+    HIP_TRY(hipMemcpy(host.data(), buf, host.size() * sizeof(T), hipMemcpyDeviceToHost));
+    for (size_t r = 0; r < (size_t)m[0] * m[1]; r++)
+      for (size_t k = m[2]; k < w.J; k++) {
+        npad++;
+        nbad += std::memcmp(&host[r * w.J + k], &pattern, sizeof(T)) != 0;
+      }
+  }
+  if (padding_elems) *padding_elems = npad;
+  if (padding_changed) *padding_changed = nbad;
+  return MGH_SUCCESS;
+}
+}
+
 extern "C" {
 
 const char *mgh_last_error(void) { return g_last_error.c_str(); }
@@ -2704,6 +2786,7 @@
     h->cls2 = (size_t)env_get("MGH_CLS2", (long)h->cls2);
     if (const char *e = std::getenv("MGH_RCH")) std::sscanf(e, "%d,%d,%d", &h->rch[0], &h->rch[1], &h->rch[2]);
     h->ipk_range_mb = (int)env_get("MGH_IPK_RANGE_MB", h->ipk_range_mb);
+    h->work_pitch = (int)env_get("MGH_WORK_PITCH", h->work_pitch);
     h->no_head = env_get("MGH_NO_RECOMPOSE_HEAD", 0) != 0;
     h->debug_sync = env_get("MGH_DEBUG_SYNC", 0) != 0;
     if (h->force_nd) h->force_v1 = true;
@@ -3104,6 +3187,15 @@
   return MGH_SUCCESS;
 }
 #endif
+
+int mgh_debug_work_arrays(mgh_hierarchy *h, int check, int byte, uint64_t *padding_elems,
+                          uint64_t *padding_changed) {
+  if (!h) return fail(MGH_ERR_INVALID_ARGUMENT, "null argument");
+  HIP_TRY(hipSetDevice(h->device));
+  return with_type(h, [&](auto t) {
+    return debug_work_arrays<decltype(t)>(h, check, byte, padding_elems, padding_changed);
+  });
+}
 
 int mgh_profile_enable(mgh_hierarchy *h, int enable) {
   if (!h) return fail(MGH_ERR_INVALID_ARGUMENT, "null argument");
diff --git a/mgard_amd/csrc/env.hpp b/mgard_amd/csrc/env.hpp
--- a/mgard_amd/csrc/env.hpp
+++ b/mgard_amd/csrc/env.hpp
@@ -47,6 +47,7 @@
       {"MGH_HL_DECODE_FOLLOWS", 0, 1},
       {"MGH_HL_COPY_AFFINITY", 0, 1},
       {"MGH_IPK_DMA_ROUNDS", 1, 64},
+      {"MGH_WORK_PITCH", 0, 1},
   };
   *count = sizeof(k) / sizeof(k[0]);
   return k;
diff --git a/mgard_amd/csrc/ipk_plan.hpp b/mgard_amd/csrc/ipk_plan.hpp
--- a/mgard_amd/csrc/ipk_plan.hpp
+++ b/mgard_amd/csrc/ipk_plan.hpp
@@ -31,18 +31,27 @@
   size_t outer_stride = 0, inner_stride = 0, stride = 0;
 };
 
-inline IpkGeom ipk_geom(int axis, const uint32_t m[3], uint32_t nbatch, size_t batch_stride) {
+inline size_t work_row_pitch(size_t elem_size, uint32_t m_f, bool padded = true) {
+  const size_t line = 128 / elem_size;
+  return padded && m_f >= 128 ? ((size_t)m_f + line - 1) / line * line : (size_t)m_f;
+}
+
+inline IpkGeom ipk_geom(int axis, const uint32_t m[3], uint32_t nbatch, size_t batch_stride, size_t pitch = 0) {
   IpkGeom g;
   g.n = m[axis];
+  const size_t J = pitch ? pitch : (size_t)m[2];
   if (axis == 2) {
     g.npencil = m[0] * m[1];
-    g.n_inner = g.npencil; g.outer_stride = 0; g.inner_stride = g.n; g.stride = 1;
+    g.n_inner = g.npencil; g.outer_stride = 0; g.inner_stride = J; g.stride = 1;
   } else if (axis == 1) {
     g.npencil = m[0] * m[2];
-    g.n_inner = m[2]; g.outer_stride = (size_t)m[1] * m[2]; g.inner_stride = 1; g.stride = m[2];
-  } else {
+    g.n_inner = m[2]; g.outer_stride = (size_t)m[1] * J; g.inner_stride = 1; g.stride = J;
+  } else if (J == m[2]) {
     g.npencil = nbatch * m[1] * m[2];
     g.n_inner = m[1] * m[2]; g.outer_stride = batch_stride; g.inner_stride = 1; g.stride = (size_t)m[1] * m[2];
+  } else {
+    g.npencil = m[1] * m[2];
+    g.n_inner = m[2]; g.outer_stride = J; g.inner_stride = 1; g.stride = (size_t)m[1] * J;
   }
   return g;
 }
@@ -85,10 +94,23 @@
   return (size_t)m[1] * (m[2] | 1u) * elem_size <= 150 * 1024 && m[1] <= 1024 && m[2] <= 1024;
 }
 
+inline bool ipk_plan_takes_pitch(const IpkPlan &p, int axis) {
+  switch (p.kernel) {
+  case IpkKernel::LdsContigChunked:
+  case IpkKernel::LdsContig:
+  case IpkKernel::Dma:
+  case IpkKernel::LdsStrided: return true;
+  case IpkKernel::Stream: return axis != 2;
+  case IpkKernel::Spec:
+  case IpkKernel::Thread: return false;
+  }
+  return false;
+}
+
 inline IpkPlan ipk_plan(const IpkTuning &t, size_t elem_size, int axis, const uint32_t m[3],
-                        uint32_t nbatch, size_t batch_stride) {
+                        uint32_t nbatch, size_t batch_stride, size_t pitch = 0) {
   IpkPlan p;
-  p.geom = ipk_geom(axis, m, nbatch, batch_stride);
+  p.geom = ipk_geom(axis, m, nbatch, batch_stride, pitch);
   const uint32_t n = p.geom.n, npencil = p.geom.npencil;
   const size_t pencil_bytes = (size_t)(n + (axis == 2 && n % 2 == 0 ? 1 : 0)) * elem_size;
   auto spec_solve = [&] {
@@ -139,7 +161,7 @@
     if (K > 0 && K <= n / 2) return lds_contig(IpkKernel::LdsContigChunked, K, kLdsPerCU - kLdsMarginChunked);
   }
   const uint32_t U = (uint32_t)(64 / elem_size);
-  const size_t box_bytes = (nbatch > 1 ? nbatch * batch_stride : (size_t)m[0] * m[1] * m[2]) * elem_size;
+  const size_t box_bytes = (nbatch > 1 ? nbatch * batch_stride : (size_t)m[0] * m[1] * (pitch ? pitch : (size_t)m[2])) * elem_size;
   if (elem_size == 4 && t.dma && axis != 2 && box_bytes < kIpkBoxBytesLimit) {
     const uint32_t KR = 10;
     const size_t lds = n < KR * U ? 0 : (size_t)(n - KR * U) * 64 * elem_size;
diff --git a/mgard_amd/csrc/kernels_box.hpp b/mgard_amd/csrc/kernels_box.hpp
--- a/mgard_amd/csrc/kernels_box.hpp
+++ b/mgard_amd/csrc/kernels_box.hpp
@@ -137,7 +137,7 @@
       const bool valid = Pr <= Pmax_r && Pr != ghost_r && Pcc <= Pmax_c && Pcc != ghost_c &&
                          Pff <= Pmax_f && Pff != ghost_f;
       const int e = wr_ * NCOL + wc_ * WF + wf_;
-      if (cls == 0 && valid) A.coarse[((size_t)(R0 + a) * mc + (C0 + bb)) * mf + (F0 + c)] = raw[e];
+      if (cls == 0 && valid) A.coarse[(size_t)(R0 + a) * A.cI + (size_t)(C0 + bb) * A.cJ + (F0 + c)] = raw[e];
       lin[k] = (size_t)((pr ? mr : 0) + R0 + a) * A.dI + (size_t)((pc ? mc : 0) + C0 + bb) * A.dJ +
                (size_t)((pf ? mf : 0) + F0 + c);
       const bool on = valid && cls != 0;
@@ -212,7 +212,7 @@
       T w[9];
 #pragma unroll
       for (int k = 0; k < 9; k++) w[k] = wrs[k * TR + jr];
-      A.load[((size_t)(R0 + jr) * mc + (C0 + jc)) * mf + (F0 + jf)] =
+      A.load[(size_t)(R0 + jr) * A.cI + (size_t)(C0 + jc) * A.cJ + (F0 + jf)] =
           mass_apply(x[0], x[S], x[2 * S], x[3 * S], x[4 * S], w);
     }
   }
diff --git a/mgard_amd/csrc/kernels_fused.hpp b/mgard_amd/csrc/kernels_fused.hpp
--- a/mgard_amd/csrc/kernels_fused.hpp
+++ b/mgard_amd/csrc/kernels_fused.hpp
@@ -14,6 +14,7 @@
   size_t uI, uJ;
   T *coarse;
   T *load;
+  size_t cI, cJ;
   T *coef;
   int64_t *q;
   uint16_t *q16;
@@ -106,7 +107,7 @@
 
 template <typename T, int OUT>
 __global__ void __launch_bounds__(256)
-k_head_out(int m0, int m1, int m2, const T *__restrict__ nodal, FusedArgs<T> A) {
+k_head_out(int m0, int m1, int m2, const T *__restrict__ nodal, size_t nI, size_t nJ, FusedArgs<T> A) {
   if (OUT == OUT_Q && A.qp) {
     A.quantizer = A.qp[0];
     A.volume = A.qp[A.nlev];
@@ -115,7 +116,7 @@
   for (int e = blockIdx.x * blockDim.x + threadIdx.x; e < total; e += gridDim.x * blockDim.x) {
     const int k = e % m2, j = (e / m2) % m1, i = e / (m2 * m1);
     const size_t lin = (size_t)i * A.dI + (size_t)j * A.dJ + k;
-    const T v = nodal[e];
+    const T v = nodal[(size_t)i * nI + (size_t)j * nJ + k];
     if (OUT == OUT_T) {
       A.coef[lin] = v;
     } else {
diff --git a/mgard_amd/csrc/kernels_fused2.hpp b/mgard_amd/csrc/kernels_fused2.hpp
--- a/mgard_amd/csrc/kernels_fused2.hpp
+++ b/mgard_amd/csrc/kernels_fused2.hpp
@@ -216,7 +216,7 @@
   const uint32_t oc0 = (uint32_t)(C0 + jc) * (uint32_t)A.dJ, oc1 = (uint32_t)(mc + C0 + jc) * (uint32_t)A.dJ;
   const uint32_t of0 = (uint32_t)(F0 + jf), of1 = (uint32_t)(mf + F0 + jf - 1 + (F0 + jf == 0));
   const uint32_t off[4] = {oc0 + of0, oc0 + of1, oc1 + of0, oc1 + of1};
-  const uint32_t coarse_off = (uint32_t)(C0 + jc) * (uint32_t)mf + (uint32_t)(F0 + jf);
+  const uint32_t coarse_off = (uint32_t)(C0 + jc) * (uint32_t)A.cJ + (uint32_t)(F0 + jf);
   const T qz = A.quantizer, qv = A.volume;
   const uint32_t dict = (uint32_t)A.dict_size, half = (uint32_t)(A.dict_size / 2);
 
@@ -539,7 +539,7 @@
         for (int k = 0; k < 4; k++) Go[k] = E[k];
         MGH_PT(6);
         if (pv_e && p + 1 < 2 * R0 + 2 * rch)
-          if (all_on || own.s0) A.coarse[(size_t)((p + 1) / 2) * mc * mf + coarse_off] = E[0];
+          if (all_on || own.s0) A.coarse[(size_t)((p + 1) / 2) * A.cI + coarse_off] = E[0];
         MGH_PT(7);
         if (tid < NH) {
           T Eh[4], ch[4];
@@ -590,7 +590,7 @@
         const T td = mass_td(e_prev, vo, ve, wr);
         tc += td_prev * wr[7] + td * wr[8];
         td_prev = td;
-        if (all_on || own.s0) A.load[(size_t)R * mc * mf + coarse_off] = tc;
+        if (all_on || own.s0) A.load[(size_t)R * A.cI + coarse_off] = tc;
       }
     }
     o_prev = vo;
diff --git a/mgard_amd/csrc/kernels_ipk.hpp b/mgard_amd/csrc/kernels_ipk.hpp
--- a/mgard_amd/csrc/kernels_ipk.hpp
+++ b/mgard_amd/csrc/kernels_ipk.hpp
@@ -176,9 +176,9 @@
   return __syncthreads_or(bad);
 }
 
-template <typename T, bool CH = false>
+template <typename T, bool CH = false, bool PITCHED = false>
 __global__ void __launch_bounds__(256, CH ? 3 : 1)
-k_ipk_lds_contig(uint32_t npencil, uint32_t n, uint32_t pad, uint32_t magic, uint32_t P,
+k_ipk_lds_contig(uint32_t npencil, uint32_t n, uint32_t pitch, uint32_t pad, uint32_t magic, uint32_t P,
                  T *__restrict__ x, const T *__restrict__ tt, T *__restrict__ add_to, int sign,
                  uint32_t K) {
   extern __shared__ __attribute__((aligned(16))) unsigned char smem_raw[];
@@ -191,10 +191,28 @@
   const uint32_t tid = threadIdx.x;
   const uint32_t p0 = blockIdx.x * P;
   const uint32_t cnt = min(P, npencil - p0);
-  const size_t base = (size_t)p0 * n;
+  const size_t base = (size_t)p0 * pitch;
   const uint32_t total = cnt * n;
   const uint32_t nvec = total / VN;
   const T *g = x + base;
+  const uint32_t gap = PITCHED ? pitch - n : 0u;
+  auto goff = [&](uint32_t e) { return e + (gap ? gap * __umulhi(e, magic) : 0u); };
+  auto whole = [&](uint32_t e) { return !gap || __umulhi(e, magic) == __umulhi(e + VN - 1, magic); };
+  auto gload = [&](const T *src, uint32_t e) {
+    if (whole(e)) return VA(*reinterpret_cast<const VU *>(src + goff(e)));
+    VA v;
+#pragma unroll
+    for (int k = 0; k < VN; k++) v[k] = src[goff(e + k)];
+    return v;
+  };
+  auto gstore = [&](T *dst, uint32_t e, const VA &v) {
+    if (whole(e)) {
+      *reinterpret_cast<VU *>(dst + goff(e)) = v;
+    } else {
+#pragma unroll
+      for (int k = 0; k < VN; k++) dst[goff(e + k)] = v[k];
+    }
+  };
   auto lds_put = [&](uint32_t e, const VA &v) {
     if (pad) {
 #pragma unroll
@@ -219,14 +237,14 @@
 #pragma unroll
       for (int u = 0; u < UV; u++) {
         const uint32_t qq = min(q + u * 256, nvec - 1);
-        v[u] = *reinterpret_cast<const VU *>(g + (size_t)qq * VN);
+        v[u] = gload(g, qq * VN);
       }
 #pragma unroll
       for (int u = 0; u < UV; u++)
         if (q + u * 256 < nvec) lds_put((q + u * 256) * VN, v[u]);
     }
     for (uint32_t e = nvec * VN + tid; e < total; e += 256)
-      sm[e + (pad ? __umulhi(e, magic) : 0u)] = g[e];
+      sm[e + (pad ? __umulhi(e, magic) : 0u)] = g[goff(e)];
     __syncthreads();
     if (CH && attempt == 0) {
       const uint32_t c = __builtin_amdgcn_readfirstlane(tid >> 6), j = tid & 63;
@@ -244,7 +262,7 @@
 #pragma unroll
       for (int u = 0; u < UV; u++) {
         const uint32_t qq = min(q + u * 256, nvec - 1);
-        v[u] = *reinterpret_cast<const VU *>(o + (size_t)qq * VN);
+        v[u] = gload(o, qq * VN);
       }
 #pragma unroll
       for (int u = 0; u < UV; u++) {
@@ -254,18 +272,19 @@
           VA r;
 #pragma unroll
           for (int k = 0; k < VN; k++) r[k] = sign > 0 ? v[u][k] + d[k] : v[u][k] - d[k];
-          *reinterpret_cast<VU *>(o + e) = r;
+          gstore(o, e, r);
         }
       }
     }
     for (uint32_t e = nvec * VN + tid; e < total; e += 256) {
       const T d = sm[e + (pad ? __umulhi(e, magic) : 0u)];
-      o[e] = sign > 0 ? o[e] + d : o[e] - d;
+      T *const q = o + goff(e);
+      *q = sign > 0 ? *q + d : *q - d;
     }
   } else {
-    for (uint32_t q = tid; q < nvec; q += 256) *reinterpret_cast<VU *>(o + (size_t)q * VN) = lds_get(q * VN);
+    for (uint32_t q = tid; q < nvec; q += 256) gstore(o, q * VN, lds_get(q * VN));
     for (uint32_t e = nvec * VN + tid; e < total; e += 256)
-      o[e] = sm[e + (pad ? __umulhi(e, magic) : 0u)];
+      o[goff(e)] = sm[e + (pad ? __umulhi(e, magic) : 0u)];
   }
 }
 
@@ -358,9 +377,9 @@
   }
 }
 
-template <typename T>
+template <typename T, bool PITCHED = false>
 __global__ void __launch_bounds__(256)
-k_ipk_plane_fc(uint32_t m1, uint32_t m2, uint32_t pitch, uint32_t magic, T *__restrict__ x,
+k_ipk_plane_fc(uint32_t m1, uint32_t m2, uint32_t gpitch, uint32_t pitch, uint32_t magic, T *__restrict__ x,
                const T *__restrict__ tt_f, const T *__restrict__ tt_c) {
   extern __shared__ __attribute__((aligned(16))) unsigned char smem_raw[];
   T *sm = reinterpret_cast<T *>(smem_raw);
@@ -368,16 +387,26 @@
   using VA = typename VecU<T>::aligned_type;
   constexpr int VN = VecU<T>::N;
   constexpr int UV = 8;
-  T *g = x + (size_t)blockIdx.x * m1 * m2;
+  T *g = x + (size_t)blockIdx.x * m1 * gpitch;
   const uint32_t total = m1 * m2;
   const uint32_t nvec = total / VN;
   const uint32_t padw = pitch - m2;
   auto at = [&](uint32_t e) { return e + (padw ? __umulhi(e, magic) : 0u); };
+  const uint32_t gap = PITCHED ? gpitch - m2 : 0u;
+  auto goff = [&](uint32_t e) { return e + (gap ? gap * __umulhi(e, magic) : 0u); };
+  auto whole = [&](uint32_t e) { return !gap || __umulhi(e, magic) == __umulhi(e + VN - 1, magic); };
   for (uint32_t q = threadIdx.x; q < nvec; q += UV * 256) {
     VA v[UV];
 #pragma unroll
-    for (int u = 0; u < UV; u++)
-      v[u] = *reinterpret_cast<const VU *>(g + (size_t)min(q + u * 256, nvec - 1) * VN);
+    for (int u = 0; u < UV; u++) {
+      const uint32_t e = min(q + u * 256, nvec - 1) * VN;
+      if (whole(e)) {
+        v[u] = *reinterpret_cast<const VU *>(g + goff(e));
+      } else {
+#pragma unroll
+        for (int k = 0; k < VN; k++) v[u][k] = g[goff(e + k)];
+      }
+    }
 #pragma unroll
     for (int u = 0; u < UV; u++) {
       if (q + u * 256 < nvec) {
@@ -391,7 +420,7 @@
       }
     }
   }
-  for (uint32_t e = nvec * VN + threadIdx.x; e < total; e += 256) sm[at(e)] = g[e];
+  for (uint32_t e = nvec * VN + threadIdx.x; e < total; e += 256) sm[at(e)] = g[goff(e)];
   __syncthreads();
   for (uint32_t r = threadIdx.x; r < m1; r += 256) thomas_lds<T>(sm + r * pitch, 1, m2, tt_f);
   __syncthreads();
@@ -406,9 +435,14 @@
     } else {
       v = *reinterpret_cast<const VA *>(sm + e);
     }
-    *reinterpret_cast<VU *>(g + e) = v;
-  }
-  for (uint32_t e = nvec * VN + threadIdx.x; e < total; e += 256) g[e] = sm[at(e)];
-}
-
-}
+    if (whole(e)) {
+      *reinterpret_cast<VU *>(g + goff(e)) = v;
+    } else {
+#pragma unroll
+      for (int k = 0; k < VN; k++) g[goff(e + k)] = v[k];
+    }
+  }
+  for (uint32_t e = nvec * VN + threadIdx.x; e < total; e += 256) g[goff(e)] = sm[at(e)];
+}
+
+}
diff --git a/mgard_amd/csrc/kernels_tail.hpp b/mgard_amd/csrc/kernels_tail.hpp
--- a/mgard_amd/csrc/kernels_tail.hpp
+++ b/mgard_amd/csrc/kernels_tail.hpp
@@ -86,9 +86,8 @@
     for (uint32_t e = tid; e < nf; e += NT) {
       const uint32_t k = e % n2, j = (e / n2) % n1, i = e / (n2 * n1);
       X[e] = A.fine[i * A.fI + j * A.fJ + k];
-    }
-    if (A.pre_load)
-      for (uint32_t e = tid; e < nf; e += NT) C[e] = A.pre_load[e];
+      if (A.pre_load) C[e] = A.pre_load[i * A.fI + j * A.fJ + k];
+    }
     __syncthreads();
     MGH_TT(0);
     if (A.pre_load) {
```

New measurement: 588.2 GB/s. 4.9% lower.
